# Runki2018/litehandnet

Hardware: AMD Instinct MI355X
Metric: images/sec fwd+bwd @256x256 bs64 litehandnet (higher is better)
Workload: dtype f32; 1 GPU; litehandnet variant B (MSRB hourglass litehourglass.py) C=128, 256x256x3 -> 21x64x64, per-GPU batch 64, train-mode BN, fwd + TopdownHeatmapLoss + bwd + fused Adam; global_batch=64, parallelism=dp1

## Files before the change

### include/lhn.h

```cpp
#ifndef LHN_H
#define LHN_H
#include <stdint.h>
#ifdef __cplusplus
extern "C" {
#endif

#define LHN_VERSION 3
#define LHN_STAT_REPLICAS 32

typedef struct lhn_view {
  float*       data;
  const float* table;
  const float* gate;
  int32_t N, H, W;
  int32_t cstride;
  int32_t coff;
  int32_t C;
  const void* pend;
} lhn_view;

typedef struct lhn_gradview {
  const float* dz;
  const float* dpool;
  const float* coef;
// ... 307 lines not shown
#define LHN_DW_F_NO_DX     32
#define LHN_DW_F_DX_ACC    64
#define LHN_DW_F_FINSRC    128
#define LHN_DW_SW_GATHER    1
#define LHN_DW_SW_BWD_V1    2
#define LHN_DW_SW_BWD_SMALL 4
const char* lhn_conv_dw_route(int backward, int H, int W, int C, int k, int stride, int pad, int dil, int features, int switches);
int lhn_conv_pw_bwd4(const lhn_view* x, const float* w, const lhn_view* y, const lhn_gradview* gy, float* dx, int dx_accumulate,
                     float* dw, float* dbias, int stride, const float* dy_nchw, int nrep, int64_t rep_stride,
                     const lhn_pw_opts* opts, const lhn_bnsum* bns, const lhn_bnbwdsrc* fin, void* stream);
#define LHN_PW_F_NCHW      1
#define LHN_PW_F_STATS     2
#define LHN_PW_F_FUSE_FIN  4
#define LHN_PW_F_EXTRA1    8
#define LHN_PW_F_EXTRA2    16
#define LHN_PW_F_SUM_OUT   32
#define LHN_PW_F_BNSUM     64
#define LHN_PW_F_FIN       128
#define LHN_PW_F_GATESUM   256
#define LHN_PW_F_NO_DX     512
#define LHN_PW_F_DX_ACC    1024
#define LHN_PW_F_DZ_DEAD   2048
#define LHN_PW_F_UNALIGNED 4096
#define LHN_PW_F_DBIAS     8192
#define LHN_PW_F_FINSRC    16384
#define LHN_PW_SW_LDSW          1
#define LHN_PW_SW_K256          2
#define LHN_PW_SW_BWD_NARROW    4
#define LHN_PW_SW_BWD_SPLIT     8
#define LHN_PW_SW_HEAD_STREAM   16
#define LHN_PW_SW_DETERMINISTIC 32
const char* lhn_conv_pw_route(int backward, int N, int H, int W, int Cin, int Cout, int stride, int w_rows, int w_cols, int features,
                              int switches);
int lhn_avgpool_bwd(const lhn_view* x, const float* dout , int OH, int OW, float* dx,
                    int dx_accumulate, void* stream);
int lhn_gate_bwd_reduce(const lhn_view* y, const float* dz, float* dgate , void* stream);
typedef struct lhn_bn_slices {
  const float* save[2];
  double*      sums[2];
  int32_t      lo[2], C[2];
  int32_t      n;
} lhn_bn_slices;
int lhn_gate_bwd_reduce2(const lhn_view* y, const float* dz, float* dgate , float* tsum,
                         const lhn_bn_slices* slices, void* stream);
int lhn_gate_bwd_reduce3(const lhn_view* y, const float* dz, float* dgate, float* tsum, const lhn_bn_slices* slices, int prezeroed,
                         void* stream);
typedef struct lhn_gatesum {
  float*               dgate;
  const lhn_bn_slices* slices;
} lhn_gatesum;
int lhn_conv_pw_bwd5(const lhn_view* x, const float* w, const lhn_view* y, const lhn_gradview* gy, float* dx, int dx_accumulate,
                     float* dw, float* dbias, int stride, const float* dy_nchw, int nrep, int64_t rep_stride,
                     const lhn_pw_opts* opts, const lhn_bnsum* bns, const lhn_bnbwdsrc* fin, const lhn_gatesum* gs, void* stream);
#define LHN_PW_BWD_DZ_DEAD 1
int lhn_conv_pw_bwd6(const lhn_view* x, const float* w, const lhn_view* y, const lhn_gradview* gy, float* dx, int dx_accumulate,
                     float* dw, float* dbias, int stride, const float* dy_nchw, int nrep, int64_t rep_stride,
                     const lhn_pw_opts* opts, const lhn_bnsum* bns, const lhn_bnbwdsrc* fin, const lhn_gatesum* gs, int flags,
                     void* stream);
int lhn_avgpool_fwd3(const lhn_view* x, float* out , int OH, int OW, float* pstat ,
                     const lhn_bn_slices* slices, void* stream);
int lhn_ca_mlp_bwd2(const float* pooled, const float* w3, const float* gamma, const float* w1, const float* w2,
                    const float* dropmask, const float* save, const float* dgate, float* dpool, int cstride, int coff, int H,
                    int W, float* dw3, float* dgamma, float* dbeta, float* dw1, float* db1, float* dw2, float* db2, int N, int C,
                    int stage, double* gsum, double count_scale, float pgrad_scale, const float* tsum, const float* pstat,
                    const lhn_bn_slices* slices, void* stream);
int lhn_avgpool_fwd4(const lhn_view* x, float* out, int OH, int OW, float* pstat, const lhn_bn_slices* slices,
                     const lhn_view* copy_src, void* stream);
int lhn_ca_mlp_bwd(const float* pooled, const float* w3, const float* gamma, const float* w1, const float* w2,
                   const float* dropmask, const float* save, const float* dgate, float* dpool ,
                   int cstride, int coff, int H, int W, float* dw3, float* dgamma, float* dbeta, float* dw1,
                   float* db1, float* dw2, float* db2, int N, int C, int stage, double* gsum, double count_scale,
                   float pgrad_scale, void* stream);

int lhn_cbam_layout(int N, int H, int W, int C, int64_t* save_off , int64_t* scratch_off );
int lhn_cbam_fwd(const lhn_view* p, const lhn_view* r, const float* w1, const float* w2, const float* w7, const lhn_view* out,
                 float* save, void* stream);
int lhn_cbam_bwd(const lhn_view* p, const lhn_view* r, const float* w1, const float* w2, const float* w7, const lhn_view* out,
                 const float* dout, float* dp, float* dr, float* dw1, float* dw2, float* dw7, const float* save, float* scratch,
                 void* stream);

int lhn_adam_step(float* param, const float* grad, float* exp_avg, float* exp_avg_sq, int64_t n, double lr, double beta1,
                  double beta2, double eps, double weight_decay, int64_t step, void* stream);

typedef struct lhn_op {
  int32_t kind;
  int32_t in_buf[3], in_coff[3], in_C[3];
  int32_t reserved[6];
  int32_t out_buf, out_coff, out_C;
  int32_t p[12];
  int64_t ws[12];
  int32_t i[8];
  float   f[8];
} lhn_op;

typedef struct lhn_buf {
  int64_t data_off, table_off, gate_off, grad_off, dpool_off, coef_off;
  int32_t N, H, W, C;
} lhn_buf;

void* lhn_plan_create(const lhn_buf* bufs, int nbufs, const lhn_op* fwd, int nfwd, const lhn_op* bwd, int nbwd);
void  lhn_plan_destroy(void* plan);
int   lhn_plan_head_gate_fold(void* plan);
int   lhn_plan_pw_dz_dead(void* plan, int bwd_index);
int   lhn_plan_fwd_fin_consumer(void* plan, int fwd_index);
#define LHN_RUN_TABLES_CURRENT 2
#define LHN_RUN_GRAPH 4
int   lhn_plan_run(void* plan, int phase, void* workspace, void* const* params, void* const* grads,
                   void* const* io, int training, int grad_replicas, int64_t grad_rep_stride, void* stream);

#ifdef __cplusplus
}
#endif
#endif
```

### litehandnet_amd/_lib.py

```python
import ctypes as C
import os

import torch

_HERE = os.path.dirname(os.path.abspath(__file__))
LIB_PATH = os.path.join(_HERE, "liblhn.so")
_lib = None


class LhnError(RuntimeError):
    pass


class View(C.Structure):
    _fields_ = [("data", C.c_void_p), ("table", C.c_void_p), ("gate", C.c_void_p),
                ("N", C.c_int32), ("H", C.c_int32), ("W", C.c_int32),
                ("cstride", C.c_int32), ("coff", C.c_int32), ("C", C.c_int32), ("pend", C.c_void_p)]


class GradView(C.Structure):
    _fields_ = [("dz", C.c_void_p), ("dpool", C.c_void_p), ("coef", C.c_void_p)]


class CcwSe(C.Structure):
    _fields_ = [("w1", C.c_void_p), ("b1", C.c_void_p), ("w2", C.c_void_p), ("b2", C.c_void_p), ("J", C.c_int32)]


class Op(C.Structure):
    _fields_ = [("kind", C.c_int32),
                ("in_buf", C.c_int32 * 3), ("in_coff", C.c_int32 * 3), ("in_C", C.c_int32 * 3), ("reserved", C.c_int32 * 6),
                ("out_buf", C.c_int32), ("out_coff", C.c_int32), ("out_C", C.c_int32),
                ("p", C.c_int32 * 12), ("ws", C.c_int64 * 12), ("i", C.c_int32 * 8), ("f", C.c_float * 8)]


class Buf(C.Structure):
    _fields_ = [("data_off", C.c_int64), ("table_off", C.c_int64), ("gate_off", C.c_int64),
                ("grad_off", C.c_int64), ("dpool_off", C.c_int64), ("coef_off", C.c_int64),
                ("N", C.c_int32), ("H", C.c_int32), ("W", C.c_int32), ("C", C.c_int32)]


SYMBOLS = [
    "lhn_version", "lhn_deterministic", "lhn_last_error", "lhn_device_ok",
    "lhn_heatmap_encode", "lhn_heatmap_argmax", "lhn_heatmap_refine", "lhn_transform_preds",
    "lhn_heatmap_decode", "lhn_heatmap_decode_dark", "lhn_heatmap_decode_dark_udp", "lhn_heatmap_nms", "lhn_heatmap_topk", "lhn_pck_accuracy",
    "lhn_eval_state_bytes", "lhn_eval_accumulate", "lhn_eval_finalize",
    "lhn_loss_balanced_mse_fwd", "lhn_loss_balanced_mse_bwd", "lhn_affine_warp_normalize", "lhn_affine_warp_normalize2", "lhn_random_flip", "lhn_hsv_jitter", "lhn_simdr_encode", "lhn_simdr_loss_fwd", "lhn_simdr_loss_bwd",
    "lhn_conv_pw_fwd", "lhn_conv_pw_fwd2", "lhn_conv_pw_bwd2", "lhn_conv_dw_fwd", "lhn_conv_dw_fwd2", "lhn_conv_dw_fwd3", "lhn_conv_pw_dw3_fwd", "lhn_conv_dw3_pw_fwd", "lhn_msrb_round_scratch_bytes", "lhn_msrb_round_fwd", "lhn_bottleneck_fwd", "lhn_stem_tail_fwd", "lhn_conv_stem_fwd", "lhn_conv_kxk_fwd", "lhn_conv_kxk_fwd_bf16x3",
    "lhn_bn_finalize", "lhn_table_fill", "lhn_table_bias", "lhn_fold_bn", "lhn_ew_fwd", "lhn_ew_fwd2", "lhn_ew_fwd3", "lhn_ew_mul_bwd", "lhn_bilinear_bwd", "lhn_shuffle2_fwd", "lhn_shuffle2_bwd", "lhn_bn_finalize2", "lhn_bn_bwd_finalize2", "lhn_maxpool2_fwd", "lhn_avgpool_fwd", "lhn_avgpool_fwd2", "lhn_avgpool_bwd2", "lhn_se_mlp_fwd2", "lhn_se_mlp_bwd2", "lhn_ca_mlp_fwd", "lhn_att_mlp_fwd", "lhn_att_mlp_bwd", "lhn_se_mlp_fwd", "lhn_se_mlp_bwd",
    "lhn_bn_bwd_reduce", "lhn_bn_bwd_finalize", "lhn_conv_pw_bwd", "lhn_conv_dw_bwd", "lhn_conv_dw_bwd2", "lhn_conv_dw_bwd3", "lhn_conv_dw_bwd4", "lhn_conv_dw_route", "lhn_conv_pw_route", "lhn_conv_pw_bwd4", "lhn_conv_pw_bwd5", "lhn_conv_pw_bwd6", "lhn_plan_head_gate_fold", "lhn_plan_pw_dz_dead", "lhn_plan_fwd_fin_consumer", "lhn_conv_dw_fwd4", "lhn_conv_pw_fwd3", "lhn_conv_stem_bwd",
    "lhn_conv_kxk_bwd", "lhn_ew_bwd", "lhn_ew_bwd2", "lhn_maxpool2_bwd", "lhn_maxpool2_bwd2", "lhn_maxpool2_bwd3", "lhn_ew_bwd3", "lhn_ew_bwd_multi", "lhn_avgpool_bwd3", "lhn_conv_pw_bwd3", "lhn_avgpool_bwd", "lhn_gate_bwd_reduce", "lhn_gate_bwd_reduce2", "lhn_gate_bwd_reduce3", "lhn_adam_step", "lhn_avgpool_fwd3", "lhn_avgpool_fwd4", "lhn_ca_mlp_bwd2",
    "lhn_ca_mlp_bwd", "lhn_reduce_replicas", "lhn_fold_stat_replicas", "lhn_plan_create", "lhn_plan_destroy", "lhn_plan_run", "lhn_plan_run_range",
    "lhn_cbam_layout", "lhn_cbam_fwd", "lhn_cbam_bwd",
    "lhn_ccw_scratch_bytes", "lhn_ccw_pool_fwd", "lhn_ccw_gate_fwd", "lhn_ccw_dw_fwd", "lhn_ccw_shuffle_fwd",
]


def lib():
    global _lib
    if _lib is None:
        if not os.path.exists(LIB_PATH):
            raise LhnError(f"{LIB_PATH} is missing: run `python -m litehandnet_amd.build` "
                           "(hipcc --offload-arch=gfx950); there is no CPU fallback")
        _lib = C.CDLL(LIB_PATH)
        _lib.lhn_last_error.restype = C.c_char_p
        _lib.lhn_plan_create.restype = C.c_void_p
        _lib.lhn_plan_destroy.restype = None
        _lib.lhn_eval_state_bytes.restype = C.c_int64
        _lib.lhn_conv_dw_route.argtypes = [C.c_int] * 10
        _lib.lhn_conv_dw_route.restype = C.c_char_p
        _lib.lhn_conv_pw_route.argtypes = [C.c_int] * 11
        _lib.lhn_conv_pw_route.restype = C.c_char_p
        _lib.lhn_conv_dw3_pw_fwd.argtypes = [C.c_void_p, C.c_void_p, C.c_int, C.c_void_p, C.c_void_p, C.c_void_p, C.c_void_p, C.c_void_p]
        _lib.lhn_conv_dw3_pw_fwd.restype = C.c_int
        _lib.lhn_msrb_round_scratch_bytes.argtypes = [C.c_int, C.c_int, C.c_int, C.c_int]
        _lib.lhn_msrb_round_scratch_bytes.restype = C.c_int64
        _lib.lhn_msrb_round_fwd.argtypes = [C.c_void_p, C.c_void_p, C.c_void_p, C.c_void_p, C.c_void_p, C.c_void_p, C.c_void_p, C.c_int, C.c_int,
                                            C.c_void_p, C.c_void_p]
        _lib.lhn_msrb_round_fwd.restype = C.c_int
        _lib.lhn_bottleneck_fwd.argtypes = [C.c_void_p, C.c_int] + [C.c_void_p] * 8 + [C.c_float, C.c_void_p, C.c_void_p, C.c_void_p]
        _lib.lhn_bottleneck_fwd.restype = C.c_int
        _lib.lhn_stem_tail_fwd.argtypes = [C.c_void_p, C.c_int] + [C.c_void_p] * 14
        _lib.lhn_stem_tail_fwd.restype = C.c_int
        _lib.lhn_conv_kxk_fwd_bf16x3.argtypes = [C.c_void_p, C.c_void_p, C.c_void_p, C.c_void_p, C.c_int, C.c_void_p]
        _lib.lhn_conv_kxk_fwd_bf16x3.restype = C.c_int
        _lib.lhn_ccw_scratch_bytes.argtypes = [C.c_int, C.c_int, C.c_void_p, C.c_void_p, C.c_void_p]
        _lib.lhn_ccw_scratch_bytes.restype = C.c_int64
        _lib.lhn_ccw_pool_fwd.argtypes = [C.c_void_p, C.c_int, C.c_void_p, C.c_void_p]
        _lib.lhn_ccw_pool_fwd.restype = C.c_int
        _lib.lhn_ccw_gate_fwd.argtypes = [C.c_void_p, C.c_int64, C.c_int, C.c_int, C.c_void_p, C.c_void_p, C.c_int, C.c_void_p, C.c_void_p, C.c_int,
                                          C.c_void_p, C.c_void_p]
        _lib.lhn_ccw_gate_fwd.restype = C.c_int
        _lib.lhn_ccw_dw_fwd.argtypes = [C.c_void_p, C.c_int] + [C.c_void_p] * 5
        _lib.lhn_ccw_dw_fwd.restype = C.c_int
        _lib.lhn_ccw_shuffle_fwd.argtypes = [C.c_void_p, C.c_void_p, C.c_int] + [C.c_void_p] * 4
        _lib.lhn_ccw_shuffle_fwd.restype = C.c_int
        _lib.lhn_cbam_layout.argtypes = [C.c_int, C.c_int, C.c_int, C.c_int, C.c_void_p, C.c_void_p]
        _lib.lhn_cbam_layout.restype = C.c_int
        _lib.lhn_cbam_fwd.argtypes = [C.c_void_p] * 8
        _lib.lhn_cbam_fwd.restype = C.c_int
        _lib.lhn_cbam_bwd.argtypes = [C.c_void_p] * 15
        _lib.lhn_cbam_bwd.restype = C.c_int
    return _lib


def cbam_layout(N, H, W, Cc):
    sv, sc = (C.c_int64 * 10)(), (C.c_int64 * 8)()
    check(lib().lhn_cbam_layout(N, H, W, Cc, sv, sc), "lhn_cbam_layout")
    return list(sv), list(sc)


def check(status, what=""):
    if status != 0:
        raise LhnError(f"{what}: status {status}: {lib().lhn_last_error().decode()}")


def require_device(t=None):
    if not torch.cuda.is_available():
        raise LhnError("no GPU visible: litehandnet_amd has no CPU fallback")
    if t is not None and not t.is_cuda:
        raise LhnError("tensor must live on the GPU (litehandnet_amd has no CPU fallback)")


def ptr(t):
    return C.c_void_p(0) if t is None else C.c_void_p(t.data_ptr())


def stream():
    return C.c_void_p(torch.cuda.current_stream().cuda_stream)


def f32c(t, name="tensor"):
    require_device(t)
    if t.dtype != torch.float32:
        t = t.float()
    return t.contiguous()
```

### litehandnet_amd/csrc/k_misc.hip

```cpp
#include "lhn_common.h"

static inline int grid_cap(int64_t blocks, int cap_per_cu) {
  const int64_t cap = (int64_t)lhn_num_cus() * cap_per_cu;
  if (blocks > cap) blocks = cap;
  if (blocks < 1) blocks = 1;
  return (int)blocks;
}
static inline bool pow2i(int v) { return v > 0 && (v & (v - 1)) == 0; }

__global__ void __launch_bounds__(LHN_FIN_THREADS) k_bn_finalize(const double* __restrict__ stats, const float* __restrict__ gamma,
                              const float* __restrict__ beta, float* __restrict__ rmean, float* __restrict__ rvar,
                              int64_t* __restrict__ nbt, float* __restrict__ table, int cs, int coff, int C,
                              float* __restrict__ save, double count, float eps, float momentum, float slope, int training,
                              const float* __restrict__ cbias, int SC) {
  __shared__ double part[2 * LHN_FIN_THREADS];
  const int nt = blockDim.x;
  int G = nt / C;
  G = G < 1 ? 1 : (G > LHN_STAT_REPLICAS ? LHN_STAT_REPLICAS : G);
  for (int c0 = 0; c0 < C; c0 += nt) {
    const int g = threadIdx.x / C, c = c0 + (G > 1 ? threadIdx.x - g * C : threadIdx.x);
    if (c0) __syncthreads();
    if (training && g < G && c < C) {
      double s1 = 0, s2 = 0;
#pragma unroll 4
      for (int r = g; r < LHN_STAT_REPLICAS; r += G) {
        s1 += stats[(size_t)r * 2 * SC + c];
        s2 += stats[(size_t)r * 2 * SC + SC + c];
      }
      part[2 * threadIdx.x] = s1;
      part[2 * threadIdx.x + 1] = s2;
    }
    __syncthreads();
    if (g != 0 || c >= C) continue;
    double mean, var;
    const double cb = cbias ? (double)cbias[c] : 0.0;
    if (training) {
      double s1 = 0, s2 = 0;
      for (int k = 0; k < G; ++k) {
        s1 += part[2 * (k * C + threadIdx.x)];
        s2 += part[2 * (k * C + threadIdx.x) + 1];
      }
      lhn_bn_fin_moments(s1, s2, count, mean, var);
      if (rmean) lhn_bn_fin_running(rmean, rvar, c, rmean[c], rvar[c], mean, var, cb, count, momentum);
    } else {
      mean = (double)rmean[c] - cb;
      var = rvar[c];
    }
    const LhnFinTab ft = lhn_bn_fin_tab(mean, var, eps, gamma ? gamma[c] : 1.f, beta ? beta[c] : 0.f);
    table[coff + c] = ft.sc;
    table[cs + coff + c] = ft.sh;
    table[2 * cs + coff + c] = slope;
    if (save && training) {
      save[c] = (float)mean;
      save[SC + c] = ft.invstd;
    }
  }
  if (training && nbt && threadIdx.x == 0) nbt[0] += 1;
}

__global__ void k_table_fill(float* __restrict__ table, int cs, int coff, int C, float sc, float sh, float sl) {
  for (int c = threadIdx.x; c < C; c += blockDim.x) {
    table[coff + c] = sc;
    table[cs + coff + c] = sh;
    table[2 * cs + coff + c] = sl;
  }
}

__global__ void k_table_bias(float* __restrict__ table, int cs, int coff, int C, const float* __restrict__ bias, float sl) {
  for (int c = threadIdx.x; c < C; c += blockDim.x) {
    table[coff + c] = 1.f;
    table[cs + coff + c] = bias ? bias[c] : 0.f;
    table[2 * cs + coff + c] = sl;
  }
}

struct EwSrcs {
  lhn_view v[3];
  float coef[3];
  int mode;
};
__device__ __forceinline__ void bil_taps(int d, int in, int out, int& i0, int& i1, float& w1) {
  if (in == out || out == 1) {
    i0 = i1 = (in == out) ? d : 0;
    w1 = 0.f;
    return;
  }
  const float pos = (float)d * ((float)(in - 1) / (float)(out - 1));
  i0 = (int)floorf(pos);
  if (i0 > in - 1) i0 = in - 1;
  i1 = i0 + 1 < in ? i0 + 1 : in - 1;
  w1 = pos - (float)i0;
}
__device__ __forceinline__ float lhn_relu_sigmoid(float v) { return 1.f / (1.f + expf(-fmaxf(v, 0.f))); }
__device__ __forceinline__ float lhn_relu_sigmoid_grad(float v) {
  if (!(v > 0.f)) return 0.f;
  const float s = 1.f / (1.f + expf(-v));
  return s * (1.f - s);
}
__device__ __forceinline__ int nearest_src(int d, int in, int out) {
  if (in == out) return d;
  const float sc = (float)in / (float)out;
  const int s = (int)floorf((float)d * sc);
  return s < in - 1 ? s : in - 1;
}
template <bool BIL>
__global__ void __launch_bounds__(256, BIL ? 1 : 3) k_ew_fwd(EwSrcs S, int nsrc, lhn_view dst, float out_slope) {
  const int C4 = dst.C >> 2, c4 = threadIdx.x % C4, pl = threadIdx.x / C4, PL = 256 / C4;
  const int rows = dst.N * dst.H;
  Xf4 xf[3];
  int ca[3];
#pragma unroll
  for (int k = 0; k < 3; ++k)
    if (k < nsrc) {
      ca[k] = S.v[k].coff + 4 * c4;
      xf[k] = lhn_load_xf(S.v[k], ca[k]);
    }
  for (int row = blockIdx.x; row < rows; row += gridDim.x) {
    const int n = row / dst.H, h = row - n * dst.H;
    const float* base[3];
    f4 gate[3];
#pragma unroll
    for (int k = 0; k < 3; ++k)
      if (k < nsrc) {
        const lhn_view& v = S.v[k];
        const int hs = nearest_src(h, v.H, dst.H);
        base[k] = v.data + ((size_t)(n * v.H + hs) * v.W) * v.cstride + ca[k];
        gate[k] = v.gate ? *reinterpret_cast<const f4*>(v.gate + (size_t)n * v.cstride + ca[k]) : (f4){1.f, 1.f, 1.f, 1.f};
      }
    float* out = dst.data + (size_t)row * dst.W * dst.cstride + dst.coff + 4 * c4;
    const bool mul = (S.mode & 1) != 0;
    constexpr bool bil = BIL;
    if (!bil) {
      for (int w0 = LHN_LANE0(pl, PL); w0 < dst.W; w0 += 4 * PL) {
        f4 raw[3][4];
#pragma unroll
        for (int k = 0; k < 3; ++k)
          if (k < nsrc) {
            const lhn_view& v = S.v[k];
#pragma unroll
            for (int j = 0; j < 4; ++j) {
              const int w = min(w0 + j * PL, dst.W - 1);
              const int ws = (v.W == dst.W) ? w : nearest_src(w, v.W, dst.W);
              raw[k][j] = *reinterpret_cast<const f4*>(base[k] + (size_t)ws * v.cstride);
            }
          }
#pragma unroll
        for (int j = 0; j < 4; ++j) {
          const int w = w0 + j * PL;
          if (w < dst.W) {
            f4 acc = mul ? (f4){1.f, 1.f, 1.f, 1.f} : (f4){0.f, 0.f, 0.f, 0.f};
#pragma unroll
            for (int k = 0; k < 3; ++k)
              if (k < nsrc) {
                const f4 val = lhn_apply_xf(raw[k][j], xf[k]) * (gate[k] * S.coef[k]);
                if (mul) acc *= val; else acc += val;
              }
            if (out_slope == LHN_SLOPE_RELU_SIGMOID) {
              acc.x = lhn_relu_sigmoid(acc.x); acc.y = lhn_relu_sigmoid(acc.y); acc.z = lhn_relu_sigmoid(acc.z); acc.w = lhn_relu_sigmoid(acc.w);
            } else if (out_slope == LHN_SLOPE_SILU) {
              acc.x = lhn_silu(acc.x); acc.y = lhn_silu(acc.y); acc.z = lhn_silu(acc.z); acc.w = lhn_silu(acc.w);
            } else {
              acc.x = lhn_lrelu(acc.x, out_slope); acc.y = lhn_lrelu(acc.y, out_slope); acc.z = lhn_lrelu(acc.z, out_slope); acc.w = lhn_lrelu(acc.w, out_slope);
            }
            *reinterpret_cast<f4*>(out + (size_t)w * dst.cstride) = acc;
          }
        }
      }
      continue;
    }
    for (int w = LHN_LANE0(pl, PL); w < dst.W; w += PL) {
      f4 acc = mul ? (f4){1.f, 1.f, 1.f, 1.f} : (f4){0.f, 0.f, 0.f, 0.f};
#pragma unroll
      for (int k = 0; k < 3; ++k)
        if (k < nsrc) {
          const lhn_view& v = S.v[k];
          f4 val;
          if (bil && (v.H != dst.H || v.W != dst.W)) {
            int h0, h1, w0, w1;
            float ah, aw;
            bil_taps(h, v.H, dst.H, h0, h1, ah);
            bil_taps(w, v.W, dst.W, w0, w1, aw);
            const float* b0 = v.data + ((size_t)(n * v.H + h0) * v.W) * v.cstride + ca[k];
            const float* b1 = v.data + ((size_t)(n * v.H + h1) * v.W) * v.cstride + ca[k];
            const f4 v00 = lhn_apply_xf(*reinterpret_cast<const f4*>(b0 + (size_t)w0 * v.cstride), xf[k]);
            const f4 v01 = lhn_apply_xf(*reinterpret_cast<const f4*>(b0 + (size_t)w1 * v.cstride), xf[k]);
            const f4 v10 = lhn_apply_xf(*reinterpret_cast<const f4*>(b1 + (size_t)w0 * v.cstride), xf[k]);
            const f4 v11 = lhn_apply_xf(*reinterpret_cast<const f4*>(b1 + (size_t)w1 * v.cstride), xf[k]);
            val = ((v00 * (1.f - aw) + v01 * aw) * (1.f - ah) + (v10 * (1.f - aw) + v11 * aw) * ah) * (gate[k] * S.coef[k]);
          } else {
            const int ws = nearest_src(w, v.W, dst.W);
            val = lhn_apply_xf(*reinterpret_cast<const f4*>(base[k] + (size_t)ws * v.cstride), xf[k]) * (gate[k] * S.coef[k]);
          }
          if (mul) acc *= val; else acc += val;
        }
      if (out_slope == LHN_SLOPE_RELU_SIGMOID) {
        acc.x = lhn_relu_sigmoid(acc.x);
        acc.y = lhn_relu_sigmoid(acc.y);
        acc.z = lhn_relu_sigmoid(acc.z);
        acc.w = lhn_relu_sigmoid(acc.w);
      } else if (out_slope == LHN_SLOPE_SILU) {
        acc.x = lhn_silu(acc.x);
        acc.y = lhn_silu(acc.y);
        acc.z = lhn_silu(acc.z);
        acc.w = lhn_silu(acc.w);
      } else {
        acc.x = lhn_lrelu(acc.x, out_slope);
        acc.y = lhn_lrelu(acc.y, out_slope);
        acc.z = lhn_lrelu(acc.z, out_slope);
        acc.w = lhn_lrelu(acc.w, out_slope);
      }
      *reinterpret_cast<f4*>(out + (size_t)w * dst.cstride) = acc;
    }
  }
}

__global__ void __launch_bounds__(256) k_ew_bwd_src(lhn_view src, lhn_view dst, const float* __restrict__ ddst,
                                                    const float* __restrict__ dst_dpool, float out_slope,
                                                    float* __restrict__ dsrc, int accumulate, lhn_bnsum bs) {
  __shared__ f4 bred[512];
  const int C4 = src.C >> 2, c4 = threadIdx.x % C4, pl = threadIdx.x / C4, PL = 256 / C4;
  f4 bsum = (f4){0.f, 0.f, 0.f, 0.f}, bsq = bsum, bmean = bsum, binv = bsum;
  Xf4 bxf;
  if (bs.sums) {
    bxf = lhn_load_xf(src, src.coff + 4 * c4);
    bmean = *reinterpret_cast<const f4*>(bs.save + bs.coff + 4 * c4);
    binv = *reinterpret_cast<const f4*>(bs.save + bs.C + bs.coff + 4 * c4);
  }
  const int fh = dst.H / src.H, fw = dst.W / src.W;
  const int cd = dst.coff + 4 * c4;
  const int rows = src.N * src.H;
  for (int row = blockIdx.x; row < rows; row += gridDim.x) {
    const int n = row / src.H, h = row - n * src.H;
    const f4 gate = dst.gate ? *reinterpret_cast<const f4*>(dst.gate + (size_t)n * dst.cstride + cd) : (f4){1.f, 1.f, 1.f, 1.f};
    for (int w = LHN_LANE0(pl, PL); w < src.W; w += PL) {
      f4 g = (f4){0.f, 0.f, 0.f, 0.f};
      for (int a = 0; a < fh; ++a)
        for (int b = 0; b < fw; ++b) {
          const int hd = h * fh + a, wd = w * fw + b;
          const size_t pd = ((size_t)(n * dst.H + hd) * dst.W + wd) * dst.cstride + cd;
          f4 e = *reinterpret_cast<const f4*>(ddst + pd) * gate;
          if (dst_dpool) {
            lhn_gradview gv{nullptr, dst_dpool, nullptr};
            e += lhn_dpool_sum(gv, dst, n, hd, wd, cd);
          }
          if (out_slope == LHN_SLOPE_SILU || out_slope == LHN_SLOPE_RELU_SIGMOID) {
            const Xf4 sxf = lhn_load_xf(src, src.coff + 4 * c4);
            const f4 v = lhn_load_val(src, sxf, (int64_t)(n * src.H + h) * src.W + w, n, src.coff + 4 * c4);
            if (out_slope == LHN_SLOPE_SILU) {
              e.x *= lhn_silu_grad(v.x);
              e.y *= lhn_silu_grad(v.y);
              e.z *= lhn_silu_grad(v.z);
              e.w *= lhn_silu_grad(v.w);
            } else {
              e.x *= lhn_relu_sigmoid_grad(v.x);
              e.y *= lhn_relu_sigmoid_grad(v.y);
              e.z *= lhn_relu_sigmoid_grad(v.z);
              e.w *= lhn_relu_sigmoid_grad(v.w);
            }
          } else if (out_slope != 1.f) {
            const f4 o = *reinterpret_cast<const f4*>(dst.data + pd);
            e.x *= o.x > 0.f ? 1.f : out_slope;
            e.y *= o.y > 0.f ? 1.f : out_slope;
            e.z *= o.z > 0.f ? 1.f : out_slope;
            e.w *= o.w > 0.f ? 1.f : out_slope;
          }
          g += e;
        }
      float* o = dsrc + ((size_t)row * src.W + w) * src.cstride + src.coff + 4 * c4;
      if (bs.sums) {
        const f4 raw = *reinterpret_cast<const f4*>(src.data + ((size_t)row * src.W + w) * src.cstride + src.coff + 4 * c4);
        const f4 du = g * lhn_dact_xf(raw, bxf);
        bsum += du;
        bsq += du * ((raw - bmean) * binv);
      }
      if (accumulate) g += *reinterpret_cast<const f4*>(o);
      *reinterpret_cast<f4*>(o) = g;
    }
  }
  if (bs.sums) lhn_bns_flush(bs, bsum, bsq, C4, bred);
}

struct EwBwdMulti {
  int n;
  lhn_view src[3];
  float* dsrc[3];
  int acc[3];
  lhn_bnsum bs[3];
};
__global__ void __launch_bounds__(256) k_ew_bwd_multi(EwBwdMulti m, lhn_view dst, const float* __restrict__ ddst,
                                                      const float* __restrict__ dst_dpool, float out_slope) {
  __shared__ f4 bred[512];
  const int C4 = dst.C >> 2, c4 = threadIdx.x % C4, pl = threadIdx.x / C4, PL = 256 / C4;
  f4 bsum[3], bsq[3], bmean[3], binv[3];
  Xf4 bxf[3];
#pragma unroll
  for (int k = 0; k < 3; ++k) {
    bsum[k] = bsq[k] = bmean[k] = binv[k] = (f4){0.f, 0.f, 0.f, 0.f};
    if (k < m.n && m.bs[k].sums) {
      bxf[k] = lhn_load_xf(m.src[k], m.src[k].coff + 4 * c4);
      bmean[k] = *reinterpret_cast<const f4*>(m.bs[k].save + m.bs[k].coff + 4 * c4);
      binv[k] = *reinterpret_cast<const f4*>(m.bs[k].save + m.bs[k].C + m.bs[k].coff + 4 * c4);
    }
  }
  const int cd = dst.coff + 4 * c4;
  const int rows = dst.N * dst.H;
  for (int row = blockIdx.x; row < rows; row += gridDim.x) {
    const int n = row / dst.H, h = row - n * dst.H;
    const f4 gate = dst.gate ? *reinterpret_cast<const f4*>(dst.gate + (size_t)n * dst.cstride + cd) : (f4){1.f, 1.f, 1.f, 1.f};
    for (int w = LHN_LANE0(pl, PL); w < dst.W; w += PL) {
      const size_t pix = (size_t)row * dst.W + w, pd = pix * dst.cstride + cd;
      f4 e = *reinterpret_cast<const f4*>(ddst + pd) * gate;
      if (dst_dpool) {
        lhn_gradview gv{nullptr, dst_dpool, nullptr};
        e += lhn_dpool_sum(gv, dst, n, h, w, cd);
      }
      if (out_slope != 1.f) {
        const f4 o = *reinterpret_cast<const f4*>(dst.data + pd);
        e.x *= o.x > 0.f ? 1.f : out_slope;
        e.y *= o.y > 0.f ? 1.f : out_slope;
        e.z *= o.z > 0.f ? 1.f : out_slope;
        e.w *= o.w > 0.f ? 1.f : out_slope;
      }
#pragma unroll
      for (int k = 0; k < 3; ++k) {
        if (k < m.n) {
          const size_t ps = pix * m.src[k].cstride + m.src[k].coff + 4 * c4;
          f4 g = e;
          if (m.bs[k].sums) {
            const f4 raw = *reinterpret_cast<const f4*>(m.src[k].data + ps);
            const f4 du = g * lhn_dact_xf(raw, bxf[k]);
            bsum[k] += du;
            bsq[k] += du * ((raw - bmean[k]) * binv[k]);
          }
          float* o = m.dsrc[k] + ps;
          if (m.acc[k]) g += *reinterpret_cast<const f4*>(o);
          *reinterpret_cast<f4*>(o) = g;
        }
      }
    }
  }
#pragma unroll
  for (int k = 0; k < 3; ++k)
    if (k < m.n && m.bs[k].sums) {
      lhn_bns_flush(m.bs[k], bsum[k], bsq[k], C4, bred);
      __syncthreads();
    }
}

__global__ void __launch_bounds__(256) k_maxpool2_fwd(lhn_view x, lhn_view y) {
  const int C4 = y.C >> 2, c4 = threadIdx.x % C4, pl = threadIdx.x / C4, PL = 256 / C4;
  const int ca = x.coff + 4 * c4;
  const Xf4 xf = lhn_load_xf(x, ca);
  const int rows = y.N * y.H;
  for (int row = blockIdx.x; row < rows; row += gridDim.x) {
    const int n = row / y.H, ho = row - n * y.H;
    const f4 gate = x.gate ? *reinterpret_cast<const f4*>(x.gate + (size_t)n * x.cstride + ca) : (f4){1.f, 1.f, 1.f, 1.f};
    for (int wo = LHN_LANE0(pl, PL); wo < y.W; wo += PL) {
      f4 m = (f4){-INFINITY, -INFINITY, -INFINITY, -INFINITY};
#pragma unroll
      for (int o = 0; o < 4; ++o) {
        const int ih = 2 * ho + (o >> 1), iw = 2 * wo + (o & 1);
        if (ih < x.H && iw < x.W) {
          const f4 v = lhn_apply_xf(*reinterpret_cast<const f4*>(x.data + ((size_t)(n * x.H + ih) * x.W + iw) * x.cstride + ca), xf) * gate;
          m.x = v.x > m.x || v.x != v.x ? v.x : m.x;
          m.y = v.y > m.y || v.y != v.y ? v.y : m.y;
          m.z = v.z > m.z || v.z != v.z ? v.z : m.z;
          m.w = v.w > m.w || v.w != v.w ? v.w : m.w;
        }
      }
      *reinterpret_cast<f4*>(y.data + ((size_t)row * y.W + wo) * y.cstride + y.coff + 4 * c4) = m;
    }
  }
}
template <bool ADD>
__global__ void __launch_bounds__(256) k_maxpool2_bwd(lhn_view x, lhn_view y, const float* __restrict__ dy,
                                                      float* __restrict__ dx, int accumulate, lhn_bnsum bs, lhn_grad_adds ad) {
  __shared__ f4 bred[512];
  const int C4 = y.C >> 2, c4 = threadIdx.x % C4, pl = threadIdx.x / C4, PL = 256 / C4;
  const int ca = x.coff + 4 * c4;
  const Xf4 xf = lhn_load_xf(x, ca);
  f4 bsum = (f4){0.f, 0.f, 0.f, 0.f}, bsq = bsum, bmean = bsum, binv = bsum;
  if (bs.sums) {
    bmean = *reinterpret_cast<const f4*>(bs.save + bs.coff + 4 * c4);
    binv = *reinterpret_cast<const f4*>(bs.save + bs.C + bs.coff + 4 * c4);
  }
  const int rows = y.N * y.H;
  for (int row = blockIdx.x; row < rows; row += gridDim.x) {
    const int n = row / y.H, ho = row - n * y.H;
    const f4 gate = x.gate ? *reinterpret_cast<const f4*>(x.gate + (size_t)n * x.cstride + ca) : (f4){1.f, 1.f, 1.f, 1.f};
    for (int wo = LHN_LANE0(pl, PL); wo < y.W; wo += PL) {
      const f4 g = *reinterpret_cast<const f4*>(dy + ((size_t)row * y.W + wo) * y.cstride + y.coff + 4 * c4);
      f4 m = (f4){-INFINITY, -INFINITY, -INFINITY, -INFINITY};
      int arg[4] = {-1, -1, -1, -1};
      f4 raws[4];
#pragma unroll
      for (int o = 0; o < 4; ++o) {
        const int ih = 2 * ho + (o >> 1), iw = 2 * wo + (o & 1);
        if (ih < x.H && iw < x.W) {
          raws[o] = *reinterpret_cast<const f4*>(x.data + ((size_t)(n * x.H + ih) * x.W + iw) * x.cstride + ca);
          const f4 v = lhn_apply_xf(raws[o], xf) * gate;
          if (v.x > m.x || v.x != v.x || arg[0] < 0) { if (!(m.x != m.x)) { m.x = v.x; arg[0] = o; } }
          if (v.y > m.y || v.y != v.y || arg[1] < 0) { if (!(m.y != m.y)) { m.y = v.y; arg[1] = o; } }
          if (v.z > m.z || v.z != v.z || arg[2] < 0) { if (!(m.z != m.z)) { m.z = v.z; arg[2] = o; } }
          if (v.w > m.w || v.w != v.w || arg[3] < 0) { if (!(m.w != m.w)) { m.w = v.w; arg[3] = o; } }
        }
      }
#pragma unroll
      for (int o = 0; o < 4; ++o) {
        const int ih = 2 * ho + (o >> 1), iw = 2 * wo + (o & 1);
        if (ih < x.H && iw < x.W) {
          f4 r = (f4){arg[0] == o ? g.x : 0.f, arg[1] == o ? g.y : 0.f, arg[2] == o ? g.z : 0.f, arg[3] == o ? g.w : 0.f};
          if (ADD) {
            if (ad.same) r += *reinterpret_cast<const f4*>(ad.same + ((size_t)(n * x.H + ih) * x.W + iw) * ad.same_cstride + ad.same_coff + 4 * c4);
            if (ad.pooled) {
              const int OH = ad.OH, OW = ad.OW, ohc = (ih * OH) / x.H, owc = (iw * OW) / x.W;
              for (int oh = max(ohc - 1, 0); oh <= min(ohc + 1, OH - 1); ++oh) {
                const int h0 = (oh * x.H) / OH, h1 = ((oh + 1) * x.H + OH - 1) / OH;
                if (ih < h0 || ih >= h1) continue;
                for (int ow = max(owc - 1, 0); ow <= min(owc + 1, OW - 1); ++ow) {
                  const int w0 = (ow * x.W) / OW, w1 = ((ow + 1) * x.W + OW - 1) / OW;
                  if (iw < w0 || iw >= w1) continue;
                  const float inv = 1.f / (float)((h1 - h0) * (w1 - w0));
                  r += *reinterpret_cast<const f4*>(ad.pooled + ((size_t)(n * OH + oh) * OW + ow) * ad.pooled_cstride + ad.pooled_coff + 4 * c4) * inv;
                }
              }
            }
          }
          float* q = dx + ((size_t)(n * x.H + ih) * x.W + iw) * x.cstride + ca;
          if (bs.sums) {
            const f4 du = r * lhn_dact_xf(raws[o], xf);
            bsum += du;
            bsq += du * ((raws[o] - bmean) * binv);
          }
          if (accumulate) r += *reinterpret_cast<const f4*>(q);
          *reinterpret_cast<f4*>(q) = r;
        }
      }
    }
  }
  if (bs.sums) lhn_bns_flush(bs, bsum, bsq, C4, bred);
}

struct BnSlices {
  const float* save[2];
  double* sums[2];
  int lo[2], C[2], n;
};
__device__ __forceinline__ void lhn_slice_mi4(const BnSlices& sl, int c, f4& mean, f4& inv) {
  mean = (f4){0.f, 0.f, 0.f, 0.f};
  inv = (f4){1.f, 1.f, 1.f, 1.f};
#pragma unroll
  for (int k = 0; k < 2; ++k)
    if (k < sl.n && c >= sl.lo[k] && c < sl.lo[k] + sl.C[k]) {
      mean = *reinterpret_cast<const f4*>(sl.save[k] + (c - sl.lo[k]));
      inv = *reinterpret_cast<const f4*>(sl.save[k] + sl.C[k] + (c - sl.lo[k]));
    }
}
__device__ __forceinline__ f4 lhn_dact4(f4 raw, const Xf4& t) {
  const f4 u = raw * t.sc + t.sh;
  return (f4){u.x > 0.f ? 1.f : t.sl.x, u.y > 0.f ? 1.f : t.sl.y, u.z > 0.f ? 1.f : t.sl.z, u.w > 0.f ? 1.f : t.sl.w};
}

template <bool STAT, bool COPY>
__global__ void __launch_bounds__(256) k_avgpool_fwd(lhn_view x, float* __restrict__ out, int OH, int OW, int ostride,
                                                     int ocoff, float* __restrict__ pstat, BnSlices sl, lhn_view src) {
  __shared__ f4 red[STAT ? 768 : 256];
  const int C4 = x.C >> 2, PL = 256 / C4;
  const int b = blockIdx.x;
  const int ow = b % OW, oh = (b / OW) % OH, n = b / (OW * OH);
  const int h0 = (oh * x.H) / OH, h1 = ((oh + 1) * x.H + OH - 1) / OH;
  const int w0 = (ow * x.W) / OW, w1 = ((ow + 1) * x.W + OW - 1) / OW;
  const int bw = w1 - w0, cnt = (h1 - h0) * bw;
  const int c4 = threadIdx.x % C4, pl = threadIdx.x / C4;
  const int ca = x.coff + 4 * c4;
  const bool cp = COPY && 4 * c4 < src.C;
  const int sca = src.coff + 4 * c4;
  Xf4 xf = lhn_load_xf(x, ca);
  f4 sgate = (f4){1.f, 1.f, 1.f, 1.f};
  if (cp) {
    xf = lhn_load_xf(src, sca);
    if (src.gate) sgate = *reinterpret_cast<const f4*>(src.gate + (int64_t)n * src.cstride + sca);
  }
  f4 mean, inv;
  if (STAT) lhn_slice_mi4(sl, ca, mean, inv);
  const float* base = cp ? src.data + (int64_t)n * x.H * x.W * src.cstride + sca : x.data + (int64_t)n * x.H * x.W * x.cstride + ca;
  const int64_t pstr = cp ? src.cstride : x.cstride;
  auto at = [&](int p) { return *reinterpret_cast<const f4*>(base + (int64_t)((h0 + p / bw) * x.W + w0 + p % bw) * pstr); };
  const int hown = ((oh + 1) * x.H) / OH, wown = ((ow + 1) * x.W) / OW;
  float* xout = x.data + (int64_t)n * x.H * x.W * x.cstride + ca;
  auto put = [&](int p, f4 v) {
    const int h = h0 + p / bw, w = w0 + p % bw;
    if (h < hown && w < wown) *reinterpret_cast<f4*>(xout + (int64_t)(h * x.W + w) * x.cstride) = v;
  };
  f4 s0 = (f4){0.f, 0.f, 0.f, 0.f}, s1 = s0, s2 = s0, s3 = s0, m0 = s0, m1 = s0;
  int p = LHN_LANE0(pl, PL);
  for (; p + 3 * PL < cnt; p += 4 * PL) {
    const f4 a = at(p), b2 = at(p + PL), c2 = at(p + 2 * PL), d2 = at(p + 3 * PL);
    const f4 va = lhn_apply_xf(a, xf) * sgate, vb = lhn_apply_xf(b2, xf) * sgate, vc = lhn_apply_xf(c2, xf) * sgate, vd = lhn_apply_xf(d2, xf) * sgate;
    s0 += va;
    s1 += vb;
    s2 += vc;
    s3 += vd;
    if (cp) {
      put(p, va);
      put(p + PL, vb);
      put(p + 2 * PL, vc);
      put(p + 3 * PL, vd);
    }
    if (STAT) {
      const f4 da = lhn_dact4(a, xf), db = lhn_dact4(b2, xf), dc = lhn_dact4(c2, xf), dd = lhn_dact4(d2, xf);
      m0 += (da + db) + (dc + dd);
      m1 += (da * ((a - mean) * inv) + db * ((b2 - mean) * inv)) + (dc * ((c2 - mean) * inv) + dd * ((d2 - mean) * inv));
    }
  }
  for (; p < cnt; p += PL) {
    const f4 a = at(p);
    const f4 va = lhn_apply_xf(a, xf) * sgate;
    s0 += va;
    if (cp) put(p, va);
    if (STAT) {
      const f4 da = lhn_dact4(a, xf);
      m0 += da;
      m1 += da * ((a - mean) * inv);
    }
  }
  f4 s = (s0 + s1) + (s2 + s3);
  if (x.gate) s *= *reinterpret_cast<const f4*>(x.gate + (int64_t)n * x.cstride + ca);
  const bool shuf = C4 <= 64 && (C4 & (C4 - 1)) == 0;
  if (shuf)
    for (int o = C4; o < 64; o <<= 1) {
      s.x += __shfl_xor(s.x, o, 64); s.y += __shfl_xor(s.y, o, 64); s.z += __shfl_xor(s.z, o, 64); s.w += __shfl_xor(s.w, o, 64);
      if (STAT) {
        m0.x += __shfl_xor(m0.x, o, 64); m0.y += __shfl_xor(m0.y, o, 64); m0.z += __shfl_xor(m0.z, o, 64); m0.w += __shfl_xor(m0.w, o, 64);
        m1.x += __shfl_xor(m1.x, o, 64); m1.y += __shfl_xor(m1.y, o, 64); m1.z += __shfl_xor(m1.z, o, 64); m1.w += __shfl_xor(m1.w, o, 64);
      }
    }
  const int lane = threadIdx.x & 63, wave = threadIdx.x >> 6;
  if (shuf && lane < C4) {
    red[wave * C4 + lane] = s;
    if (STAT) {
      red[256 + wave * C4 + lane] = m0;
      red[512 + wave * C4 + lane] = m1;
    }
  }
  if (!shuf) {
    red[threadIdx.x] = s;
    if (STAT) {
      red[256 + threadIdx.x] = m0;
      red[512 + threadIdx.x] = m1;
    }
  }
  __syncthreads();
  if (threadIdx.x < C4) {
    const int nj = shuf ? 4 : PL;
    f4 t = (f4){0.f, 0.f, 0.f, 0.f}, t0 = t, t1 = t;
    for (int j = 0; j < nj; ++j) {
      t += red[j * C4 + threadIdx.x];
      if (STAT) {
        t0 += red[256 + j * C4 + threadIdx.x];
        t1 += red[512 + j * C4 + threadIdx.x];
      }
    }
    const float invc = 1.f / (float)cnt;
    *reinterpret_cast<f4*>(out + (int64_t)b * ostride + ocoff + 4 * threadIdx.x) = t * invc;
    if (STAT) {
      *reinterpret_cast<f4*>(pstat + ((int64_t)b * 2 + 0) * x.C + 4 * threadIdx.x) = t0;
      *reinterpret_cast<f4*>(pstat + ((int64_t)b * 2 + 1) * x.C + 4 * threadIdx.x) = t1;
    }
  }
}
__global__ void __launch_bounds__(256) k_avgpool_small(lhn_view x, float* __restrict__ out, int OH, int OW, int ostride, int ocoff) {
  const int C4 = x.C >> 2;
  const int64_t total = (int64_t)x.N * OH * OW * C4;
  for (int64_t i = (int64_t)blockIdx.x * 256 + threadIdx.x; i < total; i += (int64_t)gridDim.x * 256) {
    const int c4 = (int)(i % C4);
    const int64_t b = i / C4;
    const int ow = (int)(b % OW), oh = (int)((b / OW) % OH), n = (int)(b / ((int64_t)OW * OH));
    const int h0 = (oh * x.H) / OH, h1 = ((oh + 1) * x.H + OH - 1) / OH;
    const int w0 = (ow * x.W) / OW, w1 = ((ow + 1) * x.W + OW - 1) / OW;
    const int ca = x.coff + 4 * c4;
    const Xf4 xf = lhn_load_xf(x, ca);
    f4 s = (f4){0.f, 0.f, 0.f, 0.f};
    for (int h = h0; h < h1; ++h)
      for (int w = w0; w < w1; ++w)
        s += lhn_apply_xf(*reinterpret_cast<const f4*>(x.data + ((int64_t)(n * x.H + h) * x.W + w) * x.cstride + ca), xf);
    if (x.gate) s *= *reinterpret_cast<const f4*>(x.gate + (int64_t)n * x.cstride + ca);
    *reinterpret_cast<f4*>(out + b * ostride + ocoff + 4 * c4) = s * (1.f / (float)((h1 - h0) * (w1 - w0)));
  }
}
__global__ void __launch_bounds__(256) k_avgpool_bwd(lhn_view x, const float* __restrict__ dout, int OH, int OW,
                                                     float* __restrict__ dx, int accumulate, int ostride, int ocoff, lhn_bnsum bs) {
  __shared__ f4 bred[512];
  const int C4 = x.C >> 2, c4 = threadIdx.x % C4, pl = threadIdx.x / C4, PL = 256 / C4;
  f4 bsum = (f4){0.f, 0.f, 0.f, 0.f}, bsq = bsum, bmean = bsum, binv = bsum;
  Xf4 bxf;
  if (bs.sums) {
    bxf = lhn_load_xf(x, x.coff + 4 * c4);
    bmean = *reinterpret_cast<const f4*>(bs.save + bs.coff + 4 * c4);
    binv = *reinterpret_cast<const f4*>(bs.save + bs.C + bs.coff + 4 * c4);
  }
  const int rows = x.N * x.H;
  for (int row = blockIdx.x; row < rows; row += gridDim.x) {
    const int n = row / x.H, h = row - n * x.H;
    for (int w = LHN_LANE0(pl, PL); w < x.W; w += PL) {
      f4 g = (f4){0.f, 0.f, 0.f, 0.f};
      const int ohc = (h * OH) / x.H, owc = (w * OW) / x.W;
      for (int oh = max(ohc - 1, 0); oh <= min(ohc + 1, OH - 1); ++oh) {
        const int h0 = (oh * x.H) / OH, h1 = ((oh + 1) * x.H + OH - 1) / OH;
        if (h < h0 || h >= h1) continue;
        for (int ow = max(owc - 1, 0); ow <= min(owc + 1, OW - 1); ++ow) {
          const int w0 = (ow * x.W) / OW, w1 = ((ow + 1) * x.W + OW - 1) / OW;
          if (w < w0 || w >= w1) continue;
          const float inv = 1.f / (float)((h1 - h0) * (w1 - w0));
          g += *reinterpret_cast<const f4*>(dout + ((size_t)(n * OH + oh) * OW + ow) * ostride + ocoff + 4 * c4) * inv;
        }
      }
      float* o = dx + ((size_t)row * x.W + w) * x.cstride + x.coff + 4 * c4;
      if (bs.sums) {
        const f4 raw = *reinterpret_cast<const f4*>(x.data + ((size_t)row * x.W + w) * x.cstride + x.coff + 4 * c4);
        const f4 du = g * lhn_dact_xf(raw, bxf);
        bsum += du;
        bsq += du * ((raw - bmean) * binv);
      }
      if (accumulate) g += *reinterpret_cast<const f4*>(o);
      *reinterpret_cast<f4*>(o) = g;
    }
  }
  if (bs.sums) lhn_bns_flush(bs, bsum, bsq, C4, bred);
}

__global__ void __launch_bounds__(1024) k_ca1(const float* __restrict__ pooled, const float* __restrict__ w3,
                                             const float* __restrict__ gamma, const float* __restrict__ beta,
                                             float* __restrict__ rmean, float* __restrict__ rvar, int64_t* __restrict__ nbt,
                                             const float* __restrict__ mask, float* __restrict__ save, int N, int C,
                                             float eps, float momentum, int training, int stage, double* __restrict__ gsum,
                                             double count_scale) {
  __shared__ double rs[32][32], rq[32][32];
  const int NL = blockDim.x >> 5;
  __shared__ float s_sc[32], s_sh[32];
  float* a = save;
  float* ahat = save + (int64_t)N * C;
  float* smean = save + (int64_t)N * C * 3 + (int64_t)N * (C / 2);
  float* sinv = smean + C;
  const int cl = threadIdx.x & 31, nl = threadIdx.x >> 5, c = blockIdx.x * 32 + cl;
  const bool ok = c < C;
  float wt[9];
#pragma unroll
  for (int t = 0; t < 9; ++t) wt[t] = ok ? w3[c * 9 + t] : 0.f;
  double s = 0, q = 0;
  if (ok && stage != 2)
    for (int n = nl; n < N; n += NL) {
      float v = 0.f;
// ... 900 lines not shown
  }
  double* st = sums + (size_t)(blockIdx.x % LHN_STAT_REPLICAS) * 2 * y.C;
  if (C4 <= 32 && (C4 & (C4 - 1)) == 0) {
    lhn_block_stat_atomics(s, q, C4, red, st, st + y.C);
  } else {
    red[threadIdx.x * 2] = s;
    red[threadIdx.x * 2 + 1] = q;
    __syncthreads();
    if (threadIdx.x < C4) {
      double sd[4] = {0, 0, 0, 0}, qd[4] = {0, 0, 0, 0};
      for (int j = 0; j < PL; ++j) {
        const f4 a = red[(j * C4 + threadIdx.x) * 2], b = red[(j * C4 + threadIdx.x) * 2 + 1];
        sd[0] += a.x; sd[1] += a.y; sd[2] += a.z; sd[3] += a.w;
        qd[0] += b.x; qd[1] += b.y; qd[2] += b.z; qd[3] += b.w;
      }
#pragma unroll
      for (int j = 0; j < 4; ++j) {
        atomicAdd(st + 4 * threadIdx.x + j, sd[j]);
        atomicAdd(st + y.C + 4 * threadIdx.x + j, qd[j]);
      }
    }
  }
  if (fin.counter && lhn_last_block(fin.counter)) lhn_bn_bwd_finalize_block(fin, sums, save);
}
__global__ void __launch_bounds__(LHN_FIN_THREADS) k_bn_bwd_finalize(const double* __restrict__ sums, const float* __restrict__ gamma,
                                  const float* __restrict__ save, float* __restrict__ coef, int cs, int coff, int C,
                                  double count, float* __restrict__ dgamma, float* __restrict__ dbeta, float pgrad_scale, int SC) {
  __shared__ double part[2 * LHN_FIN_THREADS];
  const int nt = blockDim.x, G = lhn_fin_groups(C);
  for (int c0 = 0; c0 < C; c0 += nt) {
    const int nc = min(G > 1 ? C : nt, C - c0);
    if (c0) __syncthreads();
    lhn_bn_bwd_fold_part(sums, SC, c0, nc, G, part);
    __syncthreads();
    if ((int)threadIdx.x >= nc) continue;
    const int c = c0 + threadIdx.x;
    const LhnBwdCoef r = lhn_bn_bwd_coef(part, nc, G, threadIdx.x, gamma ? gamma[c] : 1.f, save[c], save[SC + c], count);
    lhn_bn_bwd_coef_store(r, coef, cs, coff, c, dgamma, dbeta, pgrad_scale);
  }
}

__global__ void __launch_bounds__(256) k_reduce_replicas(float* __restrict__ out, const float* __restrict__ part, int64_t n4,
                                                         int nrep, int64_t rep_stride) {
  for (int64_t i = (int64_t)blockIdx.x * blockDim.x + threadIdx.x; i < n4; i += (int64_t)gridDim.x * blockDim.x) {
    f4 s = *reinterpret_cast<const f4*>(part + 4 * i);
    for (int r = 1; r < nrep; ++r) s += *reinterpret_cast<const f4*>(part + (size_t)r * rep_stride + 4 * i);
    *reinterpret_cast<f4*>(out + 4 * i) = s;
  }
}

__global__ void __launch_bounds__(256) k_fold_stat_replicas(double* __restrict__ st, int64_t n, int nrep) {
  for (int64_t i = (int64_t)blockIdx.x * 256 + threadIdx.x; i < n; i += (int64_t)gridDim.x * 256) {
    double s = st[i];
    for (int r = 1; r < nrep; ++r) {
      s += st[(int64_t)r * n + i];
      st[(int64_t)r * n + i] = 0.0;
    }
    st[i] = s;
  }
}

extern "C" {

int lhn_fold_stat_replicas(double* stats, int64_t n, int nrep, void* stream) {
  LHN_CHECK_ARG(stats && n > 0 && nrep >= 1, "lhn_fold_stat_replicas: bad argument");
  hipLaunchKernelGGL(k_fold_stat_replicas, dim3((unsigned)((n + 255) / 256 > 64 ? 64 : (n + 255) / 256)), dim3(256), 0, (hipStream_t)stream, stats, n, nrep);
  LHN_CHECK_LAUNCH("lhn_fold_stat_replicas");
  return 0;
}

int lhn_reduce_replicas(float* out, const float* part, int64_t n, int nrep, int64_t rep_stride, void* stream) {
  LHN_CHECK_ARG(out && part && n > 0 && n % 4 == 0 && nrep >= 1 && rep_stride % 4 == 0, "lhn_reduce_replicas: bad args (n and stride multiples of 4)");
  hipLaunchKernelGGL(k_reduce_replicas, dim3(grid_cap((n / 4 + 255) / 256, 8)), dim3(256), 0, (hipStream_t)stream, out, part, n / 4, nrep, rep_stride);
  LHN_CHECK_LAUNCH("lhn_reduce_replicas");
  return 0;
}

int lhn_bn_finalize(const double* stats, const float* gamma, const float* beta, float* running_mean, float* running_var,
                    int64_t* nbt, float* table, int cstride, int coff, int C, float* save, double count, float eps,
                    float momentum, float slope, int training, const float* conv_bias, void* stream) {
  return lhn_bn_finalize2(stats, gamma, beta, running_mean, running_var, nbt, table, cstride, coff, C, C, save, count, eps, momentum,
                          slope, training, conv_bias, stream);
}
int lhn_bn_finalize2(const double* stats, const float* gamma, const float* beta, float* running_mean, float* running_var,
                     int64_t* nbt, float* table, int cstride, int coff, int C, int stat_channels, float* save, double count,
                     float eps, float momentum, float slope, int training, const float* conv_bias, void* stream) {
  LHN_CHECK_ARG(table && C > 0 && coff >= 0 && coff + C <= cstride && stat_channels >= C, "lhn_bn_finalize: bad table slice");
  LHN_CHECK_ARG(training ? (stats != nullptr) : (running_mean && running_var), "lhn_bn_finalize: missing statistics");
  LHN_CHECK_ARG(!training || count >= 1, "lhn_bn_finalize: count");
  int nt = training ? (C >= LHN_FIN_THREADS ? LHN_FIN_THREADS : (LHN_FIN_THREADS / C > LHN_STAT_REPLICAS ? LHN_STAT_REPLICAS : LHN_FIN_THREADS / C) * C)
                    : (C <= 64 ? 64 : (C <= 128 ? 128 : 256));
  nt = (nt + 63) / 64 * 64;
  hipLaunchKernelGGL(k_bn_finalize, dim3(1), dim3(nt), 0, (hipStream_t)stream, stats,
                     gamma, beta, running_mean, running_var, nbt, table, cstride, coff, C, save, count, eps, momentum,
                     slope, training, conv_bias, stat_channels);
  LHN_CHECK_LAUNCH("lhn_bn_finalize");
  return 0;
}

int lhn_table_fill(float* table, int cstride, int coff, int C, float scale, float shift, float slope, void* stream) {
  LHN_CHECK_ARG(table && C > 0 && coff >= 0 && coff + C <= cstride, "lhn_table_fill: bad table slice");
  hipLaunchKernelGGL(k_table_fill, dim3(1), dim3(128), 0, (hipStream_t)stream, table, cstride, coff, C, scale, shift, slope);
  LHN_CHECK_LAUNCH("lhn_table_fill");
  return 0;
}

int lhn_table_bias(float* table, int cstride, int coff, int C, const float* bias, float slope, void* stream) {
  LHN_CHECK_ARG(table && C > 0 && coff >= 0 && coff + C <= cstride, "lhn_table_bias: bad slice");
  hipLaunchKernelGGL(k_table_bias, dim3(1), dim3(128), 0, (hipStream_t)stream, table, cstride, coff, C, bias, slope);
  LHN_CHECK_LAUNCH("lhn_table_bias");
  return 0;
}

int lhn_ew_fwd(const lhn_view* srcs, int nsrc, const lhn_view* dst, float out_slope, void* stream) {
  return lhn_ew_fwd2(srcs, nsrc, nullptr, dst, out_slope, stream);
}
int lhn_ew_fwd2(const lhn_view* srcs, int nsrc, const float* coef, const lhn_view* dst, float out_slope, void* stream) {
  return lhn_ew_fwd3(srcs, nsrc, coef, dst, out_slope, 0, stream);
}
int lhn_ew_fwd3(const lhn_view* srcs, int nsrc, const float* coef, const lhn_view* dst, float out_slope, int mode, void* stream) {
  LHN_CHECK_ARG(srcs && nsrc >= 1 && nsrc <= 3 && lhn_view_ok(dst) && mode >= 0 && mode <= 3, "lhn_ew_fwd: 1..3 sources, valid dst");
  EwSrcs S;
  memset(&S, 0, sizeof(S));
  S.mode = mode;
  for (int i = 0; i < nsrc; ++i) {
    LHN_CHECK_ARG(lhn_view_ok(&srcs[i]) && srcs[i].C == dst->C && srcs[i].N == dst->N && lhn_no_pend(&srcs[i]), "lhn_ew_fwd: source %d mismatch", i);
    S.v[i] = srcs[i];
    S.coef[i] = coef ? coef[i] : 1.f;
  }
  LHN_CHECK_ARG(dst->C % 4 == 0 && dst->C <= 1024, "lhn_ew_fwd: C=%d", dst->C);
  if (S.mode & 2)
    hipLaunchKernelGGL(k_ew_fwd<true>, dim3(grid_cap((int64_t)dst->N * dst->H, 8)), dim3(256), 0, (hipStream_t)stream, S, nsrc, *dst, out_slope);
  else
    hipLaunchKernelGGL(k_ew_fwd<false>, dim3(grid_cap((int64_t)dst->N * dst->H, 8)), dim3(256), 0, (hipStream_t)stream, S, nsrc, *dst, out_slope);
  LHN_CHECK_LAUNCH("lhn_ew_fwd");
  return 0;
}

int lhn_ew_bwd(const lhn_view* srcs, int nsrc, const lhn_view* dst, const float* ddst, float out_slope,
               float* const* dsrcs, const int* accumulate, void* stream) {
  LHN_CHECK_ARG(srcs && nsrc >= 1 && nsrc <= 3 && lhn_view_ok(dst) && ddst && dsrcs && accumulate, "lhn_ew_bwd: bad args");
  for (int i = 0; i < nsrc; ++i) {
    if (!dsrcs[i]) continue;
    const lhn_view* s = &srcs[i];
    LHN_CHECK_ARG(lhn_view_ok(s) && s->C == dst->C, "lhn_ew_bwd: source %d mismatch", i);
    LHN_CHECK_ARG(dst->H % s->H == 0 && dst->W % s->W == 0, "lhn_ew_bwd: non-integer upsample %dx%d -> %dx%d", s->H, s->W, dst->H, dst->W);
    LHN_CHECK_ARG(s->C % 4 == 0 && s->C <= 1024, "lhn_ew_bwd: C=%d", s->C);
    LHN_CHECK_ARG((out_slope != LHN_SLOPE_SILU && out_slope != LHN_SLOPE_RELU_SIGMOID) || (dst->H == s->H && dst->W == s->W),
                  "lhn_ew_bwd: SiLU / ReLU-sigmoid need a single same-size source (source %d)", i);
  }
  for (int i = 0; i < nsrc; ++i) {
    if (!dsrcs[i]) continue;
    const lhn_view* s = &srcs[i];
    lhn_bnsum nob;
    memset(&nob, 0, sizeof(nob));
    hipLaunchKernelGGL(k_ew_bwd_src, dim3(grid_cap((int64_t)s->N * s->H, 8)), dim3(256), 0, (hipStream_t)stream, *s, *dst, ddst,
                       (const float*)nullptr, out_slope, dsrcs[i], accumulate[i], nob);
  }
  LHN_CHECK_LAUNCH("lhn_ew_bwd");
  return 0;
}
static int bns_of(const lhn_bnsum* in, const lhn_view* v, lhn_bnsum* out, const char* who) {
  memset(out, 0, sizeof(*out));
  if (!in || !in->sums) return 0;
  LHN_CHECK_ARG(in->save && in->C > 0 && in->coff >= 0 && in->coff % 4 == 0 && in->coff + v->C <= in->C && !v->gate && v->table,
                "%s: BatchNorm sums need an ungated input view with a table, inside the producer's %d channels (offset %d, view %d)", who,
                in->C, in->coff, v->C);
  *out = *in;
  return 0;
}
int lhn_ew_bwd2(const lhn_view* src, const lhn_view* dst, const float* ddst, const float* dst_dpool, float out_slope,
                float* dsrc, int accumulate, void* stream) {
  return lhn_ew_bwd3(src, dst, ddst, dst_dpool, out_slope, dsrc, accumulate, nullptr, stream);
}
int lhn_ew_bwd3(const lhn_view* src, const lhn_view* dst, const float* ddst, const float* dst_dpool, float out_slope,
                float* dsrc, int accumulate, const lhn_bnsum* bns, void* stream) {
  LHN_CHECK_ARG(lhn_view_ok(src) && lhn_view_ok(dst) && ddst && dsrc && src->C == dst->C && lhn_no_pend(src) && lhn_no_pend(dst), "lhn_ew_bwd2: bad args");
  LHN_CHECK_ARG(dst->H % src->H == 0 && dst->W % src->W == 0, "lhn_ew_bwd2: non-integer upsample");
  LHN_CHECK_ARG((out_slope != LHN_SLOPE_SILU && out_slope != LHN_SLOPE_RELU_SIGMOID) || (dst->H == src->H && dst->W == src->W), "lhn_ew_bwd2: SiLU / ReLU-sigmoid need a single same-size source");
  LHN_CHECK_ARG(src->C % 4 == 0 && src->C <= 1024, "lhn_ew_bwd2: C=%d", src->C);
  lhn_bnsum bs;
  if (bns_of(bns, src, &bs, "lhn_ew_bwd3")) return 1;
  hipLaunchKernelGGL(k_ew_bwd_src, dim3(grid_cap((int64_t)src->N * src->H, 8)), dim3(256), 0, (hipStream_t)stream, *src, *dst, ddst,
                     dst_dpool, out_slope, dsrc, accumulate, bs);
  LHN_CHECK_LAUNCH("lhn_ew_bwd2");
  return 0;
}

int lhn_ew_bwd_multi(const lhn_view* srcs, int nsrc, const lhn_view* dst, const float* ddst, const float* dst_dpool, float out_slope,
                     float* const* dsrcs, const int* accumulate, const lhn_bnsum* const* bns, void* stream) {
  LHN_CHECK_ARG(srcs && nsrc >= 1 && nsrc <= 3 && lhn_view_ok(dst) && ddst && dsrcs && accumulate && lhn_no_pend(dst), "lhn_ew_bwd_multi: bad args");
  LHN_CHECK_ARG(out_slope != LHN_SLOPE_SILU && out_slope != LHN_SLOPE_RELU_SIGMOID, "lhn_ew_bwd_multi: SiLU / ReLU-sigmoid take lhn_ew_bwd3");
  LHN_CHECK_ARG(dst->C % 4 == 0 && dst->C <= 1024, "lhn_ew_bwd_multi: C=%d", dst->C);
  EwBwdMulti m;
  memset(&m, 0, sizeof(m));
  m.n = nsrc;
  for (int k = 0; k < nsrc; ++k) {
    const lhn_view* v = &srcs[k];
    LHN_CHECK_ARG(lhn_view_ok(v) && lhn_no_pend(v) && dsrcs[k] && v->C == dst->C && v->N == dst->N && v->H == dst->H && v->W == dst->W,
                  "lhn_ew_bwd_multi: source %d must have the destination's geometry", k);
    m.src[k] = *v;
    m.dsrc[k] = dsrcs[k];
    m.acc[k] = accumulate[k];
    if (bns_of(bns ? bns[k] : nullptr, v, &m.bs[k], "lhn_ew_bwd_multi")) return 1;
  }
  hipLaunchKernelGGL(k_ew_bwd_multi, dim3(grid_cap((int64_t)dst->N * dst->H, 8)), dim3(256), 0, (hipStream_t)stream, m, *dst, ddst, dst_dpool, out_slope);
  LHN_CHECK_LAUNCH("lhn_ew_bwd_multi");
  return 0;
}

int lhn_maxpool2_fwd(const lhn_view* x, const lhn_view* y, void* stream) {
  LHN_CHECK_ARG(lhn_view_ok(x) && lhn_view_ok(y) && x->C == y->C, "lhn_maxpool2_fwd: bad views");
  LHN_CHECK_ARG(y->H == (x->H + 1) / 2 && y->W == (x->W + 1) / 2 && y->N == x->N, "lhn_maxpool2_fwd: geometry");
  LHN_CHECK_ARG(y->C % 4 == 0 && y->C <= 1024, "lhn_maxpool2_fwd: C=%d", y->C);
  LHN_CHECK_ARG(lhn_no_pend(x), "lhn_maxpool2_fwd: lhn_view.pend is reserved (NULL)");
  hipLaunchKernelGGL(k_maxpool2_fwd, dim3(grid_cap((int64_t)y->N * y->H, 8)), dim3(256), 0, (hipStream_t)stream, *x, *y);
  LHN_CHECK_LAUNCH("lhn_maxpool2_fwd");
  return 0;
}
int lhn_maxpool2_bwd(const lhn_view* x, const lhn_view* y, const float* dy, float* dx, int dx_accumulate, void* stream) {
  return lhn_maxpool2_bwd2(x, y, dy, dx, dx_accumulate, nullptr, stream);
}
int lhn_maxpool2_bwd2(const lhn_view* x, const lhn_view* y, const float* dy, float* dx, int dx_accumulate, const lhn_bnsum* bns,
                      void* stream) {
  return lhn_maxpool2_bwd3(x, y, dy, dx, dx_accumulate, bns, nullptr, stream);
}
int lhn_maxpool2_bwd3(const lhn_view* x, const lhn_view* y, const float* dy, float* dx, int dx_accumulate, const lhn_bnsum* bns,
                      const lhn_grad_adds* adds, void* stream) {
  LHN_CHECK_ARG(lhn_view_ok(x) && lhn_view_ok(y) && dy && dx && x->C == y->C && lhn_no_pend(x), "lhn_maxpool2_bwd: bad args");
  LHN_CHECK_ARG(y->C % 4 == 0 && y->C <= 1024, "lhn_maxpool2_bwd: C=%d", y->C);
  lhn_bnsum bs;
  if (bns_of(bns, x, &bs, "lhn_maxpool2_bwd2")) return 1;
  lhn_grad_adds ad;
  memset(&ad, 0, sizeof(ad));
  if (adds && (adds->same || adds->pooled)) {
    ad = *adds;
    LHN_CHECK_ARG(x->H % 2 == 0 && x->W % 2 == 0 && y->H == x->H / 2 && y->W == x->W / 2, "lhn_maxpool2_bwd3: gradient addends need even H, W (%dx%d)", x->H, x->W);
    LHN_CHECK_ARG(!ad.same || (ad.same_cstride % 4 == 0 && ad.same_coff % 4 == 0 && ad.same_coff >= 0 && ad.same_coff + x->C <= ad.same_cstride),
                  "lhn_maxpool2_bwd3: same-resolution addend layout");
    LHN_CHECK_ARG(!ad.pooled || (ad.OH > 0 && ad.OW > 0 && ad.OH <= x->H && ad.OW <= x->W && ad.pooled_cstride % 4 == 0 && ad.pooled_coff % 4 == 0 &&
                                 ad.pooled_coff >= 0 && ad.pooled_coff + x->C <= ad.pooled_cstride),
                  "lhn_maxpool2_bwd3: pooled addend layout");
    hipLaunchKernelGGL(k_maxpool2_bwd<true>, dim3(grid_cap((int64_t)y->N * y->H, 8)), dim3(256), 0, (hipStream_t)stream, *x, *y, dy, dx, dx_accumulate, bs, ad);
  } else {
    hipLaunchKernelGGL(k_maxpool2_bwd<false>, dim3(grid_cap((int64_t)y->N * y->H, 8)), dim3(256), 0, (hipStream_t)stream, *x, *y, dy, dx, dx_accumulate, bs, ad);
  }
  LHN_CHECK_LAUNCH("lhn_maxpool2_bwd");
  return 0;
}

int lhn_avgpool_fwd(const lhn_view* x, float* out, int OH, int OW, void* stream) {
  return lhn_avgpool_fwd2(x, out, OH, OW, x ? x->C : 0, 0, stream);
}
int lhn_avgpool_fwd2(const lhn_view* x, float* out, int OH, int OW, int out_cstride, int out_coff, void* stream) {
  LHN_CHECK_ARG(lhn_view_ok(x) && out && OH > 0 && OW > 0 && out_coff >= 0 && out_coff % 4 == 0 && out_cstride % 4 == 0 &&
                    out_coff + x->C <= out_cstride,
                "lhn_avgpool_fwd: bad args");
  LHN_CHECK_ARG(x->C % 4 == 0 && x->C <= 1024, "lhn_avgpool_fwd: C=%d", x->C);
  LHN_CHECK_ARG(lhn_no_pend(x), "lhn_avgpool_fwd: lhn_view.pend is reserved (NULL)");
  const int binmax = ((x->H + OH - 1) / OH + 1) * ((x->W + OW - 1) / OW + 1);
  if (binmax <= 25) {
    const int64_t total = (int64_t)x->N * OH * OW * (x->C / 4);
    hipLaunchKernelGGL(k_avgpool_small, dim3(grid_cap((total + 255) / 256, 16)), dim3(256), 0, (hipStream_t)stream, *x, out, OH, OW, out_cstride, out_coff);
  } else
  {
    BnSlices sl;
    memset(&sl, 0, sizeof(sl));
    lhn_view nosrc;
    memset(&nosrc, 0, sizeof(nosrc));
    hipLaunchKernelGGL((k_avgpool_fwd<false, false>), dim3(x->N * OH * OW), dim3(256), 0, (hipStream_t)stream, *x, out, OH, OW, out_cstride, out_coff,
                       (float*)nullptr, sl, nosrc);
  }
  LHN_CHECK_LAUNCH("lhn_avgpool_fwd");
  return 0;
}
static int mk_slices(const lhn_bn_slices* in, int C, BnSlices* sl, const char* who) {
  memset(sl, 0, sizeof(*sl));
  if (!in) return 0;
  LHN_CHECK_ARG(in->n >= 0 && in->n <= 2, "%s: 0..2 BatchNorm slices", who);
  sl->n = in->n;
  for (int k = 0; k < in->n; ++k) {
    LHN_CHECK_ARG(in->save[k] && in->lo[k] >= 0 && in->C[k] > 0 && in->lo[k] % 4 == 0 && in->C[k] % 4 == 0 && in->lo[k] + in->C[k] <= C,
                  "%s: BatchNorm slice %d = channels [%d, %d) of %d", who, k, in->lo[k], in->lo[k] + in->C[k], C);
    sl->save[k] = in->save[k];
    sl->sums[k] = in->sums[k];
    sl->lo[k] = in->lo[k];
    sl->C[k] = in->C[k];
  }
  return 0;
}
int lhn_avgpool_fwd3(const lhn_view* x, float* out, int OH, int OW, float* pstat, const lhn_bn_slices* slices, void* stream) {
  return lhn_avgpool_fwd4(x, out, OH, OW, pstat, slices, nullptr, stream);
}
int lhn_avgpool_fwd4(const lhn_view* x, float* out, int OH, int OW, float* pstat, const lhn_bn_slices* slices, const lhn_view* copy_src,
                     void* stream) {
  if (!pstat && !copy_src) return lhn_avgpool_fwd2(x, out, OH, OW, x ? x->C : 0, 0, stream);
  LHN_CHECK_ARG(lhn_view_ok(x) && out && OH > 0 && OW > 0 && x->C % 4 == 0 && x->C <= 1024 && x->coff == 0 && x->C == x->cstride && lhn_no_pend(x),
                "lhn_avgpool_fwd4: the statistics / copy forms pool a whole buffer");
  LHN_CHECK_ARG(!copy_src || (lhn_view_ok(copy_src) && lhn_no_pend(copy_src) && copy_src->N == x->N && copy_src->H == x->H && copy_src->W == x->W &&
                              copy_src->C < x->C && copy_src->data != x->data),
                "lhn_avgpool_fwd4: copy_src = the first channels of the pooled tensor, same pixels, another buffer");
  BnSlices sl;
  if (mk_slices(pstat ? slices : nullptr, x->C, &sl, "lhn_avgpool_fwd4")) return 1;
  lhn_view src;
  memset(&src, 0, sizeof(src));
  if (copy_src) src = *copy_src;
  const dim3 g(x->N * OH * OW), bk(256);
  hipStream_t s = (hipStream_t)stream;
  if (pstat && copy_src) hipLaunchKernelGGL((k_avgpool_fwd<true, true>), g, bk, 0, s, *x, out, OH, OW, x->C, 0, pstat, sl, src);
  else if (pstat) hipLaunchKernelGGL((k_avgpool_fwd<true, false>), g, bk, 0, s, *x, out, OH, OW, x->C, 0, pstat, sl, src);
  else hipLaunchKernelGGL((k_avgpool_fwd<false, true>), g, bk, 0, s, *x, out, OH, OW, x->C, 0, pstat, sl, src);
  LHN_CHECK_LAUNCH("lhn_avgpool_fwd4");
  return 0;
}
int lhn_avgpool_bwd(const lhn_view* x, const float* dout, int OH, int OW, float* dx, int dx_accumulate, void* stream) {
  return lhn_avgpool_bwd2(x, dout, OH, OW, x ? x->C : 0, 0, dx, dx_accumulate, stream);
}
int lhn_avgpool_bwd2(const lhn_view* x, const float* dout, int OH, int OW, int out_cstride, int out_coff, float* dx,
                     int dx_accumulate, void* stream) {
  return lhn_avgpool_bwd3(x, dout, OH, OW, out_cstride, out_coff, dx, dx_accumulate, nullptr, stream);
}
int lhn_avgpool_bwd3(const lhn_view* x, const float* dout, int OH, int OW, int out_cstride, int out_coff, float* dx,
                     int dx_accumulate, const lhn_bnsum* bns, void* stream) {
  LHN_CHECK_ARG(lhn_view_ok(x) && dout && dx && out_coff >= 0 && out_coff + x->C <= out_cstride, "lhn_avgpool_bwd: bad args");
  LHN_CHECK_ARG(out_cstride % 4 == 0 && out_coff % 4 == 0, "lhn_avgpool_bwd: pooled gradient layout (stride %d, offset %d: multiples of 4)",
                out_cstride, out_coff);
  LHN_CHECK_ARG(OH >= 1 && OW >= 1 && OH <= x->H && OW <= x->W, "lhn_avgpool_bwd: pooled size %dx%d must be 1..%dx%d", OH, OW, x->H, x->W);
  LHN_CHECK_ARG(x->C % 4 == 0 && x->C <= 1024, "lhn_avgpool_bwd: C=%d", x->C);
  lhn_bnsum bs;
  if (bns_of(bns, x, &bs, "lhn_avgpool_bwd3")) return 1;
  hipLaunchKernelGGL(k_avgpool_bwd, dim3(grid_cap((int64_t)x->N * x->H, 8)), dim3(256), 0, (hipStream_t)stream, *x, dout, OH, OW, dx, dx_accumulate, out_cstride, out_coff, bs);
  LHN_CHECK_LAUNCH("lhn_avgpool_bwd");
  return 0;
}

static bool lhn_ca_mlp_staged(int C) {
  static int v = -1;
  if (v < 0) {
    const char* e = getenv("LHN_CA_MLP_V1");
    v = (e && e[0] == '1') ? 1 : 0;
  }
  return v == 0 && C <= LHN_CA_CMAX;
}

// ... 156 lines not shown
```

### litehandnet_amd/csrc/lhn_plan.cpp

```cpp
#include <stdint.h>
#include <stdlib.h>
#include <string.h>
#include <vector>
#include "lhn_common.h"

static lhn_bnsum mkbns(void* ws, int64_t sums_off, int64_t save_off, int C, int coff) {
  lhn_bnsum b;
  memset(&b, 0, sizeof(b));
  if (sums_off >= 0 && save_off >= 0 && C > 0) {
    b.sums = reinterpret_cast<double*>(static_cast<char*>(ws) + sums_off);
    b.save = reinterpret_cast<const float*>(static_cast<char*>(ws) + save_off);
    b.C = C;
    b.coff = coff;
  }
  return b;
}

enum {
  OP_STEM = 1, OP_PW = 2, OP_DW = 3, OP_KXK = 4, OP_FINALIZE = 5, OP_EW = 6, OP_MAXPOOL = 7, OP_AVGPOOL = 8,
  OP_CA_MLP = 9, OP_TABLE_FILL = 10, OP_MEMSET = 11, OP_ATT_MLP = 12, OP_SE_MLP = 13, OP_SHUFFLE = 14,
  OP_PWDW = 15, OP_DWPW = 16, OP_MSRB = 17, OP_CBAM = 18, OP_BNECK = 19, OP_STEMTAIL = 20,
  OP_CCW_POOL = 21, OP_CCW_GATE = 22, OP_CCW_DW = 23, OP_CCW_SHUFFLE = 24, OP_CCW_ARG = 25,
  OP_STEM_BWD = 101, OP_PW_BWD = 102, OP_DW_BWD = 103, OP_KXK_BWD = 104, OP_BN_BWD = 105, OP_EW_BWD = 106,
  OP_MAXPOOL_BWD = 107, OP_AVGPOOL_BWD = 108, OP_GATE_REDUCE = 109, OP_CA_MLP_BWD = 110, OP_ATT_MLP_BWD = 111, OP_SE_MLP_BWD = 112,
  OP_SHUFFLE_BWD = 113, OP_CBAM_BWD = 114,
};

struct GraphEntry {
  int phase, training, nrep, seen;
  int64_t rstr;
  void *ws, *io0, *io1;
  uint64_t phash, ghash;
  hipGraphExec_t exec;
  uint64_t last_use;
};

struct Plan {
  std::vector<lhn_buf> bufs;
  std::vector<lhn_op> fwd, bwd;
  std::vector<uint8_t> pw_dz_dead;
  std::vector<uint8_t> fwd_fin;
  std::vector<GraphEntry> graphs;
  uint64_t tick = 0;
  int graph_misses = 0;
};

static inline char* at(void* ws, int64_t off) { return off < 0 ? nullptr : static_cast<char*>(ws) + off; }

static lhn_view mkview(const Plan* P, void* ws, int buf, int coff, int C, bool with_gate = true) {
  const lhn_buf& b = P->bufs[buf];
  lhn_view v;
  v.pend = nullptr;
  v.data = reinterpret_cast<float*>(at(ws, b.data_off));
  v.table = reinterpret_cast<const float*>(at(ws, b.table_off));
  v.gate = with_gate ? reinterpret_cast<const float*>(at(ws, b.gate_off)) : nullptr;
  v.N = b.N; v.H = b.H; v.W = b.W;
  v.cstride = b.C; v.coff = coff; v.C = C;
  return v;
}
static lhn_gradview mkgrad(const Plan* P, void* ws, int buf, bool use_coef) {
  const lhn_buf& b = P->bufs[buf];
  lhn_gradview g;
  g.dz = reinterpret_cast<const float*>(at(ws, b.grad_off));
  g.dpool = reinterpret_cast<const float*>(at(ws, b.dpool_off));
  g.coef = use_coef ? reinterpret_cast<const float*>(at(ws, b.coef_off)) : nullptr;
  return g;
}
template <typename T>
static inline T* prm(void* const* arr, int idx) { return idx < 0 ? nullptr : static_cast<T*>(arr[idx]); }
static lhn_bn_slices mkslices(void* ws, const int32_t* pk, const int64_t* sv, const int64_t* sm) {
  lhn_bn_slices s;
  memset(&s, 0, sizeof(s));
  for (int k = 0; k < 2; ++k)
    if (pk[k] > 0 && sv[k] >= 0) {
      const int j = s.n++;
      s.lo[j] = pk[k] >> 16;
      s.C[j] = pk[k] & 0xffff;
      s.save[j] = reinterpret_cast<const float*>(at(ws, sv[k]));
      s.sums[j] = (sm && sm[k] >= 0) ? reinterpret_cast<double*>(at(ws, sm[k])) : nullptr;
    }
  return s;
}

static bool conv_has_bn(const lhn_op& o) { return o.p[2] >= 0 || o.p[3] >= 0 || o.ws[1] >= 0; }
static lhn_bnfin mkfin(const Plan* P, void* ws, const lhn_op& o, void* const* params) {
  const lhn_buf& b = P->bufs[o.out_buf];
  lhn_bnfin f;
  f.counter = reinterpret_cast<uint32_t*>(at(ws, o.ws[2]));
  f.gamma = prm<const float>(params, o.p[2]);
  f.beta = prm<const float>(params, o.p[3]);
  f.running_mean = prm<float>(params, o.p[4]);
  f.running_var = prm<float>(params, o.p[5]);
  f.num_batches_tracked = prm<int64_t>(params, o.p[6]);
  f.table = reinterpret_cast<float*>(at(ws, b.table_off));
  f.save_mean_invstd = reinterpret_cast<float*>(at(ws, o.ws[1]));
  f.count = (double)b.N * b.H * b.W;
  f.cstride = b.C; f.coff = o.out_coff; f.C = o.out_C;
  f.eps = o.f[0]; f.momentum = o.f[1]; f.slope = o.f[2];
  f.conv_bias = prm<const float>(params, o.p[1]);
  return f;
}
static bool fuse_finalize() {
  static int v = -1;
  if (v < 0) {
    const char* e = getenv("LHN_FUSE_FINALIZE");
    v = (e && e[0] == '1') ? 1 : 0;
  }
  return v == 1;
}
static bool bwd_fin_consumer() {
  static int v = -1;
  if (v < 0) {
    const char* e = getenv("LHN_BWD_FIN_CONSUMER");
    v = (e && e[0] == '0') ? 0 : 1;
  }
  return v == 1;
}
static bool fwd_fin_consumer() {
  static int v = -1;
  if (v < 0) {
    const char* e = getenv("LHN_FWD_FIN_CONSUMER");
    v = (e && e[0] == '0') ? 0 : 1;
  }
  return v == 1;
}
static bool fwd_fin_consumer_at(const Plan* P, const std::vector<lhn_op>& ops, size_t oi) {
  if (!fwd_fin_consumer() || fuse_finalize() || oi + 1 >= ops.size()) return false;
  const lhn_op &o = ops[oi], &nx = ops[oi + 1];
  const bool conv = o.kind == OP_STEM || o.kind == OP_PW || o.kind == OP_DW || (o.kind == OP_KXK && o.i[1] != 1);
  if (!conv || !conv_has_bn(o) || o.ws[0] < 0 || o.out_buf < 0 || (o.kind == OP_PW && (o.i[1] || o.i[2] > 0))) return false;
  if ((o.kind == OP_PW || o.kind == OP_DW) && (int)o.f[3] > 1) return false;
  if ((nx.kind != OP_DW && nx.kind != OP_PW) || nx.i[6] > 1) return false;
  if (nx.in_buf[0] != o.out_buf || nx.in_coff[0] != o.out_coff || nx.in_C[0] != o.out_C) return false;
  const lhn_buf& b = P->bufs[o.out_buf];
  if (b.table_off < 0) return false;
  const char* name;
  if (nx.kind == OP_DW)
    name = lhn_conv_dw_route(0, b.H, b.W, nx.in_C[0], nx.i[0], nx.i[1], nx.i[2], nx.i[3], LHN_DW_F_FINSRC | (nx.p[0] < 0 ? LHN_DW_F_NO_WEIGHT : 0), -1);
  else
    name = nx.i[1] ? nullptr
                   : lhn_conv_pw_route(0, b.N, b.H, b.W, nx.in_C[0], nx.out_C, nx.i[0], nx.i[2], nx.i[3],
                                       LHN_PW_F_FINSRC | (nx.ws[0] >= 0 ? LHN_PW_F_STATS : 0), -1);
  return name && strncmp(name, "lhn_bn_finalize", 15) != 0;
}
static bool head_gate_fold_at(const Plan* P, const std::vector<lhn_op>& ops, size_t oi) {
  if (!lhn_head_stream_on() || lhn_deterministic_mode() || oi + 1 >= ops.size()) return false;
  const lhn_op &o = ops[oi], &nx = ops[oi + 1];
  if (o.kind != OP_PW_BWD || !o.i[1] || o.i[0] != 1 || o.i[2] != 1 || o.in_buf[0] < 0) return false;
  if (o.i[3] || o.i[4] || !lhn_head_shape(o.in_C[0], o.out_C, o.in_C[0], o.out_C)) return false;
  const lhn_buf& b = P->bufs[o.in_buf[0]];
  return o.in_coff[0] == 0 && o.in_C[0] == b.C && b.gate_off >= 0 && nx.kind == OP_GATE_REDUCE && nx.out_buf == o.in_buf[0] &&
         nx.out_coff == 0 && nx.out_C == b.C && nx.ws[3] >= 0 && nx.ws[4] >= 0;
}
static bool pw_bwd_dy_store() {
  static int v = -1;
  if (v < 0) {
    const char* e = getenv("LHN_PW_BWD_DY_STORE");
    v = (e && e[0] == '1') ? 1 : 0;
  }
  return v == 1;
}
static bool pw_dz_dead_at(const Plan* P, const std::vector<lhn_op>& ops, size_t oi) {
  const lhn_op& o = ops[oi];
  if (o.kind != OP_PW_BWD || o.i[1] || o.out_buf < 0 || P->bufs[o.out_buf].grad_off < 0) return false;
  auto grad_bytes = [&](int buf, int64_t* lo, int64_t* hi) {
    const lhn_buf& b = P->bufs[buf];
    *lo = b.grad_off;
    *hi = b.grad_off + (int64_t)sizeof(float) * b.N * b.H * b.W * b.C;
    return b.grad_off >= 0;
  };
  int64_t lo, hi;
  grad_bytes(o.out_buf, &lo, &hi);
  const int oC = P->bufs[o.out_buf].C;
  auto touches = [&](int buf, int coff, int C) {
    int64_t a, b;
    if (buf < 0 || !grad_bytes(buf, &a, &b) || a >= hi || lo >= b) return false;
    return a != lo || P->bufs[buf].C != oC || (coff < o.out_coff + o.out_C && o.out_coff < coff + C);
  };
  for (size_t k = oi + 1; k < ops.size(); ++k) {
    const lhn_op& q = ops[k];
    if (q.kind == OP_MEMSET) {
      if (q.ws[0] < hi && lo < q.ws[0] + q.ws[1]) return false;
      continue;
    }
    if (touches(q.out_buf, q.out_coff, q.out_C)) return false;
    for (int s = 0; s < 3; ++s)
      if (touches(q.in_buf[s], q.in_coff[s], q.in_C[s])) return false;
    for (int s = 0; s < 12; ++s)
      if (q.ws[s] >= lo && q.ws[s] < hi) return false;
  }
  return true;
}

static int sep_finalize(const lhn_bnfin& f, const double* stats, int training, void* stream, int creal = 0, int repeat = 1) {
  int rc = 0;
  for (int r = 0; r < (training ? (repeat < 1 ? 1 : repeat) : 1) && !rc; ++r)
    rc = lhn_bn_finalize2(training ? stats : nullptr, f.gamma, f.beta, f.running_mean, f.running_var,
                          training ? f.num_batches_tracked : nullptr, f.table, f.cstride, f.coff, creal > 0 ? creal : f.C, f.C,
                          training ? f.save_mean_invstd : nullptr, f.count, f.eps, f.momentum, f.slope, training, f.conv_bias, stream);
  return rc;
}

extern "C" {

void* lhn_plan_create(const lhn_buf* bufs, int nbufs, const lhn_op* fwd, int nfwd, const lhn_op* bwd, int nbwd) {
  if (!bufs || nbufs <= 0 || !fwd || nfwd <= 0) {
    lhn_set_error("lhn_plan_create: empty plan");
    return nullptr;
  }
  Plan* p = new Plan();
  p->bufs.assign(bufs, bufs + nbufs);
  p->fwd.assign(fwd, fwd + nfwd);
  if (bwd && nbwd > 0) p->bwd.assign(bwd, bwd + nbwd);
  for (const auto* lst : {&p->fwd, &p->bwd})
    for (const lhn_op& o : *lst) {
      bool ok = o.out_buf < nbufs;
      for (int k = 0; k < 3; ++k) ok = ok && o.in_buf[k] < nbufs;
      if (!ok) {
        lhn_set_error("lhn_plan_create: op kind %d references buffer out of range", o.kind);
        delete p;
        return nullptr;
      }
    }
  p->fwd_fin.resize(p->fwd.size());
  for (size_t oi = 0; oi < p->fwd.size(); ++oi) p->fwd_fin[oi] = fwd_fin_consumer_at(p, p->fwd, oi) ? 1 : 0;
  p->pw_dz_dead.resize(p->bwd.size());
  for (size_t oi = 0; oi < p->bwd.size(); ++oi) p->pw_dz_dead[oi] = pw_dz_dead_at(p, p->bwd, oi) ? 1 : 0;
  return p;
}

int lhn_plan_head_gate_fold(void* plan) {
  const Plan* p = static_cast<const Plan*>(plan);
  if (!p) return -1;
  for (size_t oi = 0; oi + 1 < p->bwd.size(); ++oi)
    if (head_gate_fold_at(p, p->bwd, oi)) return (int)oi + 1;
  return -1;
}

int lhn_plan_pw_dz_dead(void* plan, int bwd_index) {
  const Plan* p = static_cast<const Plan*>(plan);
  if (!p || bwd_index < 0 || (size_t)bwd_index >= p->pw_dz_dead.size()) return -1;
  return p->pw_dz_dead[bwd_index];
}

int lhn_plan_fwd_fin_consumer(void* plan, int fwd_index) {
  const Plan* p = static_cast<const Plan*>(plan);
  if (!p || fwd_index < 0 || (size_t)fwd_index >= p->fwd_fin.size()) return -1;
  return p->fwd_fin[fwd_index];
}

void lhn_plan_destroy(void* plan) {
  Plan* p = static_cast<Plan*>(plan);
  if (!p) return;
  for (GraphEntry& g : p->graphs)
    if (g.exec) (void)hipGraphExecDestroy(g.exec);
  delete p;
}

static int run_ops(const Plan* P, int phase, void* ws, void* const* params, void* const* grads, void* const* io, int mode,
                   int nrep, int64_t rstr, void* stream, size_t sb = 0, size_t se = (size_t)-1, double cscale = 1.0,
                   float pscale = 1.f) {
  const int training = mode & 1;
  const bool skip_tables = (mode & 2) != 0 && !training;
  const std::vector<lhn_op>& ops = phase == 0 ? P->fwd : P->bwd;
  hipStream_t s = static_cast<hipStream_t>(stream);
  int rc = 0;
  const bool whole = (sb == 0 && se >= 2 * ops.size());
  lhn_bnbwdsrc cfin;
  size_t cfin_for = (size_t)-1;
  lhn_bnfinsrc ffin;
  size_t ffin_for = (size_t)-1;
  auto hand_over = [&](size_t oi, const lhn_bnfin& fin, const double* stats) {
    if (phase != 0 || !training || !whole || skip_tables || !P->fwd_fin[oi]) return false;
    ffin.stats = stats;
    ffin.gamma = fin.gamma; ffin.beta = fin.beta; ffin.conv_bias = fin.conv_bias;
    ffin.running_mean = fin.running_mean; ffin.running_var = fin.running_var; ffin.num_batches_tracked = fin.num_batches_tracked;
    ffin.table = fin.table; ffin.save_mean_invstd = fin.save_mean_invstd;
    ffin.count = fin.count;
    ffin.cstride = fin.cstride; ffin.coff = fin.coff; ffin.C = fin.C;
    ffin.eps = fin.eps; ffin.momentum = fin.momentum; ffin.slope = fin.slope;
    ffin_for = oi + 1;
    return true;
  };
  size_t gfold_at = (size_t)-1;
  for (size_t oi = 0; oi < ops.size() && rc == 0; ++oi) {
    const lhn_op& o = ops[oi];
    const bool deferred = false;
    const bool is_conv = o.kind == OP_STEM || o.kind == OP_PW || o.kind == OP_DW || o.kind == OP_KXK;
    const bool fz = is_conv && training && fuse_finalize() && whole && !(o.kind == OP_PW && o.i[2] > 0) &&
                    !((o.kind == OP_PW || o.kind == OP_DW) && (int)o.f[3] > 1);
    const bool h0 = 2 * oi >= sb && 2 * oi < se, h1 = 2 * oi + 1 >= sb && 2 * oi + 1 < se;
    if (!h0 && !h1) continue;
    const bool two_half = o.kind == OP_STEM || o.kind == OP_PW || o.kind == OP_DW || o.kind == OP_KXK || o.kind == OP_CA_MLP ||
                          o.kind == OP_ATT_MLP || o.kind == OP_BN_BWD || o.kind == OP_CA_MLP_BWD || o.kind == OP_ATT_MLP_BWD;
    if (!two_half && !h0) continue;
    const int stage = (h0 && h1) ? 0 : (h0 ? 1 : 2);
    switch (o.kind) {
      case OP_MEMSET: {
        if (hipMemsetAsync(at(ws, o.ws[0]), 0, (size_t)o.ws[1], s) != hipSuccess) {
          lhn_set_error("lhn_plan_run: memset failed");
          rc = 2;
        }
        break;
      }
      case OP_TABLE_FILL: {
        if (skip_tables) break;
        const lhn_buf& b = P->bufs[o.out_buf];
        if (o.i[0])
          rc = lhn_table_bias(reinterpret_cast<float*>(at(ws, b.table_off)), b.C, o.out_coff, o.out_C, prm<const float>(params, o.p[0]), o.f[2], stream);
        else
          rc = lhn_table_fill(reinterpret_cast<float*>(at(ws, b.table_off)), b.C, o.out_coff, o.out_C, o.f[0], o.f[1], o.f[2], stream);
        break;
      }
      case OP_STEM: {
        lhn_view y = mkview(P, ws, o.out_buf, o.out_coff, o.out_C);
        const bool bn = conv_has_bn(o);
        lhn_bnfin fin;
        if (bn) {
          fin = mkfin(P, ws, o, params);
          fin.count *= cscale;
        }
        if (h0) rc = lhn_conv_stem_fwd(static_cast<const float*>(io[0]), prm<const float>(params, o.p[0]), &y,
                               (training && o.ws[0] >= 0) ? reinterpret_cast<double*>(at(ws, o.ws[0])) : nullptr, o.i[3], o.i[4], o.i[0], o.i[1],
                               o.i[2], (bn && fz) ? &fin : nullptr, stream);
        if (!rc && bn && h1 && !skip_tables && !deferred && !fz && !hand_over(oi, fin, reinterpret_cast<const double*>(at(ws, o.ws[0]))))
          rc = sep_finalize(fin, reinterpret_cast<const double*>(at(ws, o.ws[0])), training, stream);
        break;
      }
      case OP_PW: {
        lhn_view x = mkview(P, ws, o.in_buf[0], o.in_coff[0], o.in_C[0]);
        lhn_view y;
        float* nchw = nullptr;
        if (o.i[1]) {
          y = x;
          y.data = nullptr; y.table = nullptr; y.gate = nullptr; y.pend = nullptr;
          y.cstride = o.out_C; y.coff = 0; y.C = o.out_C;
          nchw = static_cast<float*>(io[1]);
        } else {
          y = mkview(P, ws, o.out_buf, o.out_coff, o.out_C);
        }
        const bool bn = !o.i[1] && conv_has_bn(o);
        lhn_bnfin fin;
        if (bn) {
          fin = mkfin(P, ws, o, params);
          fin.count *= cscale;
        }
        lhn_pw_opts po;
        memset(&po, 0, sizeof(po));
        po.w_rows = o.i[2]; po.w_cols = o.i[3];
        lhn_view extra[2];
        if (o.i[6] > 1) {
          po.n_extra = o.i[6] - 1;
          for (int e = 0; e < po.n_extra; ++e) {
            extra[e] = mkview(P, ws, o.in_buf[e + 1], o.in_coff[e + 1], o.in_C[e + 1]);
          }
          po.extra = extra;
          for (int e = 0; e < 3; ++e) po.coef[e] = o.f[4 + e];
        }
        lhn_view sumv;
        if (o.i[6] > 1 && o.ws[4] >= 0) {
          sumv = x;
          sumv.data = reinterpret_cast<float*>(at(ws, o.ws[4]));
          sumv.table = nullptr; sumv.gate = nullptr; sumv.pend = nullptr;
          sumv.cstride = (int)(o.ws[5] >> 16); sumv.coff = (int)(o.ws[5] & 0xffff);
          po.sum_out = &sumv;
        }
        if (nchw && o.i[5] > 1) {
          const int64_t khw = (int64_t)o.out_C * y.H * y.W;
          nchw += (int64_t)o.i[4] * khw;
          po.nchw_batch_stride = (int64_t)o.i[5] * khw;
        }
        if (h0) rc = lhn_conv_pw_fwd3(&x, prm<const float>(params, o.p[0]), bn ? nullptr : prm<const float>(params, o.p[1]), &y,
                              (training && o.ws[0] >= 0) ? reinterpret_cast<double*>(at(ws, o.ws[0])) : nullptr, o.i[0], nchw,
                              (bn && fz) ? &fin : nullptr, &po, ffin_for == oi ? &ffin : nullptr, stream);
        if (!rc && bn && h1 && !skip_tables && !deferred && !fz && !hand_over(oi, fin, reinterpret_cast<const double*>(at(ws, o.ws[0]))))
          rc = sep_finalize(fin, reinterpret_cast<const double*>(at(ws, o.ws[0])), training, stream, o.i[2], (int)o.f[3]);
        break;
      }
      case OP_DW: {
        lhn_view x = mkview(P, ws, o.in_buf[0], o.in_coff[0], o.in_C[0]);
        lhn_view y = mkview(P, ws, o.out_buf, o.out_coff, o.out_C);
        const bool bn = conv_has_bn(o);
        lhn_bnfin fin;
        if (bn) {
          fin = mkfin(P, ws, o, params);
          fin.count *= cscale;
        }
        lhn_view extra;
        const float coef2[2] = {o.f[4], o.f[5]};
        if (o.i[6] > 1) {
          extra = mkview(P, ws, o.in_buf[1], o.in_coff[1], o.in_C[1]);
        }
        lhn_view sumv;
        const bool so = o.i[6] > 1 && o.ws[4] >= 0;
        if (so) {
          sumv = x;
          sumv.data = reinterpret_cast<float*>(at(ws, o.ws[4]));
          sumv.table = nullptr; sumv.gate = nullptr; sumv.pend = nullptr;
          sumv.cstride = (int)(o.ws[5] >> 16); sumv.coff = (int)(o.ws[5] & 0xffff);
        }
        if (h0) rc = lhn_conv_dw_fwd4(&x, prm<const float>(params, o.p[0]), &y,
                              (training && o.ws[0] >= 0) ? reinterpret_cast<double*>(at(ws, o.ws[0])) : nullptr, o.i[0], o.i[1], o.i[2], o.i[3],
                              (bn && fz) ? &fin : nullptr, o.i[6] > 1 ? &extra : nullptr, coef2,
                              so ? &sumv : nullptr, ffin_for == oi ? &ffin : nullptr, stream);
        if (!rc && bn && h1 && !skip_tables && !deferred && !fz && !hand_over(oi, fin, reinterpret_cast<const double*>(at(ws, o.ws[0]))))
          rc = sep_finalize(fin, reinterpret_cast<const double*>(at(ws, o.ws[0])), training, stream, 0, (int)o.f[3]);
        break;
      }
      case OP_KXK: {
        lhn_view x = mkview(P, ws, o.in_buf[0], o.in_coff[0], o.in_C[0]);
        lhn_view y = mkview(P, ws, o.out_buf, o.out_coff, o.out_C);
        const bool bn = conv_has_bn(o);
        lhn_bnfin fin;
        if (bn) {
          fin = mkfin(P, ws, o, params);
          fin.count *= cscale;
        }
        if (o.i[1] == 1) {
          if (training) {
            lhn_set_error("lhn_plan_run: a bf16x3 3x3 launch has no batch statistics (inference plans only)");
            rc = 1;
            break;
          }
          if (h0) rc = lhn_conv_kxk_fwd_bf16x3(&x, prm<const float>(params, o.p[0]), &y, o.ws[3] >= 0 ? at(ws, o.ws[3]) : nullptr,
                                               skip_tables ? 0 : 1, stream);
          if (!rc && bn && h1 && !skip_tables) rc = sep_finalize(fin, nullptr, 0, stream);
          break;
        }
        if (h0) rc = lhn_conv_kxk_fwd(&x, prm<const float>(params, o.p[0]), &y,
                              (training && o.ws[0] >= 0) ? reinterpret_cast<double*>(at(ws, o.ws[0])) : nullptr, o.i[0],
                              (bn && fz) ? &fin : nullptr,
                              o.ws[3] >= 0 ? reinterpret_cast<float*>(at(ws, o.ws[3])) : nullptr, stream);
        if (!rc && bn && h1 && !skip_tables && !deferred && !fz && !hand_over(oi, fin, reinterpret_cast<const double*>(at(ws, o.ws[0]))))
          rc = sep_finalize(fin, reinterpret_cast<const double*>(at(ws, o.ws[0])), training, stream);
        break;
      }
      case OP_PWDW: {
        if (training) {
          lhn_set_error("lhn_plan_run: a fused 1x1 -> depthwise launch has no batch statistics (inference plans only)");
          rc = 1;
          break;
        }
        lhn_view x = mkview(P, ws, o.in_buf[0], o.in_coff[0], o.in_C[0]);
        lhn_view y = mkview(P, ws, o.out_buf, o.out_coff, o.out_C);
        rc = lhn_conv_pw_dw3_fwd(&x, prm<const float>(params, o.p[0]), reinterpret_cast<const float*>(at(ws, P->bufs[o.in_buf[1]].table_off)),
                                 prm<const float>(params, o.p[1]), &y, stream);
        break;
      }
      case OP_DWPW: {
        if (training) {
          lhn_set_error("lhn_plan_run: a fused depthwise -> 1x1 launch has no batch statistics (inference plans only)");
          rc = 1;
          break;
        }
        lhn_view x = mkview(P, ws, o.in_buf[0], o.in_coff[0], o.in_C[0]);
        lhn_view y = mkview(P, ws, o.out_buf, o.out_coff, o.out_C);
        rc = lhn_conv_dw3_pw_fwd(&x, prm<const float>(params, o.p[0]), o.i[0], reinterpret_cast<const float*>(at(ws, P->bufs[o.in_buf[1]].table_off)),
                                 prm<const float>(params, o.p[1]), prm<const float>(params, o.p[2]), &y, stream);
        break;
      }
      case OP_BNECK: {
        if (training) {
          lhn_set_error("lhn_plan_run: a fused BottleNeck launch has no batch statistics (inference plans only)");
          rc = 1;
          break;
        }
        lhn_view x = mkview(P, ws, o.in_buf[0], o.in_coff[0], o.in_C[0]);
        lhn_view y = mkview(P, ws, o.out_buf, o.out_coff, o.out_C);
        rc = lhn_bottleneck_fwd_impl(&x, o.in_C[1], prm<const float>(params, o.p[0]), prm<const float>(params, o.p[1]),
                                     reinterpret_cast<const float*>(at(ws, P->bufs[o.in_buf[1]].table_off)), prm<const float>(params, o.p[2]),
                                     reinterpret_cast<const float*>(at(ws, P->bufs[o.in_buf[2]].table_off)), prm<const float>(params, o.p[3]),
                                     prm<const float>(params, o.p[4]), reinterpret_cast<const float*>(at(ws, o.ws[0])), o.f[0], &y,
                                     reinterpret_cast<float*>(at(ws, o.ws[1])), skip_tables ? 0 : 1, stream);
        break;
      }
      case OP_STEMTAIL: {
        if (training) {
          lhn_set_error("lhn_plan_run: a fused stem launch has no batch statistics (inference plans only)");
          rc = 1;
          break;
        }
        lhn_view x = mkview(P, ws, o.in_buf[0], o.in_coff[0], o.in_C[0]);
        lhn_view y = mkview(P, ws, o.out_buf, o.out_coff, o.out_C);
        rc = lhn_stem_tail_fwd_impl(&x, o.i[0], prm<const float>(params, o.p[0]), prm<const float>(params, o.p[1]),
                                    o.i[0] ? reinterpret_cast<const float*>(at(ws, P->bufs[o.in_buf[1]].table_off)) : nullptr,
                                    prm<const float>(params, o.p[2]), prm<const float>(params, o.p[3]),
                                    reinterpret_cast<const float*>(at(ws, P->bufs[o.in_buf[2]].table_off)), prm<const float>(params, o.p[4]),
                                    prm<const float>(params, o.p[5]), reinterpret_cast<const float*>(at(ws, o.ws[0])), o.i[1],
                                    prm<const float>(params, o.p[6]), prm<const float>(params, o.p[7]), &y,
                                    reinterpret_cast<float*>(at(ws, o.ws[1])), skip_tables ? 0 : 1, 0, stream);
        break;
      }
      case OP_MSRB: {
        if (training) {
          lhn_set_error("lhn_plan_run: a fused MSRB round has no batch statistics (inference plans only)");
          rc = 1;
          break;
        }
        const lhn_view x[2] = {mkview(P, ws, o.in_buf[0], o.in_coff[0], o.in_C[0]), mkview(P, ws, o.in_buf[1], o.in_coff[1], o.in_C[1])};
        lhn_view extra[2];
        const bool two = o.i[6] > 1;
        if (two) {
          if (o.in_buf[2] < 0 || o.i[1] < 0 || o.i[1] >= (int)P->bufs.size()) {
            lhn_set_error("lhn_plan_run: fused MSRB round: extra source out of range");
            rc = 1;
            break;
          }
          extra[0] = mkview(P, ws, o.in_buf[2], o.in_coff[2], o.in_C[2]);
          extra[1] = mkview(P, ws, o.i[1], o.i[2], o.i[3]);
        }
        const float coef2[2] = {o.f[4], o.f[5]};
        lhn_view y = mkview(P, ws, o.out_buf, o.out_coff, o.out_C, false);
        rc = lhn_msrb_round_fwd(x, two ? extra : nullptr, two ? coef2 : nullptr, prm<const float>(params, o.p[0]), prm<const float>(params, o.p[1]),
                                &y, reinterpret_cast<float*>(at(ws, o.ws[0])), o.i[0], o.i[0], at(ws, o.ws[1]), stream);
        break;
      }
      case OP_CCW_ARG:
// ... 1 lines not shown
      case OP_CCW_POOL:
      case OP_CCW_DW:
      case OP_CCW_SHUFFLE: {
        if (training) {
          lhn_set_error("lhn_plan_run: a grouped channel-weighting launch has no batch statistics (inference plans only)");
          rc = 1;
          break;
        }
        const int B = o.i[0];
        if (B < 2 || B > 4 || oi < (size_t)B) {
          lhn_set_error("lhn_plan_run: channel-weighting op at index %zu: %d branches", oi, B);
          rc = 1;
          break;
        }
        lhn_view x2[4], x1[4], y[4], out[4];
        const float* w[4];
        lhn_ccw_se se[4];
        for (int b = 0; b < B && rc == 0; ++b) {
          const lhn_op& g = ops[oi - B + b];
          if (g.kind != OP_CCW_ARG || g.in_buf[0] < 0 || g.in_buf[1] < 0 || g.in_buf[2] < 0 || g.out_buf < 0) {
            lhn_set_error("lhn_plan_run: channel-weighting op at index %zu: branch %d is not described", oi, b);
            rc = 1;
            break;
          }
          x2[b] = mkview(P, ws, g.in_buf[0], g.in_coff[0], g.in_C[0]);
          x1[b] = mkview(P, ws, g.in_buf[1], g.in_coff[1], g.in_C[1]);
          y[b] = mkview(P, ws, g.in_buf[2], g.in_coff[2], g.in_C[2], false);
          out[b] = mkview(P, ws, g.out_buf, g.out_coff, g.out_C);
          w[b] = prm<const float>(params, g.p[0]);
          se[b].w1 = prm<const float>(params, g.p[1]); se[b].b1 = prm<const float>(params, g.p[2]);
          se[b].w2 = prm<const float>(params, g.p[3]); se[b].b2 = prm<const float>(params, g.p[4]);
          se[b].J = g.i[0];
        }
        if (rc) break;
        if ((o.kind == OP_CCW_POOL && o.out_buf < 0) || (o.kind == OP_CCW_DW && o.in_buf[0] < 0)) {
          lhn_set_error("lhn_plan_run: channel-weighting op at index %zu: missing buffer", oi);
          rc = 1;
          break;
        }
        if (o.kind == OP_CCW_POOL)
          rc = lhn_ccw_pool_fwd(x2, B, reinterpret_cast<float*>(at(ws, P->bufs[o.out_buf].data_off)), stream);
        else if (o.kind == OP_CCW_DW)
          rc = lhn_ccw_dw_fwd(x2, B, reinterpret_cast<const float*>(at(ws, P->bufs[o.in_buf[0]].data_off)), w, y, at(ws, o.ws[0]), stream);
        else
          rc = lhn_ccw_shuffle_fwd(x1, y, B, se, at(ws, o.ws[0]), out, stream);
        break;
      }
      case OP_CCW_GATE: {
        if (training) {
          lhn_set_error("lhn_plan_run: a grouped channel-weighting launch has no batch statistics (inference plans only)");
          rc = 1;
          break;
        }
        if (o.in_buf[0] < 0 || o.in_buf[1] < 0 || o.in_buf[2] < 0 || o.out_buf < 0) {
          lhn_set_error("lhn_plan_run: channel-weighting gate at index %zu: missing buffer", oi);
          rc = 1;
          break;
        }
        const lhn_buf &pb = P->bufs[o.in_buf[0]], &b1 = P->bufs[o.in_buf[1]], &b2 = P->bufs[o.in_buf[2]], &gb = P->bufs[o.out_buf];
        if (gb.C != pb.C || gb.H != pb.H || gb.W != pb.W) {
          lhn_set_error("lhn_plan_run: channel-weighting gate at index %zu: pooled and g differ", oi);
          rc = 1;
          break;
        }
        rc = lhn_ccw_gate_fwd(reinterpret_cast<const float*>(at(ws, pb.data_off)), (int64_t)pb.N * pb.H * pb.W, pb.C, o.i[0],
                              prm<const float>(params, o.p[0]), reinterpret_cast<const float*>(at(ws, b1.table_off)), b1.C,
                              prm<const float>(params, o.p[1]), reinterpret_cast<const float*>(at(ws, b2.table_off)), b2.C,
                              reinterpret_cast<float*>(at(ws, gb.data_off)), stream);
        break;
      }
      case OP_FINALIZE: {
        if (skip_tables) break;
        const lhn_buf& b = P->bufs[o.out_buf];
        const int src = o.in_buf[0] >= 0 ? o.in_buf[0] : o.out_buf;
        const lhn_buf& sb = P->bufs[src];
        rc = lhn_bn_finalize(reinterpret_cast<const double*>(at(ws, o.ws[0])), prm<const float>(params, o.p[0]),
                             prm<const float>(params, o.p[1]), prm<float>(params, o.p[2]), prm<float>(params, o.p[3]),
                             prm<int64_t>(params, o.p[4]), reinterpret_cast<float*>(at(ws, b.table_off)), b.C, o.out_coff,
                             o.out_C, reinterpret_cast<float*>(at(ws, o.ws[1])), (double)sb.N * sb.H * sb.W, o.f[0], o.f[1],
                             o.f[2], training, prm<const float>(params, o.p[5]), stream);
        break;
      }
      case OP_EW: {
        lhn_view srcs[3];
        for (int k = 0; k < o.i[0]; ++k) {
          srcs[k] = mkview(P, ws, o.in_buf[k], o.in_coff[k], o.in_C[k]);
        }
        lhn_view d = mkview(P, ws, o.out_buf, o.out_coff, o.out_C);
        const float coef[3] = {o.f[4], o.f[5], o.f[6]};
        rc = lhn_ew_fwd3(srcs, o.i[0], o.i[1] ? coef : nullptr, &d, o.f[0], o.i[2], stream);
        break;
      }
      case OP_MAXPOOL: {
        lhn_view x = mkview(P, ws, o.in_buf[0], o.in_coff[0], o.in_C[0]);
        lhn_view y = mkview(P, ws, o.out_buf, o.out_coff, o.out_C);
        rc = lhn_maxpool2_fwd(&x, &y, stream);
        break;
      }
      case OP_SHUFFLE: {
        lhn_view a = mkview(P, ws, o.in_buf[0], o.in_coff[0], o.in_C[0]);
        lhn_view b = mkview(P, ws, o.in_buf[1], o.in_coff[1], o.in_C[1]);
        lhn_view d = mkview(P, ws, o.out_buf, o.out_coff, o.out_C);
        rc = lhn_shuffle2_fwd(&a, &b, &d, stream);
        break;
      }
      case OP_AVGPOOL: {
        lhn_view x = mkview(P, ws, o.in_buf[0], o.in_coff[0], o.in_C[0], o.i[2] == 0);
        if (o.ws[1] >= 0 || o.in_buf[1] >= 0) {
          const lhn_bn_slices sl = mkslices(ws, &o.i[5], &o.ws[2], nullptr);
          lhn_view src;
          if (o.in_buf[1] >= 0) src = mkview(P, ws, o.in_buf[1], o.in_coff[1], o.in_C[1]);
          rc = lhn_avgpool_fwd4(&x, reinterpret_cast<float*>(at(ws, o.ws[0])), o.i[0], o.i[1],
                                o.ws[1] >= 0 ? reinterpret_cast<float*>(at(ws, o.ws[1])) : nullptr, &sl, o.in_buf[1] >= 0 ? &src : nullptr, stream);
          break;
        }
        rc = lhn_avgpool_fwd2(&x, reinterpret_cast<float*>(at(ws, o.ws[0])), o.i[0], o.i[1], o.i[3] > 0 ? o.i[3] : x.C, o.i[4], stream);
        break;
      }
      case OP_CA_MLP: {
        const lhn_buf& b = P->bufs[o.out_buf];
        if ((!training || o.ws[3] < 0) && !h0) break;
        rc = lhn_ca_mlp_fwd(reinterpret_cast<const float*>(at(ws, o.ws[0])), prm<const float>(params, o.p[0]),
                            prm<const float>(params, o.p[1]), prm<const float>(params, o.p[2]), prm<float>(params, o.p[3]),
                            prm<float>(params, o.p[4]), prm<int64_t>(params, o.p[5]), prm<const float>(params, o.p[6]),
                            prm<const float>(params, o.p[7]), prm<const float>(params, o.p[8]), prm<const float>(params, o.p[9]),
                            (training && o.ws[2] >= 0) ? reinterpret_cast<const float*>(at(ws, o.ws[2])) : nullptr,
                            reinterpret_cast<float*>(at(ws, b.gate_off)), b.C, o.out_coff,
                            reinterpret_cast<float*>(at(ws, o.ws[1])), b.N, o.out_C, o.f[0], o.f[1], training,
                            (training && o.ws[3] >= 0) ? stage : 0, o.ws[3] >= 0 ? reinterpret_cast<double*>(at(ws, o.ws[3])) : nullptr,
                            cscale, stream);
        break;
      }
      case OP_ATT_MLP: {
        const lhn_buf& b = P->bufs[o.out_buf];
        if ((!training || o.ws[3] < 0) && !h0) break;
        rc = lhn_att_mlp_fwd(reinterpret_cast<const float*>(at(ws, o.ws[0])), prm<const float>(params, o.p[0]),
                             prm<const float>(params, o.p[1]), prm<float>(params, o.p[2]), prm<float>(params, o.p[3]),
                             prm<int64_t>(params, o.p[4]), prm<const float>(params, o.p[5]), prm<const float>(params, o.p[6]),
                             prm<const float>(params, o.p[7]), prm<const float>(params, o.p[8]),
                             (training && o.ws[2] >= 0) ? reinterpret_cast<const float*>(at(ws, o.ws[2])) : nullptr,
                             reinterpret_cast<float*>(at(ws, b.gate_off)), b.C, o.out_coff,
                             reinterpret_cast<float*>(at(ws, o.ws[1])), b.N, o.out_C, o.f[0], o.f[1], training,
                             (training && o.ws[3] >= 0) ? stage : 0, o.ws[3] >= 0 ? reinterpret_cast<double*>(at(ws, o.ws[3])) : nullptr,
                             cscale, stream);
        break;
      }
      case OP_SE_MLP: {
        const lhn_buf& b = P->bufs[o.out_buf];
        rc = lhn_se_mlp_fwd2(reinterpret_cast<const float*>(at(ws, o.ws[0])), prm<const float>(params, o.p[0]),
                             prm<const float>(params, o.p[1]), prm<const float>(params, o.p[2]), prm<const float>(params, o.p[3]),
                             reinterpret_cast<float*>(at(ws, b.gate_off)), b.C, o.out_coff, reinterpret_cast<float*>(at(ws, o.ws[1])),
                             b.N, o.out_C, o.i[0], o.i[1], stream);
        break;
      }
      case OP_STEM_BWD: {
        lhn_view y = mkview(P, ws, o.out_buf, o.out_coff, o.out_C);
        lhn_gradview g = mkgrad(P, ws, o.out_buf, o.i[5] != 0);
        rc = lhn_conv_stem_bwd(static_cast<const float*>(io[0]), &y, &g, prm<float>(grads, o.p[1]), o.i[3], o.i[4], o.i[0],
                               o.i[1], o.i[2], nrep, rstr, stream);
        break;
      }
      case OP_PW_BWD: {
        lhn_view x = mkview(P, ws, o.in_buf[0], o.in_coff[0], o.in_C[0]);
        lhn_view y;
        lhn_gradview g;
        const float* nchw = nullptr;
        if (o.i[1]) {
          y = x;
          y.data = nullptr; y.table = nullptr; y.gate = nullptr;
          y.cstride = o.out_C; y.coff = 0; y.C = o.out_C;
          g.dz = nullptr; g.dpool = nullptr; g.coef = nullptr;
          nchw = static_cast<const float*>(io[1]);
        } else {
          y = mkview(P, ws, o.out_buf, o.out_coff, o.out_C);
          g = mkgrad(P, ws, o.out_buf, o.i[5] != 0);
        }
        float* dx = o.i[2] ? reinterpret_cast<float*>(at(ws, P->bufs[o.in_buf[0]].grad_off)) : nullptr;
        lhn_pw_opts po;
        memset(&po, 0, sizeof(po));
        po.w_rows = o.i[3]; po.w_cols = o.i[4];
        if (nchw && o.i[7] > 1) {
          const int64_t khw = (int64_t)o.out_C * y.H * y.W;
          nchw += (int64_t)o.i[6] * khw;
          po.nchw_batch_stride = (int64_t)o.i[7] * khw;
        }
        const lhn_bnsum bs = mkbns(ws, o.ws[0], o.ws[1], (int)o.f[6], (int)o.f[7]);
        lhn_gatesum gsum;
        lhn_bn_slices gsl;
        memset(&gsum, 0, sizeof(gsum));
        if (phase == 1 && whole && head_gate_fold_at(P, ops, oi)) {
          const lhn_op& nx = ops[oi + 1];
          gsl = mkslices(ws, &nx.i[0], &nx.ws[5], nullptr);
          gsum.dgate = reinterpret_cast<float*>(at(ws, nx.ws[3]));
          gsum.slices = &gsl;
          gfold_at = oi + 1;
        }
        const int flags = (phase == 1 && whole && P->pw_dz_dead[oi] && !pw_bwd_dy_store()) ? LHN_PW_BWD_DZ_DEAD : 0;
        rc = lhn_conv_pw_bwd6(&x, prm<const float>(params, o.p[0]), &y, &g, dx, o.i[2] == 2, prm<float>(grads, o.p[1]),
                              prm<float>(grads, o.p[2]), o.i[0], nchw, nrep, rstr, &po, bs.sums ? &bs : nullptr,
                              cfin_for == oi ? &cfin : nullptr, gsum.dgate ? &gsum : nullptr, flags, stream);
        break;
      }
      case OP_DW_BWD: {
        lhn_view x = mkview(P, ws, o.in_buf[0], o.in_coff[0], o.in_C[0]);
        lhn_view y = mkview(P, ws, o.out_buf, o.out_coff, o.out_C);
        lhn_gradview g = mkgrad(P, ws, o.out_buf, o.i[5] != 0);
        float* dx = o.i[4] ? reinterpret_cast<float*>(at(ws, P->bufs[o.in_buf[0]].grad_off)) : nullptr;
        const bool adds = o.ws[2] >= 0 || o.ws[3] >= 0;
        const lhn_bnsum bs = mkbns(ws, adds ? -1 : o.ws[4], adds ? -1 : o.ws[5], o.i[6], o.i[7]);
        rc = lhn_conv_dw_bwd4(&x, prm<const float>(params, o.p[0]), &y, &g, dx, o.i[4] == 2, prm<float>(grads, o.p[1]), o.i[0], o.i[1],
                              o.i[2], o.i[3], nrep, rstr, bs.sums ? &bs : nullptr,
                              o.ws[2] >= 0 ? reinterpret_cast<const float*>(at(ws, o.ws[2])) : nullptr,
                              o.ws[3] >= 0 ? reinterpret_cast<const float*>(at(ws, o.ws[3])) : nullptr, cfin_for == oi ? &cfin : nullptr, stream);
        break;
      }
      case OP_KXK_BWD: {
        lhn_view x = mkview(P, ws, o.in_buf[0], o.in_coff[0], o.in_C[0]);
        lhn_view y = mkview(P, ws, o.out_buf, o.out_coff, o.out_C);
        lhn_gradview g = mkgrad(P, ws, o.out_buf, o.i[5] != 0);
        float* dx = o.i[2] ? reinterpret_cast<float*>(at(ws, P->bufs[o.in_buf[0]].grad_off)) : nullptr;
        rc = lhn_conv_kxk_bwd(&x, prm<const float>(params, o.p[0]), &y, &g, dx, o.i[2] == 2, prm<float>(grads, o.p[1]), o.i[0],
                              nrep, rstr, o.ws[3] >= 0 ? reinterpret_cast<float*>(at(ws, o.ws[3])) : nullptr, stream);
        break;
      }
      case OP_BN_BWD: {
        const lhn_buf& b = P->bufs[o.out_buf];
        lhn_view y = mkview(P, ws, o.out_buf, o.out_coff, o.out_C);
        lhn_gradview g = mkgrad(P, ws, o.out_buf, false);
        double* sums = reinterpret_cast<double*>(at(ws, o.ws[0]));
        const float* save = reinterpret_cast<const float*>(at(ws, o.ws[1]));
        lhn_bnbwdfin fin;
        fin.counter = reinterpret_cast<uint32_t*>(at(ws, o.ws[2]));
        fin.gamma = prm<const float>(params, o.p[0]);
        fin.coef = reinterpret_cast<float*>(at(ws, b.coef_off));
        fin.dgamma = prm<float>(grads, o.p[1]);
        fin.dbeta = prm<float>(grads, o.p[2]);
        fin.count = (double)b.N * b.H * b.W * cscale;
        fin.cstride = b.C; fin.coff = o.out_coff; fin.C = o.out_C;
        if (fin.counter && fuse_finalize() && whole && !o.i[1]) {
          rc = lhn_bn_bwd_reduce(&y, &g, save, sums, &fin, stream);
        } else {
          if (h0 && !o.i[1]) rc = lhn_bn_bwd_reduce(&y, &g, save, sums, nullptr, stream);
          const lhn_op* nx = oi + 1 < ops.size() ? &ops[oi + 1] : nullptr;
          if (!rc && h1 && whole && bwd_fin_consumer() && !fuse_finalize() && o.i[0] == 0 && nx &&
              (nx->kind == OP_DW_BWD || (nx->kind == OP_PW_BWD && !nx->i[1])) && nx->out_buf == o.out_buf && nx->out_coff == o.out_coff &&
              nx->out_C == o.out_C && nx->i[5] != 0) {
            cfin.sums = sums;
            cfin.save_mean_invstd = save;
            cfin.gamma = fin.gamma;
            cfin.dgamma = fin.dgamma;
            cfin.dbeta = fin.dbeta;
            cfin.count = fin.count;
            cfin.pgrad_scale = pscale;
            cfin.stat_channels = o.out_C;
            cfin_for = oi + 1;
          } else if (!rc && h1)
            rc = lhn_bn_bwd_finalize2(sums, fin.gamma, save, fin.coef, b.C, o.out_coff, o.i[0] > 0 ? o.i[0] : o.out_C, o.out_C, fin.count,
                                      fin.dgamma, fin.dbeta, pscale, stream);
        }
        break;
      }
      case OP_EW_BWD: {
        lhn_view src = mkview(P, ws, o.in_buf[0], o.in_coff[0], o.in_C[0]);
        lhn_view d = mkview(P, ws, o.out_buf, o.out_coff, o.out_C);
        const lhn_buf& db = P->bufs[o.out_buf];
        if (o.i[1] == 1) {
          lhn_view other = mkview(P, ws, o.in_buf[1], o.in_coff[1], o.in_C[1]);
          rc = lhn_ew_mul_bwd(&src, &other, &d, reinterpret_cast<const float*>(at(ws, db.grad_off)),
                              reinterpret_cast<float*>(at(ws, P->bufs[o.in_buf[0]].grad_off)), o.i[0], stream);
        } else if (o.i[1] == 2) {
          rc = lhn_bilinear_bwd(&src, &d, reinterpret_cast<const float*>(at(ws, db.grad_off)),
                                reinterpret_cast<float*>(at(ws, P->bufs[o.in_buf[0]].grad_off)), o.i[0], o.f[0], stream);
        } else if (o.i[1] == 3) {
          lhn_view srcs[3];
          float* dsrcs[3];
          int acc[3] = {o.i[0], o.i[2], o.i[3]};
          lhn_bnsum bsv[3] = {mkbns(ws, o.ws[0], o.ws[1], o.i[4], o.i[5]), mkbns(ws, o.ws[2], o.ws[3], o.i[6], o.i[7]),
                              mkbns(ws, o.ws[4], o.ws[5], (int)o.f[4], (int)o.f[5])};
          const lhn_bnsum* bsp[3];
          int ns = 0;
          for (; ns < 3 && o.in_buf[ns] >= 0; ++ns) {
            srcs[ns] = mkview(P, ws, o.in_buf[ns], o.in_coff[ns], o.in_C[ns]);
            dsrcs[ns] = reinterpret_cast<float*>(at(ws, P->bufs[o.in_buf[ns]].grad_off));
            bsp[ns] = bsv[ns].sums ? &bsv[ns] : nullptr;
          }
          rc = lhn_ew_bwd_multi(srcs, ns, &d, reinterpret_cast<const float*>(at(ws, db.grad_off)),
                                reinterpret_cast<const float*>(at(ws, db.dpool_off)), o.f[0], dsrcs, acc, bsp, stream);
        } else {
          const lhn_bnsum bs = mkbns(ws, o.ws[0], o.ws[1], o.i[4], o.i[5]);
          rc = lhn_ew_bwd3(&src, &d, reinterpret_cast<const float*>(at(ws, db.grad_off)),
                           reinterpret_cast<const float*>(at(ws, db.dpool_off)), o.f[0],
                           reinterpret_cast<float*>(at(ws, P->bufs[o.in_buf[0]].grad_off)), o.i[0], bs.sums ? &bs : nullptr, stream);
        }
        break;
      }
      case OP_MAXPOOL_BWD: {
        lhn_view x = mkview(P, ws, o.in_buf[0], o.in_coff[0], o.in_C[0]);
        lhn_view y = mkview(P, ws, o.out_buf, o.out_coff, o.out_C);
        const lhn_bnsum bs = mkbns(ws, o.ws[0], o.ws[1], o.i[4], o.i[5]);
        lhn_grad_adds ad;
        memset(&ad, 0, sizeof(ad));
        if (o.ws[2] >= 0) {
          ad.same = reinterpret_cast<const float*>(at(ws, o.ws[2]));
          ad.same_cstride = o.i[1]; ad.same_coff = o.i[2];
        }
        if (o.ws[3] >= 0) {
          ad.pooled = reinterpret_cast<const float*>(at(ws, o.ws[3]));
          ad.pooled_cstride = o.i[3]; ad.pooled_coff = o.i[6];
          ad.OH = o.i[7] >> 16; ad.OW = o.i[7] & 0xffff;
        }
        rc = lhn_maxpool2_bwd3(&x, &y, reinterpret_cast<const float*>(at(ws, P->bufs[o.out_buf].grad_off)),
                               reinterpret_cast<float*>(at(ws, P->bufs[o.in_buf[0]].grad_off)), o.i[0], bs.sums ? &bs : nullptr,
                               (ad.same || ad.pooled) ? &ad : nullptr, stream);
        break;
      }
      case OP_AVGPOOL_BWD: {
        lhn_view x = mkview(P, ws, o.in_buf[0], o.in_coff[0], o.in_C[0]);
        const lhn_bnsum bs = mkbns(ws, o.ws[1], o.ws[2], o.i[5], o.i[6]);
        rc = lhn_avgpool_bwd3(&x, reinterpret_cast<const float*>(at(ws, o.ws[0])), o.i[0], o.i[1], o.i[3] > 0 ? o.i[3] : x.C, o.i[4],
                              reinterpret_cast<float*>(at(ws, P->bufs[o.in_buf[0]].grad_off)), o.i[2], bs.sums ? &bs : nullptr, stream);
        break;
      }
      case OP_SHUFFLE_BWD: {
        lhn_view a = mkview(P, ws, o.in_buf[0], o.in_coff[0], o.in_C[0]);
        lhn_view b = mkview(P, ws, o.in_buf[1], o.in_coff[1], o.in_C[1]);
        lhn_view d = mkview(P, ws, o.out_buf, o.out_coff, o.out_C);
        rc = lhn_shuffle2_bwd(&a, &b, &d, reinterpret_cast<const float*>(at(ws, P->bufs[o.out_buf].grad_off)),
                              o.i[0] ? reinterpret_cast<float*>(at(ws, P->bufs[o.in_buf[0]].grad_off)) : nullptr, o.i[0] == 2,
                              o.i[1] ? reinterpret_cast<float*>(at(ws, P->bufs[o.in_buf[1]].grad_off)) : nullptr, o.i[1] == 2, stream);
        break;
      }
      case OP_GATE_REDUCE: {
        if (gfold_at == oi) break;
        lhn_view y = mkview(P, ws, o.out_buf, o.out_coff, o.out_C, false);
        float* dg = reinterpret_cast<float*>(at(ws, o.ws[3]));
        const lhn_bn_slices sl = mkslices(ws, &o.i[0], &o.ws[5], nullptr);
        rc = lhn_gate_bwd_reduce3(&y, reinterpret_cast<const float*>(at(ws, P->bufs[o.out_buf].grad_off)), dg,
                                  o.ws[4] >= 0 ? dg + (size_t)y.N * y.C : nullptr, &sl, 1, stream);
        break;
      }
      case OP_CA_MLP_BWD: {
        const lhn_buf& b = P->bufs[o.out_buf];
        if (o.ws[4] < 0 && !h0) break;
        const lhn_bn_slices sl = mkslices(ws, &o.i[0], &o.ws[6], &o.ws[8]);
        const float* dgp = reinterpret_cast<const float*>(at(ws, o.ws[3]));
        rc = lhn_ca_mlp_bwd2(reinterpret_cast<const float*>(at(ws, o.ws[0])), prm<const float>(params, o.p[0]),
                            prm<const float>(params, o.p[1]), prm<const float>(params, o.p[2]), prm<const float>(params, o.p[3]),
                            o.ws[2] >= 0 ? reinterpret_cast<const float*>(at(ws, o.ws[2])) : nullptr,
                            reinterpret_cast<const float*>(at(ws, o.ws[1])), reinterpret_cast<const float*>(at(ws, o.ws[3])),
                            reinterpret_cast<float*>(at(ws, b.dpool_off)), b.C, o.out_coff, b.H, b.W, prm<float>(grads, o.p[4]),
                            prm<float>(grads, o.p[5]), prm<float>(grads, o.p[6]), prm<float>(grads, o.p[7]),
                            prm<float>(grads, o.p[8]), prm<float>(grads, o.p[9]), prm<float>(grads, o.p[10]), b.N, o.out_C,
                            o.ws[4] >= 0 ? stage : 0, o.ws[4] >= 0 ? reinterpret_cast<double*>(at(ws, o.ws[4])) : nullptr, cscale, pscale,
                            o.ws[5] >= 0 ? dgp + (size_t)b.N * b.C : nullptr, o.ws[5] >= 0 ? reinterpret_cast<const float*>(at(ws, o.ws[5])) : nullptr,
                            &sl, stream);
        break;
      }
      case OP_ATT_MLP_BWD: {
        const lhn_buf& b = P->bufs[o.out_buf];
        if (o.ws[4] < 0 && !h0) break;
        rc = lhn_att_mlp_bwd(reinterpret_cast<const float*>(at(ws, o.ws[0])), prm<const float>(params, o.p[0]),
                             prm<const float>(params, o.p[1]), prm<const float>(params, o.p[2]), prm<const float>(params, o.p[3]),
                             o.ws[2] >= 0 ? reinterpret_cast<const float*>(at(ws, o.ws[2])) : nullptr,
                             reinterpret_cast<float*>(at(ws, o.ws[1])), reinterpret_cast<const float*>(at(ws, o.ws[3])),
                             reinterpret_cast<float*>(at(ws, b.dpool_off)), b.C, o.out_coff, b.H, b.W, prm<float>(grads, o.p[4]),
                             prm<float>(grads, o.p[5]), prm<float>(grads, o.p[6]), prm<float>(grads, o.p[7]),
                             prm<float>(grads, o.p[8]), prm<float>(grads, o.p[9]), b.N, o.out_C,
                             o.ws[4] >= 0 ? stage : 0, o.ws[4] >= 0 ? reinterpret_cast<double*>(at(ws, o.ws[4])) : nullptr, cscale, pscale,
                             stream);
        break;
      }
      case OP_SE_MLP_BWD: {
        const lhn_buf& b = P->bufs[o.out_buf];
        rc = lhn_se_mlp_bwd2(reinterpret_cast<const float*>(at(ws, o.ws[0])), prm<const float>(params, o.p[0]),
                             prm<const float>(params, o.p[1]), reinterpret_cast<const float*>(at(ws, o.ws[1])),
                             reinterpret_cast<const float*>(at(ws, o.ws[3])), reinterpret_cast<float*>(at(ws, b.dpool_off)), b.C,
                             o.out_coff, b.H, b.W, prm<float>(grads, o.p[2]), prm<float>(grads, o.p[3]), prm<float>(grads, o.p[4]),
                             prm<float>(grads, o.p[5]), b.N, o.out_C, o.i[0], o.i[1], stream);
        break;
      }
      case OP_CBAM: {
        lhn_view p = mkview(P, ws, o.in_buf[0], o.in_coff[0], o.in_C[0]), r = mkview(P, ws, o.in_buf[1], o.in_coff[1], o.in_C[1]);
        lhn_view y = mkview(P, ws, o.out_buf, o.out_coff, o.out_C);
        rc = lhn_cbam_fwd(&p, &r, prm<const float>(params, o.p[0]), prm<const float>(params, o.p[1]), prm<const float>(params, o.p[2]),
                          &y, reinterpret_cast<float*>(at(ws, o.ws[0])), stream);
        break;
      }
      case OP_CBAM_BWD: {
        lhn_view p = mkview(P, ws, o.in_buf[0], o.in_coff[0], o.in_C[0]), r = mkview(P, ws, o.in_buf[1], o.in_coff[1], o.in_C[1]);
        lhn_view y = mkview(P, ws, o.out_buf, o.out_coff, o.out_C);
        rc = lhn_cbam_bwd(&p, &r, prm<const float>(params, o.p[0]), prm<const float>(params, o.p[1]), prm<const float>(params, o.p[2]),
                          &y, reinterpret_cast<const float*>(at(ws, P->bufs[o.out_buf].grad_off)),
                          reinterpret_cast<float*>(at(ws, P->bufs[o.in_buf[0]].grad_off)),
                          reinterpret_cast<float*>(at(ws, P->bufs[o.in_buf[1]].grad_off)), prm<float>(grads, o.p[3]),
                          prm<float>(grads, o.p[4]), prm<float>(grads, o.p[5]), reinterpret_cast<const float*>(at(ws, o.ws[0])),
                          reinterpret_cast<float*>(at(ws, o.ws[1])), stream);
// ... 111 lines not shown
```

Measured before the change: 9643 images/s.

## Batch adjacent independent plan ops into paired kernel launches

Adds paired kernel variants for maxpool fwd/bwd, elementwise fwd/bwd, avgpool fwd and BN finalize. Each paired kernel runs two independent jobs selected by blockIdx.y. The plan detects adjacent independent ops at creation time and dispatches them as one launch. This cuts kernel launch count and tail gaps between small kernels, at the cost of extra dependency analysis and the risk of pairing ops that are not truly independent.

```diff
diff --git a/include/lhn.h b/include/lhn.h
--- a/include/lhn.h
+++ b/include/lhn.h
@@ -413,6 +413,45 @@
 int lhn_adam_step(float* param, const float* grad, float* exp_avg, float* exp_avg_sq, int64_t n, double lr, double beta1,
                   double beta2, double eps, double weight_decay, int64_t step, void* stream);
 
+typedef struct lhn_maxpool_job {
+  const lhn_view*      x;
+  const lhn_view*      y;
+  const float*         dy;
+  float*               dx;
+  int32_t              dx_accumulate;
+  const lhn_bnsum*     bns;
+  const lhn_grad_adds* adds;
+} lhn_maxpool_job;
+typedef struct lhn_ew_job {
+  const lhn_view*         srcs;
+  int32_t                 nsrc;
+  const float*            coef;
+  const lhn_view*         dst;
+  float                   out_slope;
+  int32_t                 mode;
+  const float*            ddst;
+  const float*            dst_dpool;
+  float* const*           dsrcs;
+  const int*              accumulate;
+  const lhn_bnsum* const* bns;
+} lhn_ew_job;
+typedef struct lhn_avgpool_job {
+  const lhn_view*      x;
+  float*               out;
+  int32_t              OH, OW, out_cstride, out_coff;
+  float*               pstat;
+  const lhn_bn_slices* slices;
+  const lhn_view*      copy_src;
+} lhn_avgpool_job;
+int lhn_maxpool2_fwd_pair(const lhn_maxpool_job* a, const lhn_maxpool_job* b, void* stream);
+int lhn_maxpool2_bwd_pair(const lhn_maxpool_job* a, const lhn_maxpool_job* b, void* stream);
+int lhn_ew_fwd_pair(const lhn_ew_job* a, const lhn_ew_job* b, void* stream);
+int lhn_ew_bwd_pair(const lhn_ew_job* a, const lhn_ew_job* b, void* stream);
+int lhn_ew_bwd_multi_pair(const lhn_ew_job* a, const lhn_ew_job* b, void* stream);
+int lhn_avgpool_fwd_pair(const lhn_avgpool_job* a, const lhn_avgpool_job* b, void* stream);
+int lhn_bn_finalize_pair(const double* stats_a, const lhn_bnfin* a, int stat_channels_a, const double* stats_b, const lhn_bnfin* b,
+                         int stat_channels_b, int training, void* stream);
+
 typedef struct lhn_op {
   int32_t kind;
   int32_t in_buf[3], in_coff[3], in_C[3];
@@ -434,6 +473,7 @@
 int   lhn_plan_head_gate_fold(void* plan);
 int   lhn_plan_pw_dz_dead(void* plan, int bwd_index);
 int   lhn_plan_fwd_fin_consumer(void* plan, int fwd_index);
+int   lhn_plan_pair(void* plan, int phase, int index);
 #define LHN_RUN_TABLES_CURRENT 2
 #define LHN_RUN_GRAPH 4
 int   lhn_plan_run(void* plan, int phase, void* workspace, void* const* params, void* const* grads,
diff --git a/litehandnet_amd/_lib.py b/litehandnet_amd/_lib.py
--- a/litehandnet_amd/_lib.py
+++ b/litehandnet_amd/_lib.py
@@ -52,6 +52,8 @@
     "lhn_ca_mlp_bwd", "lhn_reduce_replicas", "lhn_fold_stat_replicas", "lhn_plan_create", "lhn_plan_destroy", "lhn_plan_run", "lhn_plan_run_range",
     "lhn_cbam_layout", "lhn_cbam_fwd", "lhn_cbam_bwd",
     "lhn_ccw_scratch_bytes", "lhn_ccw_pool_fwd", "lhn_ccw_gate_fwd", "lhn_ccw_dw_fwd", "lhn_ccw_shuffle_fwd",
+    "lhn_maxpool2_fwd_pair", "lhn_maxpool2_bwd_pair", "lhn_ew_fwd_pair", "lhn_ew_bwd_pair", "lhn_ew_bwd_multi_pair", "lhn_avgpool_fwd_pair",
+    "lhn_bn_finalize_pair", "lhn_plan_pair",
 ]
 
 
diff --git a/litehandnet_amd/csrc/k_misc.hip b/litehandnet_amd/csrc/k_misc.hip
--- a/litehandnet_amd/csrc/k_misc.hip
+++ b/litehandnet_amd/csrc/k_misc.hip
@@ -8,19 +8,18 @@
 }
 static inline bool pow2i(int v) { return v > 0 && (v & (v - 1)) == 0; }
 
-__global__ void __launch_bounds__(LHN_FIN_THREADS) k_bn_finalize(const double* __restrict__ stats, const float* __restrict__ gamma,
+__device__ __forceinline__ void bn_finalize_job(const double* __restrict__ stats, const float* __restrict__ gamma,
                               const float* __restrict__ beta, float* __restrict__ rmean, float* __restrict__ rvar,
                               int64_t* __restrict__ nbt, float* __restrict__ table, int cs, int coff, int C,
                               float* __restrict__ save, double count, float eps, float momentum, float slope, int training,
-                              const float* __restrict__ cbias, int SC) {
-  __shared__ double part[2 * LHN_FIN_THREADS];
-  const int nt = blockDim.x;
+                              const float* __restrict__ cbias, int SC, int nt, double* __restrict__ part) {
+  const bool mine = (int)threadIdx.x < nt;
   int G = nt / C;
   G = G < 1 ? 1 : (G > LHN_STAT_REPLICAS ? LHN_STAT_REPLICAS : G);
   for (int c0 = 0; c0 < C; c0 += nt) {
     const int g = threadIdx.x / C, c = c0 + (G > 1 ? threadIdx.x - g * C : threadIdx.x);
     if (c0) __syncthreads();
-    if (training && g < G && c < C) {
+    if (training && mine && g < G && c < C) {
       double s1 = 0, s2 = 0;
 #pragma unroll 4
       for (int r = g; r < LHN_STAT_REPLICAS; r += G) {
@@ -31,7 +30,7 @@
       part[2 * threadIdx.x + 1] = s2;
     }
     __syncthreads();
-    if (g != 0 || c >= C) continue;
+    if (!mine || g != 0 || c >= C) continue;
     double mean, var;
     const double cb = cbias ? (double)cbias[c] : 0.0;
     if (training) {
@@ -56,6 +55,33 @@
     }
   }
   if (training && nbt && threadIdx.x == 0) nbt[0] += 1;
+}
+__global__ void __launch_bounds__(LHN_FIN_THREADS) k_bn_finalize(const double* __restrict__ stats, const float* __restrict__ gamma,
+                              const float* __restrict__ beta, float* __restrict__ rmean, float* __restrict__ rvar,
+                              int64_t* __restrict__ nbt, float* __restrict__ table, int cs, int coff, int C,
+                              float* __restrict__ save, double count, float eps, float momentum, float slope, int training,
+                              const float* __restrict__ cbias, int SC) {
+  __shared__ double part[2 * LHN_FIN_THREADS];
+  bn_finalize_job(stats, gamma, beta, rmean, rvar, nbt, table, cs, coff, C, save, count, eps, momentum, slope, training, cbias, SC,
+                  blockDim.x, part);
+}
+struct FinJob {
+  const double* stats;
+  const float *gamma, *beta, *cbias;
+  float *rmean, *rvar, *table, *save;
+  int64_t* nbt;
+  double count;
+  int cs, coff, C, SC, nt;
+  float eps, momentum, slope;
+};
+__global__ void __launch_bounds__(LHN_FIN_THREADS) k_bn_finalize_pair(FinJob a, FinJob b, int training) {
+  __shared__ double part[2 * LHN_FIN_THREADS];
+  if (blockIdx.y == 0)
+    bn_finalize_job(a.stats, a.gamma, a.beta, a.rmean, a.rvar, a.nbt, a.table, a.cs, a.coff, a.C, a.save, a.count, a.eps, a.momentum,
+                    a.slope, training, a.cbias, a.SC, a.nt, part);
+  else
+    bn_finalize_job(b.stats, b.gamma, b.beta, b.rmean, b.rvar, b.nbt, b.table, b.cs, b.coff, b.C, b.save, b.count, b.eps, b.momentum,
+                    b.slope, training, b.cbias, b.SC, b.nt, part);
 }
 
 __global__ void k_table_fill(float* __restrict__ table, int cs, int coff, int C, float sc, float sh, float sl) {
@@ -104,7 +130,7 @@
   return s < in - 1 ? s : in - 1;
 }
 template <bool BIL>
-__global__ void __launch_bounds__(256, BIL ? 1 : 3) k_ew_fwd(EwSrcs S, int nsrc, lhn_view dst, float out_slope) {
+__device__ __forceinline__ void ew_fwd_body(const EwSrcs& S, int nsrc, const lhn_view& dst, float out_slope) {
   const int C4 = dst.C >> 2, c4 = threadIdx.x % C4, pl = threadIdx.x / C4, PL = 256 / C4;
   const int rows = dst.N * dst.H;
   Xf4 xf[3];
@@ -213,11 +239,24 @@
     }
   }
 }
-
-__global__ void __launch_bounds__(256) k_ew_bwd_src(lhn_view src, lhn_view dst, const float* __restrict__ ddst,
-                                                    const float* __restrict__ dst_dpool, float out_slope,
-                                                    float* __restrict__ dsrc, int accumulate, lhn_bnsum bs) {
-  __shared__ f4 bred[512];
+template <bool BIL>
+__global__ void __launch_bounds__(256, BIL ? 1 : 3) k_ew_fwd(EwSrcs S, int nsrc, lhn_view dst, float out_slope) {
+  ew_fwd_body<BIL>(S, nsrc, dst, out_slope);
+}
+struct EwFwdJob {
+  EwSrcs S;
+  int nsrc;
+  lhn_view dst;
+  float out_slope;
+};
+__global__ void __launch_bounds__(256, 3) k_ew_fwd_pair(EwFwdJob a, EwFwdJob b) {
+  if (blockIdx.y == 0) ew_fwd_body<false>(a.S, a.nsrc, a.dst, a.out_slope);
+  else ew_fwd_body<false>(b.S, b.nsrc, b.dst, b.out_slope);
+}
+
+__device__ __forceinline__ void ew_bwd_src_job(const lhn_view& src, const lhn_view& dst, const float* __restrict__ ddst,
+                                               const float* __restrict__ dst_dpool, float out_slope,
+                                               float* __restrict__ dsrc, int accumulate, const lhn_bnsum& bs, f4* bred) {
   const int C4 = src.C >> 2, c4 = threadIdx.x % C4, pl = threadIdx.x / C4, PL = 256 / C4;
   f4 bsum = (f4){0.f, 0.f, 0.f, 0.f}, bsq = bsum, bmean = bsum, binv = bsum;
   Xf4 bxf;
@@ -279,6 +318,25 @@
   }
   if (bs.sums) lhn_bns_flush(bs, bsum, bsq, C4, bred);
 }
+__global__ void __launch_bounds__(256) k_ew_bwd_src(lhn_view src, lhn_view dst, const float* __restrict__ ddst,
+                                                    const float* __restrict__ dst_dpool, float out_slope,
+                                                    float* __restrict__ dsrc, int accumulate, lhn_bnsum bs) {
+  __shared__ f4 bred[512];
+  ew_bwd_src_job(src, dst, ddst, dst_dpool, out_slope, dsrc, accumulate, bs, bred);
+}
+struct EwBwdSrcJob {
+  lhn_view src, dst;
+  const float *ddst, *dst_dpool;
+  float* dsrc;
+  float out_slope;
+  int accumulate;
+  lhn_bnsum bs;
+};
+__global__ void __launch_bounds__(256) k_ew_bwd_src_pair(EwBwdSrcJob a, EwBwdSrcJob b) {
+  __shared__ f4 bred[512];
+  if (blockIdx.y == 0) ew_bwd_src_job(a.src, a.dst, a.ddst, a.dst_dpool, a.out_slope, a.dsrc, a.accumulate, a.bs, bred);
+  else ew_bwd_src_job(b.src, b.dst, b.ddst, b.dst_dpool, b.out_slope, b.dsrc, b.accumulate, b.bs, bred);
+}
 
 struct EwBwdMulti {
   int n;
@@ -287,9 +345,8 @@
   int acc[3];
   lhn_bnsum bs[3];
 };
-__global__ void __launch_bounds__(256) k_ew_bwd_multi(EwBwdMulti m, lhn_view dst, const float* __restrict__ ddst,
-                                                      const float* __restrict__ dst_dpool, float out_slope) {
-  __shared__ f4 bred[512];
+__device__ __forceinline__ void ew_bwd_multi_job(const EwBwdMulti& m, const lhn_view& dst, const float* __restrict__ ddst,
+                                                 const float* __restrict__ dst_dpool, float out_slope, f4* bred) {
   const int C4 = dst.C >> 2, c4 = threadIdx.x % C4, pl = threadIdx.x / C4, PL = 256 / C4;
   f4 bsum[3], bsq[3], bmean[3], binv[3];
   Xf4 bxf[3];
@@ -346,8 +403,24 @@
       __syncthreads();
     }
 }
-
-__global__ void __launch_bounds__(256) k_maxpool2_fwd(lhn_view x, lhn_view y) {
+__global__ void __launch_bounds__(256) k_ew_bwd_multi(EwBwdMulti m, lhn_view dst, const float* __restrict__ ddst,
+                                                      const float* __restrict__ dst_dpool, float out_slope) {
+  __shared__ f4 bred[512];
+  ew_bwd_multi_job(m, dst, ddst, dst_dpool, out_slope, bred);
+}
+struct EwBwdMultiJob {
+  EwBwdMulti m;
+  lhn_view dst;
+  const float *ddst, *dst_dpool;
+  float out_slope;
+};
+__global__ void __launch_bounds__(256) k_ew_bwd_multi_pair(EwBwdMultiJob a, EwBwdMultiJob b) {
+  __shared__ f4 bred[512];
+  if (blockIdx.y == 0) ew_bwd_multi_job(a.m, a.dst, a.ddst, a.dst_dpool, a.out_slope, bred);
+  else ew_bwd_multi_job(b.m, b.dst, b.ddst, b.dst_dpool, b.out_slope, bred);
+}
+
+__device__ __forceinline__ void maxpool2_fwd_job(const lhn_view& x, const lhn_view& y) {
   const int C4 = y.C >> 2, c4 = threadIdx.x % C4, pl = threadIdx.x / C4, PL = 256 / C4;
   const int ca = x.coff + 4 * c4;
   const Xf4 xf = lhn_load_xf(x, ca);
@@ -372,10 +445,18 @@
     }
   }
 }
+__global__ void __launch_bounds__(256) k_maxpool2_fwd(lhn_view x, lhn_view y) { maxpool2_fwd_job(x, y); }
+struct MaxpoolFwdJob {
+  lhn_view x, y;
+};
+__global__ void __launch_bounds__(256) k_maxpool2_fwd_pair(MaxpoolFwdJob a, MaxpoolFwdJob b) {
+  if (blockIdx.y == 0) maxpool2_fwd_job(a.x, a.y);
+  else maxpool2_fwd_job(b.x, b.y);
+}
 template <bool ADD>
-__global__ void __launch_bounds__(256) k_maxpool2_bwd(lhn_view x, lhn_view y, const float* __restrict__ dy,
-                                                      float* __restrict__ dx, int accumulate, lhn_bnsum bs, lhn_grad_adds ad) {
-  __shared__ f4 bred[512];
+__device__ __forceinline__ void maxpool2_bwd_job(const lhn_view& x, const lhn_view& y, const float* __restrict__ dy,
+                                                 float* __restrict__ dx, int accumulate, const lhn_bnsum& bs, const lhn_grad_adds& ad,
+                                                 f4* bred) {
   const int C4 = y.C >> 2, c4 = threadIdx.x % C4, pl = threadIdx.x / C4, PL = 256 / C4;
   const int ca = x.coff + 4 * c4;
   const Xf4 xf = lhn_load_xf(x, ca);
@@ -440,6 +521,26 @@
   }
   if (bs.sums) lhn_bns_flush(bs, bsum, bsq, C4, bred);
 }
+template <bool ADD>
+__global__ void __launch_bounds__(256) k_maxpool2_bwd(lhn_view x, lhn_view y, const float* __restrict__ dy,
+                                                      float* __restrict__ dx, int accumulate, lhn_bnsum bs, lhn_grad_adds ad) {
+  __shared__ f4 bred[512];
+  maxpool2_bwd_job<ADD>(x, y, dy, dx, accumulate, bs, ad, bred);
+}
+struct MaxpoolBwdJob {
+  lhn_view x, y;
+  const float* dy;
+  float* dx;
+  int accumulate;
+  lhn_bnsum bs;
+  lhn_grad_adds ad;
+};
+template <bool ADD>
+__global__ void __launch_bounds__(256) k_maxpool2_bwd_pair(MaxpoolBwdJob a, MaxpoolBwdJob b) {
+  __shared__ f4 bred[512];
+  if (blockIdx.y == 0) maxpool2_bwd_job<ADD>(a.x, a.y, a.dy, a.dx, a.accumulate, a.bs, a.ad, bred);
+  else maxpool2_bwd_job<ADD>(b.x, b.y, b.dy, b.dx, b.accumulate, b.bs, b.ad, bred);
+}
 
 struct BnSlices {
   const float* save[2];
@@ -462,9 +563,8 @@
 }
 
 template <bool STAT, bool COPY>
-__global__ void __launch_bounds__(256) k_avgpool_fwd(lhn_view x, float* __restrict__ out, int OH, int OW, int ostride,
-                                                     int ocoff, float* __restrict__ pstat, BnSlices sl, lhn_view src) {
-  __shared__ f4 red[STAT ? 768 : 256];
+__device__ __forceinline__ void avgpool_fwd_job(const lhn_view& x, float* __restrict__ out, int OH, int OW, int ostride,
+                                                int ocoff, float* __restrict__ pstat, const BnSlices& sl, const lhn_view& src, f4* red) {
   const int C4 = x.C >> 2, PL = 256 / C4;
   const int b = blockIdx.x;
   const int ow = b % OW, oh = (b / OW) % OH, n = b / (OW * OH);
@@ -568,6 +668,24 @@
       *reinterpret_cast<f4*>(pstat + ((int64_t)b * 2 + 1) * x.C + 4 * threadIdx.x) = t1;
     }
   }
+}
+template <bool STAT, bool COPY>
+__global__ void __launch_bounds__(256) k_avgpool_fwd(lhn_view x, float* __restrict__ out, int OH, int OW, int ostride,
+                                                     int ocoff, float* __restrict__ pstat, BnSlices sl, lhn_view src) {
+  __shared__ f4 red[STAT ? 768 : 256];
+  avgpool_fwd_job<STAT, COPY>(x, out, OH, OW, ostride, ocoff, pstat, sl, src, red);
+}
+struct AvgpoolFwdJob {
+  lhn_view x;
+  float* out;
+  int ostride, ocoff;
+};
+__global__ void __launch_bounds__(256) k_avgpool_fwd_pair(AvgpoolFwdJob a, AvgpoolFwdJob b, int OH, int OW) {
+  __shared__ f4 red[256];
+  BnSlices sl;
+  sl.n = 0;
+  if (blockIdx.y == 0) avgpool_fwd_job<false, false>(a.x, a.out, OH, OW, a.ostride, a.ocoff, nullptr, sl, a.x, red);
+  else avgpool_fwd_job<false, false>(b.x, b.out, OH, OW, b.ostride, b.ocoff, nullptr, sl, b.x, red);
 }
 __global__ void __launch_bounds__(256) k_avgpool_small(lhn_view x, float* __restrict__ out, int OH, int OW, int ostride, int ocoff) {
   const int C4 = x.C >> 2;
@@ -1634,19 +1752,59 @@
   return lhn_bn_finalize2(stats, gamma, beta, running_mean, running_var, nbt, table, cstride, coff, C, C, save, count, eps, momentum,
                           slope, training, conv_bias, stream);
 }
-int lhn_bn_finalize2(const double* stats, const float* gamma, const float* beta, float* running_mean, float* running_var,
-                     int64_t* nbt, float* table, int cstride, int coff, int C, int stat_channels, float* save, double count,
-                     float eps, float momentum, float slope, int training, const float* conv_bias, void* stream) {
+static int fin_args(const double* stats, const float* gamma, const float* beta, float* running_mean, float* running_var, int64_t* nbt,
+                   float* table, int cstride, int coff, int C, int stat_channels, float* save, double count, float eps, float momentum,
+                   float slope, int training, const float* conv_bias, FinJob* j) {
   LHN_CHECK_ARG(table && C > 0 && coff >= 0 && coff + C <= cstride && stat_channels >= C, "lhn_bn_finalize: bad table slice");
   LHN_CHECK_ARG(training ? (stats != nullptr) : (running_mean && running_var), "lhn_bn_finalize: missing statistics");
   LHN_CHECK_ARG(!training || count >= 1, "lhn_bn_finalize: count");
   int nt = training ? (C >= LHN_FIN_THREADS ? LHN_FIN_THREADS : (LHN_FIN_THREADS / C > LHN_STAT_REPLICAS ? LHN_STAT_REPLICAS : LHN_FIN_THREADS / C) * C)
                     : (C <= 64 ? 64 : (C <= 128 ? 128 : 256));
   nt = (nt + 63) / 64 * 64;
-  hipLaunchKernelGGL(k_bn_finalize, dim3(1), dim3(nt), 0, (hipStream_t)stream, stats,
+  j->stats = stats; j->gamma = gamma; j->beta = beta; j->cbias = conv_bias;
+  j->rmean = running_mean; j->rvar = running_var; j->table = table; j->save = save; j->nbt = nbt;
+  j->count = count;
+  j->cs = cstride; j->coff = coff; j->C = C; j->SC = stat_channels; j->nt = nt;
+  j->eps = eps; j->momentum = momentum; j->slope = slope;
+  return 0;
+}
+int lhn_bn_finalize2(const double* stats, const float* gamma, const float* beta, float* running_mean, float* running_var,
+                     int64_t* nbt, float* table, int cstride, int coff, int C, int stat_channels, float* save, double count,
+                     float eps, float momentum, float slope, int training, const float* conv_bias, void* stream) {
+  FinJob j;
+  if (fin_args(stats, gamma, beta, running_mean, running_var, nbt, table, cstride, coff, C, stat_channels, save, count, eps, momentum, slope,
+              training, conv_bias, &j))
+    return 1;
+  hipLaunchKernelGGL(k_bn_finalize, dim3(1), dim3(j.nt), 0, (hipStream_t)stream, stats,
                      gamma, beta, running_mean, running_var, nbt, table, cstride, coff, C, save, count, eps, momentum,
                      slope, training, conv_bias, stat_channels);
   LHN_CHECK_LAUNCH("lhn_bn_finalize");
+  return 0;
+}
+static bool spans_meet(const float* a, int64_t na, const float* b, int64_t nb) {
+  return a && b && a < b + nb && b < a + na;
+}
+static bool views_meet(const float* a, int64_t pix_a, int cs_a, int co_a, int C_a, const float* b, int64_t pix_b, int cs_b, int co_b, int C_b) {
+  if (!a || !b) return false;
+  if (a == b && cs_a == cs_b) return co_a < co_b + C_b && co_b < co_a + C_a;
+  return spans_meet(a + co_a, (pix_a - 1) * cs_a + C_a, b + co_b, (pix_b - 1) * cs_b + C_b);
+}
+int lhn_bn_finalize_pair(const double* stats_a, const lhn_bnfin* a, int stat_channels_a, const double* stats_b, const lhn_bnfin* b,
+                         int stat_channels_b, int training, void* stream) {
+  LHN_CHECK_ARG(a && b, "lhn_bn_finalize_pair: two jobs");
+  FinJob ja, jb;
+  if (fin_args(stats_a, a->gamma, a->beta, a->running_mean, a->running_var, a->num_batches_tracked, a->table, a->cstride, a->coff, a->C,
+              stat_channels_a, a->save_mean_invstd, a->count, a->eps, a->momentum, a->slope, training, a->conv_bias, &ja) ||
+      fin_args(stats_b, b->gamma, b->beta, b->running_mean, b->running_var, b->num_batches_tracked, b->table, b->cstride, b->coff, b->C,
+              stat_channels_b, b->save_mean_invstd, b->count, b->eps, b->momentum, b->slope, training, b->conv_bias, &jb))
+    return 1;
+  LHN_CHECK_ARG(!views_meet(ja.table, 3, ja.cs, ja.coff, ja.C, jb.table, 3, jb.cs, jb.coff, jb.C), "lhn_bn_finalize_pair: the table slices overlap");
+  LHN_CHECK_ARG(!training || (!spans_meet(ja.rmean, ja.C, jb.rmean, jb.C) && !spans_meet(ja.rvar, ja.C, jb.rvar, jb.C) &&
+                              !spans_meet(ja.rmean, ja.C, jb.rvar, jb.C) && !spans_meet(ja.rvar, ja.C, jb.rmean, jb.C) &&
+                              !(ja.nbt && ja.nbt == jb.nbt) && !spans_meet(ja.save, 2 * ja.SC, jb.save, 2 * jb.SC)),
+                "lhn_bn_finalize_pair: running statistics, num_batches_tracked or saved statistics overlap");
+  hipLaunchKernelGGL(k_bn_finalize_pair, dim3(1, 2), dim3(ja.nt > jb.nt ? ja.nt : jb.nt), 0, (hipStream_t)stream, ja, jb, training);
+  LHN_CHECK_LAUNCH("lhn_bn_finalize_pair");
   return 0;
 }
 
@@ -1670,22 +1828,51 @@
 int lhn_ew_fwd2(const lhn_view* srcs, int nsrc, const float* coef, const lhn_view* dst, float out_slope, void* stream) {
   return lhn_ew_fwd3(srcs, nsrc, coef, dst, out_slope, 0, stream);
 }
-int lhn_ew_fwd3(const lhn_view* srcs, int nsrc, const float* coef, const lhn_view* dst, float out_slope, int mode, void* stream) {
+static int ew_fwd_args(const lhn_view* srcs, int nsrc, const float* coef, const lhn_view* dst, float out_slope, int mode, EwFwdJob* j) {
   LHN_CHECK_ARG(srcs && nsrc >= 1 && nsrc <= 3 && lhn_view_ok(dst) && mode >= 0 && mode <= 3, "lhn_ew_fwd: 1..3 sources, valid dst");
-  EwSrcs S;
-  memset(&S, 0, sizeof(S));
-  S.mode = mode;
+  memset(j, 0, sizeof(*j));
+  j->S.mode = mode;
   for (int i = 0; i < nsrc; ++i) {
     LHN_CHECK_ARG(lhn_view_ok(&srcs[i]) && srcs[i].C == dst->C && srcs[i].N == dst->N && lhn_no_pend(&srcs[i]), "lhn_ew_fwd: source %d mismatch", i);
-    S.v[i] = srcs[i];
-    S.coef[i] = coef ? coef[i] : 1.f;
+    j->S.v[i] = srcs[i];
+    j->S.coef[i] = coef ? coef[i] : 1.f;
   }
   LHN_CHECK_ARG(dst->C % 4 == 0 && dst->C <= 1024, "lhn_ew_fwd: C=%d", dst->C);
-  if (S.mode & 2)
-    hipLaunchKernelGGL(k_ew_fwd<true>, dim3(grid_cap((int64_t)dst->N * dst->H, 8)), dim3(256), 0, (hipStream_t)stream, S, nsrc, *dst, out_slope);
+  j->nsrc = nsrc;
+  j->dst = *dst;
+  j->out_slope = out_slope;
+  return 0;
+}
+int lhn_ew_fwd3(const lhn_view* srcs, int nsrc, const float* coef, const lhn_view* dst, float out_slope, int mode, void* stream) {
+  EwFwdJob j;
+  if (ew_fwd_args(srcs, nsrc, coef, dst, out_slope, mode, &j)) return 1;
+  if (j.S.mode & 2)
+    hipLaunchKernelGGL(k_ew_fwd<true>, dim3(grid_cap((int64_t)dst->N * dst->H, 8)), dim3(256), 0, (hipStream_t)stream, j.S, nsrc, *dst, out_slope);
   else
-    hipLaunchKernelGGL(k_ew_fwd<false>, dim3(grid_cap((int64_t)dst->N * dst->H, 8)), dim3(256), 0, (hipStream_t)stream, S, nsrc, *dst, out_slope);
+    hipLaunchKernelGGL(k_ew_fwd<false>, dim3(grid_cap((int64_t)dst->N * dst->H, 8)), dim3(256), 0, (hipStream_t)stream, j.S, nsrc, *dst, out_slope);
   LHN_CHECK_LAUNCH("lhn_ew_fwd");
+  return 0;
+}
+static bool same_geometry(const lhn_view& a, const lhn_view& b) { return a.N == b.N && a.H == b.H && a.W == b.W && a.C == b.C; }
+static bool view_outputs_meet(const lhn_view& a, const lhn_view& b) {
+  return views_meet(a.data, (int64_t)a.N * a.H * a.W, a.cstride, a.coff, a.C, b.data, (int64_t)b.N * b.H * b.W, b.cstride, b.coff, b.C);
+}
+static bool grad_outputs_meet(const float* da, const lhn_view& a, const float* db, const lhn_view& b) {
+  return views_meet(da, (int64_t)a.N * a.H * a.W, a.cstride, a.coff, a.C, db, (int64_t)b.N * b.H * b.W, b.cstride, b.coff, b.C);
+}
+int lhn_ew_fwd_pair(const lhn_ew_job* a, const lhn_ew_job* b, void* stream) {
+  LHN_CHECK_ARG(a && b, "lhn_ew_fwd_pair: two jobs");
+  EwFwdJob ja, jb;
+  if (ew_fwd_args(a->srcs, a->nsrc, a->coef, a->dst, a->out_slope, a->mode, &ja) ||
+      ew_fwd_args(b->srcs, b->nsrc, b->coef, b->dst, b->out_slope, b->mode, &jb))
+    return 1;
+  LHN_CHECK_ARG(a->mode == 0 && b->mode == 0, "lhn_ew_fwd_pair: product and bilinear combines take lhn_ew_fwd3");
+  bool geo = same_geometry(ja.dst, jb.dst) && ja.nsrc == jb.nsrc;
+  for (int i = 0; geo && i < ja.nsrc; ++i) geo = same_geometry(ja.S.v[i], jb.S.v[i]);
+  LHN_CHECK_ARG(geo, "lhn_ew_fwd_pair: the two jobs differ in geometry");
+  LHN_CHECK_ARG(!view_outputs_meet(ja.dst, jb.dst), "lhn_ew_fwd_pair: the two outputs overlap");
+  hipLaunchKernelGGL(k_ew_fwd_pair, dim3(grid_cap((int64_t)ja.dst.N * ja.dst.H, 8), 2), dim3(256), 0, (hipStream_t)stream, ja, jb);
+  LHN_CHECK_LAUNCH("lhn_ew_fwd_pair");
   return 0;
 }
 
@@ -1721,31 +1908,55 @@
   *out = *in;
   return 0;
 }
-int lhn_ew_bwd2(const lhn_view* src, const lhn_view* dst, const float* ddst, const float* dst_dpool, float out_slope,
-                float* dsrc, int accumulate, void* stream) {
-  return lhn_ew_bwd3(src, dst, ddst, dst_dpool, out_slope, dsrc, accumulate, nullptr, stream);
-}
-int lhn_ew_bwd3(const lhn_view* src, const lhn_view* dst, const float* ddst, const float* dst_dpool, float out_slope,
-                float* dsrc, int accumulate, const lhn_bnsum* bns, void* stream) {
+static int ew_bwd_src_args(const lhn_view* src, const lhn_view* dst, const float* ddst, const float* dst_dpool, float out_slope,
+                           float* dsrc, int accumulate, const lhn_bnsum* bns, EwBwdSrcJob* j) {
   LHN_CHECK_ARG(lhn_view_ok(src) && lhn_view_ok(dst) && ddst && dsrc && src->C == dst->C && lhn_no_pend(src) && lhn_no_pend(dst), "lhn_ew_bwd2: bad args");
   LHN_CHECK_ARG(dst->H % src->H == 0 && dst->W % src->W == 0, "lhn_ew_bwd2: non-integer upsample");
   LHN_CHECK_ARG((out_slope != LHN_SLOPE_SILU && out_slope != LHN_SLOPE_RELU_SIGMOID) || (dst->H == src->H && dst->W == src->W), "lhn_ew_bwd2: SiLU / ReLU-sigmoid need a single same-size source");
   LHN_CHECK_ARG(src->C % 4 == 0 && src->C <= 1024, "lhn_ew_bwd2: C=%d", src->C);
-  lhn_bnsum bs;
-  if (bns_of(bns, src, &bs, "lhn_ew_bwd3")) return 1;
+  if (bns_of(bns, src, &j->bs, "lhn_ew_bwd3")) return 1;
+  j->src = *src; j->dst = *dst;
+  j->ddst = ddst; j->dst_dpool = dst_dpool; j->dsrc = dsrc;
+  j->out_slope = out_slope; j->accumulate = accumulate;
+  return 0;
+}
+int lhn_ew_bwd2(const lhn_view* src, const lhn_view* dst, const float* ddst, const float* dst_dpool, float out_slope,
+                float* dsrc, int accumulate, void* stream) {
+  return lhn_ew_bwd3(src, dst, ddst, dst_dpool, out_slope, dsrc, accumulate, nullptr, stream);
+}
+int lhn_ew_bwd3(const lhn_view* src, const lhn_view* dst, const float* ddst, const float* dst_dpool, float out_slope,
+                float* dsrc, int accumulate, const lhn_bnsum* bns, void* stream) {
+  EwBwdSrcJob j;
+  if (ew_bwd_src_args(src, dst, ddst, dst_dpool, out_slope, dsrc, accumulate, bns, &j)) return 1;
   hipLaunchKernelGGL(k_ew_bwd_src, dim3(grid_cap((int64_t)src->N * src->H, 8)), dim3(256), 0, (hipStream_t)stream, *src, *dst, ddst,
-                     dst_dpool, out_slope, dsrc, accumulate, bs);
+                     dst_dpool, out_slope, dsrc, accumulate, j.bs);
   LHN_CHECK_LAUNCH("lhn_ew_bwd2");
   return 0;
 }
-
-int lhn_ew_bwd_multi(const lhn_view* srcs, int nsrc, const lhn_view* dst, const float* ddst, const float* dst_dpool, float out_slope,
-                     float* const* dsrcs, const int* accumulate, const lhn_bnsum* const* bns, void* stream) {
+int lhn_ew_bwd_pair(const lhn_ew_job* a, const lhn_ew_job* b, void* stream) {
+  LHN_CHECK_ARG(a && b && a->nsrc == 1 && b->nsrc == 1 && a->dsrcs && b->dsrcs && a->accumulate && b->accumulate,
+                "lhn_ew_bwd_pair: two single-source jobs");
+  EwBwdSrcJob ja, jb;
+  if (ew_bwd_src_args(a->srcs, a->dst, a->ddst, a->dst_dpool, a->out_slope, a->dsrcs[0], a->accumulate[0], a->bns ? a->bns[0] : nullptr, &ja) ||
+      ew_bwd_src_args(b->srcs, b->dst, b->ddst, b->dst_dpool, b->out_slope, b->dsrcs[0], b->accumulate[0], b->bns ? b->bns[0] : nullptr, &jb))
+    return 1;
+  LHN_CHECK_ARG(a->out_slope != LHN_SLOPE_SILU && a->out_slope != LHN_SLOPE_RELU_SIGMOID && b->out_slope != LHN_SLOPE_SILU &&
+                    b->out_slope != LHN_SLOPE_RELU_SIGMOID,
+                "lhn_ew_bwd_pair: SiLU / ReLU-sigmoid take lhn_ew_bwd3");
+  LHN_CHECK_ARG(same_geometry(ja.src, jb.src) && same_geometry(ja.dst, jb.dst), "lhn_ew_bwd_pair: the two jobs differ in geometry");
+  LHN_CHECK_ARG(!grad_outputs_meet(ja.dsrc, ja.src, jb.dsrc, jb.src), "lhn_ew_bwd_pair: the two outputs overlap");
+  hipLaunchKernelGGL(k_ew_bwd_src_pair, dim3(grid_cap((int64_t)ja.src.N * ja.src.H, 8), 2), dim3(256), 0, (hipStream_t)stream, ja, jb);
+  LHN_CHECK_LAUNCH("lhn_ew_bwd_pair");
+  return 0;
+}
+
+static int ew_bwd_multi_args(const lhn_view* srcs, int nsrc, const lhn_view* dst, const float* ddst, const float* dst_dpool, float out_slope,
+                             float* const* dsrcs, const int* accumulate, const lhn_bnsum* const* bns, EwBwdMultiJob* j) {
   LHN_CHECK_ARG(srcs && nsrc >= 1 && nsrc <= 3 && lhn_view_ok(dst) && ddst && dsrcs && accumulate && lhn_no_pend(dst), "lhn_ew_bwd_multi: bad args");
   LHN_CHECK_ARG(out_slope != LHN_SLOPE_SILU && out_slope != LHN_SLOPE_RELU_SIGMOID, "lhn_ew_bwd_multi: SiLU / ReLU-sigmoid take lhn_ew_bwd3");
   LHN_CHECK_ARG(dst->C % 4 == 0 && dst->C <= 1024, "lhn_ew_bwd_multi: C=%d", dst->C);
-  EwBwdMulti m;
-  memset(&m, 0, sizeof(m));
+  memset(j, 0, sizeof(*j));
+  EwBwdMulti& m = j->m;
   m.n = nsrc;
   for (int k = 0; k < nsrc; ++k) {
     const lhn_view* v = &srcs[k];
@@ -1756,18 +1967,57 @@
     m.acc[k] = accumulate[k];
     if (bns_of(bns ? bns[k] : nullptr, v, &m.bs[k], "lhn_ew_bwd_multi")) return 1;
   }
-  hipLaunchKernelGGL(k_ew_bwd_multi, dim3(grid_cap((int64_t)dst->N * dst->H, 8)), dim3(256), 0, (hipStream_t)stream, m, *dst, ddst, dst_dpool, out_slope);
+  j->dst = *dst;
+  j->ddst = ddst; j->dst_dpool = dst_dpool;
+  j->out_slope = out_slope;
+  return 0;
+}
+int lhn_ew_bwd_multi(const lhn_view* srcs, int nsrc, const lhn_view* dst, const float* ddst, const float* dst_dpool, float out_slope,
+                     float* const* dsrcs, const int* accumulate, const lhn_bnsum* const* bns, void* stream) {
+  EwBwdMultiJob j;
+  if (ew_bwd_multi_args(srcs, nsrc, dst, ddst, dst_dpool, out_slope, dsrcs, accumulate, bns, &j)) return 1;
+  hipLaunchKernelGGL(k_ew_bwd_multi, dim3(grid_cap((int64_t)dst->N * dst->H, 8)), dim3(256), 0, (hipStream_t)stream, j.m, *dst, ddst, dst_dpool, out_slope);
   LHN_CHECK_LAUNCH("lhn_ew_bwd_multi");
   return 0;
 }
-
-int lhn_maxpool2_fwd(const lhn_view* x, const lhn_view* y, void* stream) {
+int lhn_ew_bwd_multi_pair(const lhn_ew_job* a, const lhn_ew_job* b, void* stream) {
+  LHN_CHECK_ARG(a && b, "lhn_ew_bwd_multi_pair: two jobs");
+  EwBwdMultiJob ja, jb;
+  if (ew_bwd_multi_args(a->srcs, a->nsrc, a->dst, a->ddst, a->dst_dpool, a->out_slope, a->dsrcs, a->accumulate, a->bns, &ja) ||
+      ew_bwd_multi_args(b->srcs, b->nsrc, b->dst, b->ddst, b->dst_dpool, b->out_slope, b->dsrcs, b->accumulate, b->bns, &jb))
+    return 1;
+  LHN_CHECK_ARG(same_geometry(ja.dst, jb.dst) && ja.m.n == jb.m.n, "lhn_ew_bwd_multi_pair: the two jobs differ in geometry");
+  for (int k = 0; k < ja.m.n; ++k)
+    for (int l = 0; l < jb.m.n; ++l)
+      LHN_CHECK_ARG(!grad_outputs_meet(ja.m.dsrc[k], ja.m.src[k], jb.m.dsrc[l], jb.m.src[l]), "lhn_ew_bwd_multi_pair: outputs %d and %d of the two jobs overlap", k, l);
+  hipLaunchKernelGGL(k_ew_bwd_multi_pair, dim3(grid_cap((int64_t)ja.dst.N * ja.dst.H, 8), 2), dim3(256), 0, (hipStream_t)stream, ja, jb);
+  LHN_CHECK_LAUNCH("lhn_ew_bwd_multi_pair");
+  return 0;
+}
+
+static int maxpool2_fwd_args(const lhn_view* x, const lhn_view* y, MaxpoolFwdJob* j) {
   LHN_CHECK_ARG(lhn_view_ok(x) && lhn_view_ok(y) && x->C == y->C, "lhn_maxpool2_fwd: bad views");
   LHN_CHECK_ARG(y->H == (x->H + 1) / 2 && y->W == (x->W + 1) / 2 && y->N == x->N, "lhn_maxpool2_fwd: geometry");
   LHN_CHECK_ARG(y->C % 4 == 0 && y->C <= 1024, "lhn_maxpool2_fwd: C=%d", y->C);
   LHN_CHECK_ARG(lhn_no_pend(x), "lhn_maxpool2_fwd: lhn_view.pend is reserved (NULL)");
+  j->x = *x; j->y = *y;
+  return 0;
+}
+int lhn_maxpool2_fwd(const lhn_view* x, const lhn_view* y, void* stream) {
+  MaxpoolFwdJob j;
+  if (maxpool2_fwd_args(x, y, &j)) return 1;
   hipLaunchKernelGGL(k_maxpool2_fwd, dim3(grid_cap((int64_t)y->N * y->H, 8)), dim3(256), 0, (hipStream_t)stream, *x, *y);
   LHN_CHECK_LAUNCH("lhn_maxpool2_fwd");
+  return 0;
+}
+int lhn_maxpool2_fwd_pair(const lhn_maxpool_job* a, const lhn_maxpool_job* b, void* stream) {
+  LHN_CHECK_ARG(a && b, "lhn_maxpool2_fwd_pair: two jobs");
+  MaxpoolFwdJob ja, jb;
+  if (maxpool2_fwd_args(a->x, a->y, &ja) || maxpool2_fwd_args(b->x, b->y, &jb)) return 1;
+  LHN_CHECK_ARG(same_geometry(ja.x, jb.x) && same_geometry(ja.y, jb.y), "lhn_maxpool2_fwd_pair: the two jobs differ in geometry");
+  LHN_CHECK_ARG(!view_outputs_meet(ja.y, jb.y), "lhn_maxpool2_fwd_pair: the two outputs overlap");
+  hipLaunchKernelGGL(k_maxpool2_fwd_pair, dim3(grid_cap((int64_t)ja.y.N * ja.y.H, 8), 2), dim3(256), 0, (hipStream_t)stream, ja, jb);
+  LHN_CHECK_LAUNCH("lhn_maxpool2_fwd_pair");
   return 0;
 }
 int lhn_maxpool2_bwd(const lhn_view* x, const lhn_view* y, const float* dy, float* dx, int dx_accumulate, void* stream) {
@@ -1777,15 +2027,15 @@
                       void* stream) {
   return lhn_maxpool2_bwd3(x, y, dy, dx, dx_accumulate, bns, nullptr, stream);
 }
-int lhn_maxpool2_bwd3(const lhn_view* x, const lhn_view* y, const float* dy, float* dx, int dx_accumulate, const lhn_bnsum* bns,
-                      const lhn_grad_adds* adds, void* stream) {
+static int maxpool2_bwd_args(const lhn_view* x, const lhn_view* y, const float* dy, float* dx, int dx_accumulate, const lhn_bnsum* bns,
+                             const lhn_grad_adds* adds, MaxpoolBwdJob* j, bool* with_adds) {
   LHN_CHECK_ARG(lhn_view_ok(x) && lhn_view_ok(y) && dy && dx && x->C == y->C && lhn_no_pend(x), "lhn_maxpool2_bwd: bad args");
   LHN_CHECK_ARG(y->C % 4 == 0 && y->C <= 1024, "lhn_maxpool2_bwd: C=%d", y->C);
-  lhn_bnsum bs;
-  if (bns_of(bns, x, &bs, "lhn_maxpool2_bwd2")) return 1;
-  lhn_grad_adds ad;
+  if (bns_of(bns, x, &j->bs, "lhn_maxpool2_bwd2")) return 1;
+  lhn_grad_adds& ad = j->ad;
   memset(&ad, 0, sizeof(ad));
-  if (adds && (adds->same || adds->pooled)) {
+  *with_adds = adds && (adds->same || adds->pooled);
+  if (*with_adds) {
     ad = *adds;
     LHN_CHECK_ARG(x->H % 2 == 0 && x->W % 2 == 0 && y->H == x->H / 2 && y->W == x->W / 2, "lhn_maxpool2_bwd3: gradient addends need even H, W (%dx%d)", x->H, x->W);
     LHN_CHECK_ARG(!ad.same || (ad.same_cstride % 4 == 0 && ad.same_coff % 4 == 0 && ad.same_coff >= 0 && ad.same_coff + x->C <= ad.same_cstride),
@@ -1793,25 +2043,78 @@
     LHN_CHECK_ARG(!ad.pooled || (ad.OH > 0 && ad.OW > 0 && ad.OH <= x->H && ad.OW <= x->W && ad.pooled_cstride % 4 == 0 && ad.pooled_coff % 4 == 0 &&
                                  ad.pooled_coff >= 0 && ad.pooled_coff + x->C <= ad.pooled_cstride),
                   "lhn_maxpool2_bwd3: pooled addend layout");
-    hipLaunchKernelGGL(k_maxpool2_bwd<true>, dim3(grid_cap((int64_t)y->N * y->H, 8)), dim3(256), 0, (hipStream_t)stream, *x, *y, dy, dx, dx_accumulate, bs, ad);
-  } else {
-    hipLaunchKernelGGL(k_maxpool2_bwd<false>, dim3(grid_cap((int64_t)y->N * y->H, 8)), dim3(256), 0, (hipStream_t)stream, *x, *y, dy, dx, dx_accumulate, bs, ad);
-  }
+  }
+  j->x = *x; j->y = *y;
+  j->dy = dy; j->dx = dx;
+  j->accumulate = dx_accumulate;
+  return 0;
+}
+int lhn_maxpool2_bwd3(const lhn_view* x, const lhn_view* y, const float* dy, float* dx, int dx_accumulate, const lhn_bnsum* bns,
+                      const lhn_grad_adds* adds, void* stream) {
+  MaxpoolBwdJob j;
+  bool with_adds;
+  if (maxpool2_bwd_args(x, y, dy, dx, dx_accumulate, bns, adds, &j, &with_adds)) return 1;
+  if (with_adds)
+    hipLaunchKernelGGL(k_maxpool2_bwd<true>, dim3(grid_cap((int64_t)y->N * y->H, 8)), dim3(256), 0, (hipStream_t)stream, *x, *y, dy, dx, dx_accumulate, j.bs, j.ad);
+  else
+    hipLaunchKernelGGL(k_maxpool2_bwd<false>, dim3(grid_cap((int64_t)y->N * y->H, 8)), dim3(256), 0, (hipStream_t)stream, *x, *y, dy, dx, dx_accumulate, j.bs, j.ad);
   LHN_CHECK_LAUNCH("lhn_maxpool2_bwd");
+  return 0;
+}
+int lhn_maxpool2_bwd_pair(const lhn_maxpool_job* a, const lhn_maxpool_job* b, void* stream) {
+  LHN_CHECK_ARG(a && b, "lhn_maxpool2_bwd_pair: two jobs");
+  MaxpoolBwdJob ja, jb;
+  bool adds_a, adds_b;
+  if (maxpool2_bwd_args(a->x, a->y, a->dy, a->dx, a->dx_accumulate, a->bns, a->adds, &ja, &adds_a) ||
+      maxpool2_bwd_args(b->x, b->y, b->dy, b->dx, b->dx_accumulate, b->bns, b->adds, &jb, &adds_b))
+    return 1;
+  LHN_CHECK_ARG(same_geometry(ja.x, jb.x) && same_geometry(ja.y, jb.y), "lhn_maxpool2_bwd_pair: the two jobs differ in geometry");
+  LHN_CHECK_ARG(!grad_outputs_meet(ja.dx, ja.x, jb.dx, jb.x), "lhn_maxpool2_bwd_pair: the two outputs overlap");
+  const dim3 g(grid_cap((int64_t)ja.y.N * ja.y.H, 8), 2);
+  if (adds_a || adds_b) hipLaunchKernelGGL(k_maxpool2_bwd_pair<true>, g, dim3(256), 0, (hipStream_t)stream, ja, jb);
+  else hipLaunchKernelGGL(k_maxpool2_bwd_pair<false>, g, dim3(256), 0, (hipStream_t)stream, ja, jb);
+  LHN_CHECK_LAUNCH("lhn_maxpool2_bwd_pair");
   return 0;
 }
 
 int lhn_avgpool_fwd(const lhn_view* x, float* out, int OH, int OW, void* stream) {
   return lhn_avgpool_fwd2(x, out, OH, OW, x ? x->C : 0, 0, stream);
 }
-int lhn_avgpool_fwd2(const lhn_view* x, float* out, int OH, int OW, int out_cstride, int out_coff, void* stream) {
+static int avgpool_fwd_args(const lhn_view* x, float* out, int OH, int OW, int out_cstride, int out_coff, AvgpoolFwdJob* j, bool* small) {
   LHN_CHECK_ARG(lhn_view_ok(x) && out && OH > 0 && OW > 0 && out_coff >= 0 && out_coff % 4 == 0 && out_cstride % 4 == 0 &&
                     out_coff + x->C <= out_cstride,
                 "lhn_avgpool_fwd: bad args");
   LHN_CHECK_ARG(x->C % 4 == 0 && x->C <= 1024, "lhn_avgpool_fwd: C=%d", x->C);
   LHN_CHECK_ARG(lhn_no_pend(x), "lhn_avgpool_fwd: lhn_view.pend is reserved (NULL)");
   const int binmax = ((x->H + OH - 1) / OH + 1) * ((x->W + OW - 1) / OW + 1);
-  if (binmax <= 25) {
+  *small = binmax <= 25;
+  j->x = *x;
+  j->out = out;
+  j->ostride = out_cstride; j->ocoff = out_coff;
+  return 0;
+}
+int lhn_avgpool_fwd_pair(const lhn_avgpool_job* a, const lhn_avgpool_job* b, void* stream) {
+  LHN_CHECK_ARG(a && b, "lhn_avgpool_fwd_pair: two jobs");
+  LHN_CHECK_ARG(!a->pstat && !a->copy_src && !b->pstat && !b->copy_src, "lhn_avgpool_fwd_pair: the statistics / copy forms take lhn_avgpool_fwd4");
+  AvgpoolFwdJob ja, jb;
+  bool small_a, small_b;
+  if (avgpool_fwd_args(a->x, a->out, a->OH, a->OW, a->out_cstride, a->out_coff, &ja, &small_a) ||
+      avgpool_fwd_args(b->x, b->out, b->OH, b->OW, b->out_cstride, b->out_coff, &jb, &small_b))
+    return 1;
+  LHN_CHECK_ARG(same_geometry(ja.x, jb.x) && a->OH == b->OH && a->OW == b->OW, "lhn_avgpool_fwd_pair: the two jobs differ in geometry");
+  LHN_CHECK_ARG(!small_a && !small_b, "lhn_avgpool_fwd_pair: bins of at most 4x4 take lhn_avgpool_fwd2 (one thread per bin)");
+  const int64_t bins = (int64_t)ja.x.N * a->OH * a->OW;
+  LHN_CHECK_ARG(!views_meet(ja.out, bins, ja.ostride, ja.ocoff, ja.x.C, jb.out, bins, jb.ostride, jb.ocoff, jb.x.C),
+                "lhn_avgpool_fwd_pair: the two outputs overlap");
+  hipLaunchKernelGGL(k_avgpool_fwd_pair, dim3((unsigned)bins, 2), dim3(256), 0, (hipStream_t)stream, ja, jb, a->OH, a->OW);
+  LHN_CHECK_LAUNCH("lhn_avgpool_fwd_pair");
+  return 0;
+}
+int lhn_avgpool_fwd2(const lhn_view* x, float* out, int OH, int OW, int out_cstride, int out_coff, void* stream) {
+  AvgpoolFwdJob j;
+  bool small;
+  if (avgpool_fwd_args(x, out, OH, OW, out_cstride, out_coff, &j, &small)) return 1;
+  if (small) {
     const int64_t total = (int64_t)x->N * OH * OW * (x->C / 4);
     hipLaunchKernelGGL(k_avgpool_small, dim3(grid_cap((total + 255) / 256, 16)), dim3(256), 0, (hipStream_t)stream, *x, out, OH, OW, out_cstride, out_coff);
   } else
diff --git a/litehandnet_amd/csrc/lhn_plan.cpp b/litehandnet_amd/csrc/lhn_plan.cpp
--- a/litehandnet_amd/csrc/lhn_plan.cpp
+++ b/litehandnet_amd/csrc/lhn_plan.cpp
@@ -40,6 +40,7 @@
   std::vector<lhn_op> fwd, bwd;
   std::vector<uint8_t> pw_dz_dead;
   std::vector<uint8_t> fwd_fin;
+  std::vector<uint8_t> pair[2];
   std::vector<GraphEntry> graphs;
   uint64_t tick = 0;
   int graph_misses = 0;
@@ -192,6 +193,224 @@
   return true;
 }
 
+static bool pair_launch() {
+  static int v = -1;
+  if (v < 0) {
+    const char* e = getenv("LHN_PAIR_LAUNCH");
+    v = (e && e[0] == '0') ? 0 : 1;
+  }
+  return v == 1;
+}
+struct Region {
+  int64_t base, pix;
+  int cs, coff, C;
+};
+static bool regions_meet(const Region& a, const Region& b) {
+  if (a.base < 0 || b.base < 0) return false;
+  if (a.base == b.base && a.cs == b.cs) return a.coff < b.coff + b.C && b.coff < a.coff + a.C;
+  const int64_t alo = a.base + 4 * (int64_t)a.coff, ahi = a.base + 4 * ((a.pix - 1) * a.cs + a.coff + a.C);
+  const int64_t blo = b.base + 4 * (int64_t)b.coff, bhi = b.base + 4 * ((b.pix - 1) * b.cs + b.coff + b.C);
+  return alo < bhi && blo < ahi;
+}
+struct Access {
+  std::vector<Region> rd, wr;
+};
+static bool pair_access(const Plan* P, const lhn_op& o, Access* A) {
+  auto data = [&](int buf, int coff, int C) {
+    const lhn_buf& b = P->bufs[buf];
+    return Region{b.data_off, (int64_t)b.N * b.H * b.W, b.C, coff, C};
+  };
+  auto grad = [&](int buf, int coff, int C) {
+    const lhn_buf& b = P->bufs[buf];
+    return Region{b.grad_off, (int64_t)b.N * b.H * b.W, b.C, coff, C};
+  };
+  if (o.out_buf < 0 && o.kind != OP_AVGPOOL) return false;
+  switch (o.kind) {
+    case OP_MAXPOOL:
+      if (o.in_buf[0] < 0) return false;
+      A->rd.push_back(data(o.in_buf[0], o.in_coff[0], o.in_C[0]));
+      A->wr.push_back(data(o.out_buf, o.out_coff, o.out_C));
+      return true;
+    case OP_EW:
+      if (o.i[0] < 1 || o.i[0] > 3 || o.i[2] != 0) return false;
+      for (int k = 0; k < o.i[0]; ++k) {
+        if (o.in_buf[k] < 0) return false;
+        A->rd.push_back(data(o.in_buf[k], o.in_coff[k], o.in_C[k]));
+      }
+      A->wr.push_back(data(o.out_buf, o.out_coff, o.out_C));
+      return true;
+    case OP_AVGPOOL: {
+      if (o.in_buf[0] < 0 || o.ws[0] < 0 || o.ws[1] >= 0 || o.in_buf[1] >= 0) return false;
+      const lhn_buf& b = P->bufs[o.in_buf[0]];
+      const int OH = o.i[0], OW = o.i[1];
+      if (OH < 1 || OW < 1 || ((b.H + OH - 1) / OH + 1) * ((b.W + OW - 1) / OW + 1) <= 25) return false;
+      A->rd.push_back(data(o.in_buf[0], o.in_coff[0], o.in_C[0]));
+      A->wr.push_back(Region{o.ws[0], (int64_t)b.N * OH * OW, o.i[3] > 0 ? o.i[3] : o.in_C[0], o.i[4], o.in_C[0]});
+      return true;
+    }
+    case OP_MAXPOOL_BWD: {
+      if (o.in_buf[0] < 0) return false;
+      const lhn_buf& xb = P->bufs[o.in_buf[0]];
+      A->rd.push_back(data(o.in_buf[0], o.in_coff[0], o.in_C[0]));
+      A->rd.push_back(grad(o.out_buf, o.out_coff, o.out_C));
+      if (o.ws[2] >= 0) A->rd.push_back(Region{o.ws[2], (int64_t)xb.N * xb.H * xb.W, o.i[1], o.i[2], o.in_C[0]});
+      if (o.ws[3] >= 0) A->rd.push_back(Region{o.ws[3], (int64_t)xb.N * (o.i[7] >> 16) * (o.i[7] & 0xffff), o.i[3], o.i[6], o.in_C[0]});
+      A->wr.push_back(grad(o.in_buf[0], o.in_coff[0], o.in_C[0]));
+      return true;
+    }
+    case OP_EW_BWD: {
+      if ((o.i[1] != 0 && o.i[1] != 3) || o.f[0] == LHN_SLOPE_SILU || o.f[0] == LHN_SLOPE_RELU_SIGMOID) return false;
+      A->rd.push_back(data(o.out_buf, o.out_coff, o.out_C));
+      A->rd.push_back(grad(o.out_buf, o.out_coff, o.out_C));
+      for (int k = 0; k < (o.i[1] == 3 ? 3 : 1) && o.in_buf[k] >= 0; ++k) {
+        A->rd.push_back(data(o.in_buf[k], o.in_coff[k], o.in_C[k]));
+        A->wr.push_back(grad(o.in_buf[k], o.in_coff[k], o.in_C[k]));
+      }
+      return !A->wr.empty();
+    }
+    default:
+      return false;
+  }
+}
+static bool same_shape(const Plan* P, int a, int b) {
+  if ((a < 0) != (b < 0)) return false;
+  if (a < 0) return true;
+  const lhn_buf &x = P->bufs[a], &y = P->bufs[b];
+  return x.N == y.N && x.H == y.H && x.W == y.W;
+}
+static bool conv_keeps_finalize_launch(const Plan* P, const std::vector<lhn_op>& ops, size_t oi) {
+  const lhn_op& o = ops[oi];
+  const bool conv = o.kind == OP_STEM || o.kind == OP_PW || o.kind == OP_DW || (o.kind == OP_KXK && o.i[1] != 1);
+  if (!conv || !conv_has_bn(o) || o.ws[0] < 0 || o.out_buf < 0 || P->bufs[o.out_buf].table_off < 0) return false;
+  if (o.kind == OP_PW && (o.i[1] || o.i[2] > 0)) return false;
+  if ((o.kind == OP_PW || o.kind == OP_DW) && (int)o.f[3] > 1) return false;
+  return !fuse_finalize() && !P->fwd_fin[oi];
+}
+static int pair_at(const Plan* P, const std::vector<lhn_op>& ops, size_t oi, bool forward) {
+  if (!pair_launch() || oi + 1 >= ops.size()) return 0;
+  const lhn_op &a = ops[oi], &b = ops[oi + 1];
+  if (forward && conv_keeps_finalize_launch(P, ops, oi) && conv_keeps_finalize_launch(P, ops, oi + 1)) {
+    for (int k = 0; k < 3; ++k)
+      if (b.in_buf[k] == a.out_buf && b.in_coff[k] < a.out_coff + a.out_C && a.out_coff < b.in_coff[k] + b.in_C[k]) return 0;
+    if (b.kind == OP_STEM) return 0;
+    if (a.out_buf == b.out_buf && a.out_coff < b.out_coff + b.out_C && b.out_coff < a.out_coff + a.out_C) return 0;
+    for (int k = 2; k <= 6; ++k)
+      if (a.p[k] >= 0 && a.p[k] == b.p[k]) return 0;
+    if (a.ws[0] == b.ws[0] || (a.ws[1] >= 0 && a.ws[1] == b.ws[1])) return 0;
+    return 2;
+  }
+  if (a.kind != b.kind) return 0;
+  if (a.kind == OP_EW && (a.i[0] != b.i[0] || a.i[2] != b.i[2])) return 0;
+  if (a.kind == OP_EW_BWD && a.i[1] != b.i[1]) return 0;
+  if (a.kind == OP_AVGPOOL && (a.i[0] != b.i[0] || a.i[1] != b.i[1])) return 0;
+  if (a.out_C != b.out_C || !same_shape(P, a.out_buf, b.out_buf)) return 0;
+  for (int k = 0; k < 3; ++k)
+    if (!same_shape(P, a.in_buf[k], b.in_buf[k]) || (a.in_buf[k] >= 0 && a.in_C[k] != b.in_C[k])) return 0;
+  Access A, B;
+  if (!pair_access(P, a, &A) || !pair_access(P, b, &B)) return 0;
+  for (const Region& w : A.wr) {
+    for (const Region& q : B.wr)
+      if (regions_meet(w, q)) return 0;
+    for (const Region& q : B.rd)
+      if (regions_meet(w, q)) return 0;
+  }
+  for (const Region& w : B.wr)
+    for (const Region& q : A.rd)
+      if (regions_meet(w, q)) return 0;
+  return 1;
+}
+
+struct MaxpoolArgs {
+  lhn_view x, y;
+  lhn_bnsum bs;
+  lhn_grad_adds ad;
+  lhn_maxpool_job job;
+};
+static void mk_maxpool(const Plan* P, void* ws, const lhn_op& o, bool backward, MaxpoolArgs* A) {
+  A->x = mkview(P, ws, o.in_buf[0], o.in_coff[0], o.in_C[0]);
+  A->y = mkview(P, ws, o.out_buf, o.out_coff, o.out_C);
+  memset(&A->job, 0, sizeof(A->job));
+  A->job.x = &A->x;
+  A->job.y = &A->y;
+  if (!backward) return;
+  A->bs = mkbns(ws, o.ws[0], o.ws[1], o.i[4], o.i[5]);
+  lhn_grad_adds& ad = A->ad;
+  memset(&ad, 0, sizeof(ad));
+  if (o.ws[2] >= 0) {
+    ad.same = reinterpret_cast<const float*>(at(ws, o.ws[2]));
+    ad.same_cstride = o.i[1]; ad.same_coff = o.i[2];
+  }
+  if (o.ws[3] >= 0) {
+    ad.pooled = reinterpret_cast<const float*>(at(ws, o.ws[3]));
+    ad.pooled_cstride = o.i[3]; ad.pooled_coff = o.i[6];
+    ad.OH = o.i[7] >> 16; ad.OW = o.i[7] & 0xffff;
+  }
+  A->job.dy = reinterpret_cast<const float*>(at(ws, P->bufs[o.out_buf].grad_off));
+  A->job.dx = reinterpret_cast<float*>(at(ws, P->bufs[o.in_buf[0]].grad_off));
+  A->job.dx_accumulate = o.i[0];
+  A->job.bns = A->bs.sums ? &A->bs : nullptr;
+  A->job.adds = (ad.same || ad.pooled) ? &ad : nullptr;
+}
+struct EwArgs {
+  lhn_view srcs[3], d;
+  float coef[3];
+  float* dsrcs[3];
+  int acc[3];
+  lhn_bnsum bsv[3];
+  const lhn_bnsum* bsp[3];
+  lhn_ew_job job;
+};
+static void mk_ew_fwd(const Plan* P, void* ws, const lhn_op& o, EwArgs* A) {
+  for (int k = 0; k < o.i[0]; ++k) A->srcs[k] = mkview(P, ws, o.in_buf[k], o.in_coff[k], o.in_C[k]);
+  A->d = mkview(P, ws, o.out_buf, o.out_coff, o.out_C);
+  for (int k = 0; k < 3; ++k) A->coef[k] = o.f[4 + k];
+  memset(&A->job, 0, sizeof(A->job));
+  A->job.srcs = A->srcs;
+  A->job.nsrc = o.i[0];
+  A->job.coef = o.i[1] ? A->coef : nullptr;
+  A->job.dst = &A->d;
+  A->job.out_slope = o.f[0];
+  A->job.mode = o.i[2];
+}
+static void mk_ew_bwd(const Plan* P, void* ws, const lhn_op& o, EwArgs* A) {
+  const lhn_buf& db = P->bufs[o.out_buf];
+  A->d = mkview(P, ws, o.out_buf, o.out_coff, o.out_C);
+  const bool multi = o.i[1] == 3;
+  A->acc[0] = o.i[0]; A->acc[1] = o.i[2]; A->acc[2] = o.i[3];
+  A->bsv[0] = mkbns(ws, o.ws[0], o.ws[1], o.i[4], o.i[5]);
+  A->bsv[1] = multi ? mkbns(ws, o.ws[2], o.ws[3], o.i[6], o.i[7]) : mkbns(ws, -1, -1, 0, 0);
+  A->bsv[2] = multi ? mkbns(ws, o.ws[4], o.ws[5], (int)o.f[4], (int)o.f[5]) : mkbns(ws, -1, -1, 0, 0);
+  int ns = 0;
+  for (; ns < (multi ? 3 : 1) && o.in_buf[ns] >= 0; ++ns) {
+    A->srcs[ns] = mkview(P, ws, o.in_buf[ns], o.in_coff[ns], o.in_C[ns]);
+    A->dsrcs[ns] = reinterpret_cast<float*>(at(ws, P->bufs[o.in_buf[ns]].grad_off));
+    A->bsp[ns] = A->bsv[ns].sums ? &A->bsv[ns] : nullptr;
+  }
+  memset(&A->job, 0, sizeof(A->job));
+  A->job.srcs = A->srcs;
+  A->job.nsrc = ns;
+  A->job.dst = &A->d;
+  A->job.out_slope = o.f[0];
+  A->job.ddst = reinterpret_cast<const float*>(at(ws, db.grad_off));
+  A->job.dst_dpool = reinterpret_cast<const float*>(at(ws, db.dpool_off));
+  A->job.dsrcs = A->dsrcs;
+  A->job.accumulate = A->acc;
+  A->job.bns = A->bsp;
+}
+struct AvgpoolArgs {
+  lhn_view x;
+  lhn_avgpool_job job;
+};
+static void mk_avgpool(const Plan* P, void* ws, const lhn_op& o, AvgpoolArgs* A) {
+  A->x = mkview(P, ws, o.in_buf[0], o.in_coff[0], o.in_C[0], o.i[2] == 0);
+  memset(&A->job, 0, sizeof(A->job));
+  A->job.x = &A->x;
+  A->job.out = reinterpret_cast<float*>(at(ws, o.ws[0]));
+  A->job.OH = o.i[0]; A->job.OW = o.i[1];
+  A->job.out_cstride = o.i[3] > 0 ? o.i[3] : A->x.C;
+  A->job.out_coff = o.i[4];
+}
+
 static int sep_finalize(const lhn_bnfin& f, const double* stats, int training, void* stream, int creal = 0, int repeat = 1) {
   int rc = 0;
   for (int r = 0; r < (training ? (repeat < 1 ? 1 : repeat) : 1) && !rc; ++r)
@@ -226,7 +445,23 @@
   for (size_t oi = 0; oi < p->fwd.size(); ++oi) p->fwd_fin[oi] = fwd_fin_consumer_at(p, p->fwd, oi) ? 1 : 0;
   p->pw_dz_dead.resize(p->bwd.size());
   for (size_t oi = 0; oi < p->bwd.size(); ++oi) p->pw_dz_dead[oi] = pw_dz_dead_at(p, p->bwd, oi) ? 1 : 0;
+  for (int phase = 0; phase < 2; ++phase) {
+    const std::vector<lhn_op>& ops = phase == 0 ? p->fwd : p->bwd;
+    std::vector<uint8_t>& pr = p->pair[phase];
+    pr.assign(ops.size(), 0);
+    for (size_t oi = 0; oi + 1 < ops.size(); ++oi)
+      if (!pr[oi] && pair_at(p, ops, oi, phase == 0)) {
+        pr[oi] = 1;
+        pr[oi + 1] = 2;
+      }
+  }
   return p;
+}
+
+int lhn_plan_pair(void* plan, int phase, int index) {
+  const Plan* p = static_cast<const Plan*>(plan);
+  if (!p || phase < 0 || phase > 1 || index < 0 || (size_t)index >= p->pair[phase].size()) return -1;
+  return p->pair[phase][index];
 }
 
 int lhn_plan_head_gate_fold(void* plan) {
@@ -282,6 +517,27 @@
     ffin_for = oi + 1;
     return true;
   };
+  const uint8_t* pr = whole ? P->pair[phase].data() : nullptr;
+  lhn_bnfin dfin;
+  const double* dstats = nullptr;
+  size_t dfin_for = (size_t)-1;
+  auto finalize = [&](size_t oi, const lhn_bnfin& fin, const double* stats, int creal, int repeat) -> int {
+    if (pr && pr[oi] == 1) {
+      dfin = fin;
+      dstats = stats;
+      dfin_for = oi + 1;
+      return 0;
+    }
+    if (pr && pr[oi] == 2 && dfin_for == oi) {
+      lhn_bnfin fa = dfin, fb = fin;
+      if (!training) {
+        fa.num_batches_tracked = fb.num_batches_tracked = nullptr;
+        fa.save_mean_invstd = fb.save_mean_invstd = nullptr;
+      }
+      return lhn_bn_finalize_pair(training ? dstats : nullptr, &fa, fa.C, training ? stats : nullptr, &fb, fb.C, training, stream);
+    }
+    return sep_finalize(fin, stats, training, stream, creal, repeat);
+  };
   size_t gfold_at = (size_t)-1;
   for (size_t oi = 0; oi < ops.size() && rc == 0; ++oi) {
     const lhn_op& o = ops[oi];
@@ -324,7 +580,7 @@
                                (training && o.ws[0] >= 0) ? reinterpret_cast<double*>(at(ws, o.ws[0])) : nullptr, o.i[3], o.i[4], o.i[0], o.i[1],
                                o.i[2], (bn && fz) ? &fin : nullptr, stream);
         if (!rc && bn && h1 && !skip_tables && !deferred && !fz && !hand_over(oi, fin, reinterpret_cast<const double*>(at(ws, o.ws[0]))))
-          rc = sep_finalize(fin, reinterpret_cast<const double*>(at(ws, o.ws[0])), training, stream);
+          rc = finalize(oi, fin, reinterpret_cast<const double*>(at(ws, o.ws[0])), 0, 1);
         break;
       }
       case OP_PW: {
@@ -374,7 +630,7 @@
                               (training && o.ws[0] >= 0) ? reinterpret_cast<double*>(at(ws, o.ws[0])) : nullptr, o.i[0], nchw,
                               (bn && fz) ? &fin : nullptr, &po, ffin_for == oi ? &ffin : nullptr, stream);
         if (!rc && bn && h1 && !skip_tables && !deferred && !fz && !hand_over(oi, fin, reinterpret_cast<const double*>(at(ws, o.ws[0]))))
-          rc = sep_finalize(fin, reinterpret_cast<const double*>(at(ws, o.ws[0])), training, stream, o.i[2], (int)o.f[3]);
+          rc = finalize(oi, fin, reinterpret_cast<const double*>(at(ws, o.ws[0])), o.i[2], (int)o.f[3]);
         break;
       }
       case OP_DW: {
@@ -404,7 +660,7 @@
                               (bn && fz) ? &fin : nullptr, o.i[6] > 1 ? &extra : nullptr, coef2,
                               so ? &sumv : nullptr, ffin_for == oi ? &ffin : nullptr, stream);
         if (!rc && bn && h1 && !skip_tables && !deferred && !fz && !hand_over(oi, fin, reinterpret_cast<const double*>(at(ws, o.ws[0]))))
-          rc = sep_finalize(fin, reinterpret_cast<const double*>(at(ws, o.ws[0])), training, stream, 0, (int)o.f[3]);
+          rc = finalize(oi, fin, reinterpret_cast<const double*>(at(ws, o.ws[0])), 0, (int)o.f[3]);
         break;
       }
       case OP_KXK: {
@@ -432,7 +688,7 @@
                               (bn && fz) ? &fin : nullptr,
                               o.ws[3] >= 0 ? reinterpret_cast<float*>(at(ws, o.ws[3])) : nullptr, stream);
         if (!rc && bn && h1 && !skip_tables && !deferred && !fz && !hand_over(oi, fin, reinterpret_cast<const double*>(at(ws, o.ws[0]))))
-          rc = sep_finalize(fin, reinterpret_cast<const double*>(at(ws, o.ws[0])), training, stream);
+          rc = finalize(oi, fin, reinterpret_cast<const double*>(at(ws, o.ws[0])), 0, 1);
         break;
       }
       case OP_PWDW: {
@@ -600,19 +856,25 @@
         break;
       }
       case OP_EW: {
-        lhn_view srcs[3];
-        for (int k = 0; k < o.i[0]; ++k) {
-          srcs[k] = mkview(P, ws, o.in_buf[k], o.in_coff[k], o.in_C[k]);
-        }
-        lhn_view d = mkview(P, ws, o.out_buf, o.out_coff, o.out_C);
-        const float coef[3] = {o.f[4], o.f[5], o.f[6]};
-        rc = lhn_ew_fwd3(srcs, o.i[0], o.i[1] ? coef : nullptr, &d, o.f[0], o.i[2], stream);
+        if (pr && pr[oi] == 2) break;
+        EwArgs A, B;
+        mk_ew_fwd(P, ws, o, &A);
+        if (pr && pr[oi] == 1) {
+          mk_ew_fwd(P, ws, ops[oi + 1], &B);
+          rc = lhn_ew_fwd_pair(&A.job, &B.job, stream);
+        } else
+          rc = lhn_ew_fwd3(A.srcs, A.job.nsrc, A.job.coef, &A.d, A.job.out_slope, A.job.mode, stream);
         break;
       }
       case OP_MAXPOOL: {
-        lhn_view x = mkview(P, ws, o.in_buf[0], o.in_coff[0], o.in_C[0]);
-        lhn_view y = mkview(P, ws, o.out_buf, o.out_coff, o.out_C);
-        rc = lhn_maxpool2_fwd(&x, &y, stream);
+        if (pr && pr[oi] == 2) break;
+        MaxpoolArgs A, B;
+        mk_maxpool(P, ws, o, false, &A);
+        if (pr && pr[oi] == 1) {
+          mk_maxpool(P, ws, ops[oi + 1], false, &B);
+          rc = lhn_maxpool2_fwd_pair(&A.job, &B.job, stream);
+        } else
+          rc = lhn_maxpool2_fwd(&A.x, &A.y, stream);
         break;
       }
       case OP_SHUFFLE: {
@@ -623,6 +885,14 @@
         break;
       }
       case OP_AVGPOOL: {
+        if (pr && pr[oi] == 2) break;
+        if (pr && pr[oi] == 1) {
+          AvgpoolArgs A, B;
+          mk_avgpool(P, ws, o, &A);
+          mk_avgpool(P, ws, ops[oi + 1], &B);
+          rc = lhn_avgpool_fwd_pair(&A.job, &B.job, stream);
+          break;
+        }
         lhn_view x = mkview(P, ws, o.in_buf[0], o.in_coff[0], o.in_C[0], o.i[2] == 0);
         if (o.ws[1] >= 0 || o.in_buf[1] >= 0) {
           const lhn_bn_slices sl = mkslices(ws, &o.i[5], &o.ws[2], nullptr);
@@ -779,6 +1049,14 @@
         break;
       }
       case OP_EW_BWD: {
+        if (pr && pr[oi] == 2) break;
+        if (pr && pr[oi] == 1) {
+          EwArgs A, B;
+          mk_ew_bwd(P, ws, o, &A);
+          mk_ew_bwd(P, ws, ops[oi + 1], &B);
+          rc = o.i[1] == 3 ? lhn_ew_bwd_multi_pair(&A.job, &B.job, stream) : lhn_ew_bwd_pair(&A.job, &B.job, stream);
+          break;
+        }
         lhn_view src = mkview(P, ws, o.in_buf[0], o.in_coff[0], o.in_C[0]);
         lhn_view d = mkview(P, ws, o.out_buf, o.out_coff, o.out_C);
         const lhn_buf& db = P->bufs[o.out_buf];
@@ -813,23 +1091,14 @@
         break;
       }
       case OP_MAXPOOL_BWD: {
-        lhn_view x = mkview(P, ws, o.in_buf[0], o.in_coff[0], o.in_C[0]);
-        lhn_view y = mkview(P, ws, o.out_buf, o.out_coff, o.out_C);
-        const lhn_bnsum bs = mkbns(ws, o.ws[0], o.ws[1], o.i[4], o.i[5]);
-        lhn_grad_adds ad;
-        memset(&ad, 0, sizeof(ad));
-        if (o.ws[2] >= 0) {
-          ad.same = reinterpret_cast<const float*>(at(ws, o.ws[2]));
-          ad.same_cstride = o.i[1]; ad.same_coff = o.i[2];
-        }
-        if (o.ws[3] >= 0) {
-          ad.pooled = reinterpret_cast<const float*>(at(ws, o.ws[3]));
-          ad.pooled_cstride = o.i[3]; ad.pooled_coff = o.i[6];
-          ad.OH = o.i[7] >> 16; ad.OW = o.i[7] & 0xffff;
-        }
-        rc = lhn_maxpool2_bwd3(&x, &y, reinterpret_cast<const float*>(at(ws, P->bufs[o.out_buf].grad_off)),
-                               reinterpret_cast<float*>(at(ws, P->bufs[o.in_buf[0]].grad_off)), o.i[0], bs.sums ? &bs : nullptr,
-                               (ad.same || ad.pooled) ? &ad : nullptr, stream);
+        if (pr && pr[oi] == 2) break;
+        MaxpoolArgs A, B;
+        mk_maxpool(P, ws, o, true, &A);
+        if (pr && pr[oi] == 1) {
+          mk_maxpool(P, ws, ops[oi + 1], true, &B);
+          rc = lhn_maxpool2_bwd_pair(&A.job, &B.job, stream);
+        } else
+          rc = lhn_maxpool2_bwd3(&A.x, &A.y, A.job.dy, A.job.dx, A.job.dx_accumulate, A.job.bns, A.job.adds, stream);
         break;
       }
       case OP_AVGPOOL_BWD: {
```

Result: faster. 9754 images/s (median of 6 runs) (+1.1%).
